# chihyaoma/cyclical-visual-captioning

Hardware: AMD Instinct MI355X
Metric: caption decode-steps/sec (BxT) at N=100,D=2048 (higher is better)
Workload: dtype f32; 1 GPU; cfg2: greedy caption decode; B_per_gpu=64, N=100, F=480, D=2048, A=1024, E=1024, V=5000, T=20, beam=1, hip_graph=True, parallelism=clips sharded over 1 rank(s), no collective, schedule=embedding-gate table (att-LSTM GEMM over K = 2R + one table row per word)

## Files before the change

### cyclical-visual-captioning_amd/csrc/blocks.hip

```cpp
#include <string.h>
#include "cvc_common.h"

namespace {
struct Entry { const char* name; void* fn; };
#define CVC_B(f) {#f, (void*)&f}
const Entry table[] = {
    CVC_B(cvc_attn_scores),
    CVC_B(cvc_attn_wsum),
    CVC_B(cvc_attn_scores_qparts),
    CVC_B(cvc_attn_wsum_quad),
    CVC_B(cvc_attn_wsum_frag),
    CVC_B(cvc_attn_wsum_quad_rm),
    CVC_B(cvc_attn_bwd_pair),
    CVC_B(cvc_ctxfeat_bwd_steps),
    CVC_B(cvc_tile_gemm_big),
    CVC_B(cvc_tile_gemm_plan),
    CVC_B(cvc_dproj_bwd_steps),
    CVC_B(cvc_linear_splitk_fwd),
    CVC_B(cvc_linear_top2_fwd),
    CVC_B(cvc_top2_final),
    CVC_B(cvc_packed_lstm_fwd),
    CVC_B(cvc_packed_linear_fwd),
    CVC_B(cvc_packed_lstm_embgate_fwd),
    CVC_B(cvc_packed_lstm_embgate_ex_fwd),
    CVC_B(cvc_packed_lstm_late_fwd),
    CVC_B(cvc_packed_lstm_train_fwd),
    CVC_B(cvc_packed_lstm_train_pre_fwd),
    CVC_B(cvc_packed_lstm_train_drop_fwd),
    CVC_B(cvc_lstm_pointwise_bwd),
    CVC_B(cvc_lstm_pointwise_bwd3),
    CVC_B(cvc_lstm_pointwise_bwd3_drop),
    CVC_B(cvc_pack_lstm_weights),
    CVC_B(cvc_linear_nn_planes_fwd),
    CVC_B(cvc_linear_nn_planes2_fwd),
    CVC_B(cvc_gru_seq_train_fwd),
    CVC_B(cvc_lstm_pointwise_bwd4_pair),
    CVC_B(cvc_beam_select_parts),
    CVC_B(cvc_sample_select_parts),
    CVC_B(cvc_sample_advance),
    CVC_B(cvc_tile_lstm_finish),
    CVC_B(cvc_tile_lstm_finish_embgate),
    CVC_B(cvc_tile_reorder_pack),
    CVC_B(cvc_decode_num_launches),
    CVC_B(cvc_gemm_force_generic),
    CVC_B(cvc_tile_gemm_loaders),
    CVC_B(cvc_gru_persistent_waves8),
    CVC_B(cvc_relu_dropout_fwd),
    CVC_B(cvc_relu_dropout_bwd),
    CVC_B(cvc_bn_workspace),
    CVC_B(cvc_bn_relu_train_fwd),
    CVC_B(cvc_bn_relu_train_bwd),
    CVC_B(cvc_class_softmax_bwd),
    CVC_B(cvc_layernorm_cat_bwd),
    CVC_B(cvc_attn_weighted_rows),
    CVC_B(cvc_stable_order),
    CVC_B(cvc_col_sum),
    CVC_B(cvc_col_sum_ws),
    CVC_B(cvc_lstm_persistent_sync_words),
    CVC_B(cvc_lstm_seq_persistent_fwd),
    CVC_B(cvc_lstm_seq_persistent_train_fwd),
    CVC_B(cvc_lstm_seq_fwd),
    CVC_B(cvc_lstm_seq_train_fwd),
    CVC_B(cvc_lstm_seq_bwd_work),
    CVC_B(cvc_lstm_seq_bwd),
    CVC_B(cvc_packed_lstm_bf16w_fwd),
    CVC_B(cvc_packed_linear_bf16w_fwd),
#ifdef CVC_EXPERIMENTAL
    CVC_B(cvc_gsk_plan),
    CVC_B(cvc_gsk_gemm),
    CVC_B(cvc_attn_scores_qslab),
    CVC_B(cvc_top2_slab),
    CVC_B(cvc_packed_lstm_ks_slices),
    CVC_B(cvc_packed_lstm_ks_fwd),
    CVC_B(cvc_packed_lstm_ksf_fwd),
    CVC_B(cvc_packed_lstm_ksx_local),
    CVC_B(cvc_packed_lstm_ksx_fwd),
    CVC_B(cvc_packed_lstm_wg_blocks),
    CVC_B(cvc_packed_linear_select_fwd),
    CVC_B(cvc_gru_persistent_halves),
#endif
};
}

extern "C" void* cvc_block(const char* name) {
    if (name == nullptr) return nullptr;
    for (const Entry& e : table)
        if (strcmp(e.name, name) == 0) return e.fn;
    return nullptr;
}
```

### cyclical-visual-captioning_amd/csrc/decode_driver.hip

```cpp
#include <hip/hip_runtime.h>
#include <new>
#include <stdint.h>
#include "../../include/cvc_hip.h"
#include "../../include/cvc_hip_blocks.h"
#include "../../include/cvc_hip_experimental.h"

struct gsk_launch {
    int U;
    int unit0[2], maxseg[2];
};
struct cvc_decode_plan {
    cvc_decode_desc d;
    int launches;
    gsk_launch ga, go, gl;
};

namespace {

#define CVC_TRY(expr)            \
    do {                         \
        int rc_ = (expr);        \
        ++n;                     \
        if (rc_ != 0) return rc_; \
    } while (0)

inline float* quad_off(float* buf, int k0) { return buf + (size_t)(k0 / 4) * 64 * 4; }
inline void* frag_off(void* xb, int k0) { return (char*)xb + (size_t)(k0 / 16) * 3 * 1024; }

int hip_rc(hipError_t e) { return e == hipSuccess ? 0 : (int)e; }

__global__ __launch_bounds__(256) void reset_kernel(uint4* dst, const uint4* src, size_t n16) {
    const size_t i = (size_t)blockIdx.x * 256 + threadIdx.x;
    if (i < n16) dst[i] = src != nullptr ? src[i] : uint4{0, 0, 0, 0};
}
int reset(void* dst, const void* src, size_t bytes, hipStream_t st) {
    if ((bytes & 15) || ((uintptr_t)dst & 15) || ((uintptr_t)src & 15)) {
        return hip_rc(src ? hipMemcpyAsync(dst, src, bytes, hipMemcpyDeviceToDevice, st) : hipMemsetAsync(dst, 0, bytes, st));
    }
    const size_t n16 = bytes / 16;
    hipLaunchKernelGGL(reset_kernel, dim3((unsigned)((n16 + 255) / 256)), dim3(256), 0, st, (uint4*)dst, (const uint4*)src, n16);
    return hip_rc(hipGetLastError());
}

void attn_sets(const cvc_decode_desc& d, int t, int rows, cvc_attn_set* sets) {
    sets[0] = cvc_attn_set{d.ppool, d.pool, d.mask, nullptr, d.scores_r, nullptr, d.att_steps + (size_t)t * rows * d.N, nullptr,
                           d.N, d.stream_r};
    sets[1] = cvc_attn_set{d.pconv, d.conv, nullptr, nullptr, d.scores_f, nullptr, d.attn_f, nullptr, d.F, d.stream_f};
}

int run_packed(cvc_decode_plan* p, hipStream_t st) {
    const cvc_decode_desc& d = p->d;
    const int rows = d.B, R = d.R, E = d.E, A = d.A, V = d.V, N = d.N;
    const size_t qbytes = (size_t)64 * 4 * sizeof(float);
    int n = 0;
    CVC_TRY(reset(d.xa[0], d.xa0_init, (size_t)((2 * R + E) / 4) * qbytes, st));
    CVC_TRY(reset(d.xl[0], nullptr, (size_t)(3 * R / 4) * qbytes, st));
    CVC_TRY(reset(d.ca[0], nullptr, (size_t)(R / 4) * qbytes, st));
    CVC_TRY(reset(d.cl[0], nullptr, (size_t)(R / 4) * qbytes, st));
    CVC_TRY(reset(d.words, nullptr, (size_t)rows * sizeof(int64_t), st));
    cvc_gemm_seg seg{d.fc, nullptr, d.w_fc, R, R, d.ld_w_fc, 0};
    CVC_TRY(cvc_linear_fwd(&seg, 1, d.b_ih_att, d.b_hh_att, rows, 4 * R, d.gate_fc, 4 * R, st));
    const int nblk_v = (V + 31) / 32;
    for (int t = 0; t < d.T; ++t) {
        const int rd = t & 1, wr = (t + 1) & 1;
        float *XA_r = d.xa[rd], *XA_w = d.xa[wr], *XL_r = d.xl[rd], *XL_w = d.xl[wr];
        CVC_TRY(cvc_packed_lstm_fwd((const float*)d.w_att, XA_r, 2 * R + E, nullptr, nullptr, d.gate_fc, d.ca[rd], rows, R,
                                    quad_off(XL_r, R), quad_off(XA_w, R + E), d.ca[wr], st));
        CVC_TRY(cvc_packed_linear_fwd((const float*)d.w_h, quad_off(XL_r, R), R, nullptr, rows, A, d.qsplit, d.q_parts, A, nullptr, st));
        cvc_attn_set sets[2];
        attn_sets(d, t, rows, sets);
        CVC_TRY(cvc_attn_scores_qparts(d.attn_kind, d.q_parts, d.qsplit, d.b_h, d.w_a, d.b_a, d.inv_temp, sets, 2, d.B, 1, A, st));
        CVC_TRY(cvc_attn_wsum_quad(sets, 2, d.B, 1, R, XL_r, st));
#ifdef CVC_EXPERIMENTAL
        if (d.lang_ksx)
            CVC_TRY(cvc_packed_lstm_ksx_fwd((const float*)d.w_lang, XL_r, 3 * R, d.b_ih_lang, d.b_hh_lang, nullptr, nullptr, nullptr, d.cl[rd],
                                            rows, R, XA_w, quad_off(XL_w, 2 * R), d.cl[wr], d.ksx_slab, d.ksx_flags, (unsigned)(t + 1), st));
        else
#endif
        CVC_TRY(cvc_packed_lstm_fwd((const float*)d.w_lang, XL_r, 3 * R, d.b_ih_lang, d.b_hh_lang, nullptr, d.cl[rd], rows, R, XA_w,
                                    quad_off(XL_w, 2 * R), d.cl[wr], st));
        CVC_TRY(cvc_packed_linear_fwd((const float*)d.w_o, XA_w, R, d.b_o, rows, V, 1, nullptr, V, d.top2_part, st));
        CVC_TRY(cvc_top2_final(d.top2_part, nblk_v, rows, d.unk_idx, d.words + (size_t)(t + 1) * rows, 1,
                               d.logprob ? d.logprob + (size_t)t * rows : nullptr, d.embed, E, quad_off(XA_w, R), 0, st));
    }
    p->launches = n;
    return 0;
}

int run_packed_eg(cvc_decode_plan* p, hipStream_t st) {
    const cvc_decode_desc& d = p->d;
    const int rows = d.B, R = d.R, A = d.A, V = d.V;
    const size_t qbytes = (size_t)64 * 4 * sizeof(float);
    int n = 0;
    CVC_TRY(reset(d.xa[0], nullptr, (size_t)(2 * R / 4) * qbytes, st));
    CVC_TRY(reset(d.xl[0], nullptr, (size_t)(3 * R / 4) * qbytes, st));
    CVC_TRY(reset(d.ca[0], nullptr, (size_t)(R / 4) * qbytes, st));
    CVC_TRY(reset(d.cl[0], nullptr, (size_t)(R / 4) * qbytes, st));
    CVC_TRY(reset(d.words, nullptr, (size_t)rows * sizeof(int64_t), st));
    cvc_gemm_seg seg{d.fc, nullptr, d.w_fc, R, R, d.ld_w_fc, 0};
    CVC_TRY(cvc_linear_fwd(&seg, 1, d.b_ih_att, d.b_hh_att, rows, 4 * R, d.gate_fc, 4 * R, st));
    const long long ws_att = (long long)(2 * R / 4) * 128, ws_lang = (long long)(3 * R / 4) * 128;
    const bool split2 = cvc_gemm_packed_split(-1) == 2;
    for (int t = 0; t < d.T; ++t) {
        const int rd = t & 1, wr = (t + 1) & 1;
        float *XA_r = d.xa[rd], *XA_w = d.xa[wr], *XL_r = d.xl[rd], *XL_w = d.xl[wr];
        const bool first = t == 0 && split2;
        CVC_TRY(cvc_packed_lstm_embgate_ex_fwd((const float*)d.w_att, ws_att, XA_r, first ? 32 : 2 * R, nullptr, nullptr, d.gate_fc,
                                               d.emb_gate, d.words + (size_t)t * rows, d.ca[rd], rows, R, quad_off(XL_r, R),
                                               quad_off(XA_w, R), d.ca[wr], d.att_w_cached, st));
        CVC_TRY(cvc_packed_linear_fwd((const float*)d.w_h, quad_off(XL_r, R), R, nullptr, rows, A, d.qsplit, d.q_parts, A, nullptr, st));
        cvc_attn_set sets[2];
        attn_sets(d, t, rows, sets);
        CVC_TRY(cvc_attn_scores_qparts(d.attn_kind, d.q_parts, d.qsplit, d.b_h, d.w_a, d.b_a, d.inv_temp, sets, 2, d.B, 1, A, st));
        CVC_TRY(cvc_attn_wsum_quad(sets, 2, d.B, 1, R, XL_r, st));
        if (first)
            CVC_TRY(cvc_packed_lstm_late_fwd((const float*)d.w_lang, ws_lang, XL_r, 2 * R, d.b_ih_lang, d.b_hh_lang, nullptr, d.cl[rd], rows,
                                             R, XA_w, quad_off(XL_w, 2 * R), d.cl[wr], nullptr, st));
#ifdef CVC_EXPERIMENTAL
        else if (d.lang_ksx)
            CVC_TRY(cvc_packed_lstm_ksx_fwd((const float*)d.w_lang, XL_r, 3 * R, d.b_ih_lang, d.b_hh_lang, nullptr, nullptr, nullptr, d.cl[rd],
                                            rows, R, XA_w, quad_off(XL_w, 2 * R), d.cl[wr], d.ksx_slab, d.ksx_flags, (unsigned)(t + 1), st));
#endif
        else
        CVC_TRY(cvc_packed_lstm_fwd((const float*)d.w_lang, XL_r, 3 * R, d.b_ih_lang, d.b_hh_lang, nullptr, d.cl[rd], rows, R, XA_w,
                                    quad_off(XL_w, 2 * R), d.cl[wr], st));
        CVC_TRY(cvc_packed_linear_fwd((const float*)d.w_o, XA_w, R, d.b_o, rows, V, 1, nullptr, V, d.top2_part, st));
        CVC_TRY(cvc_top2_final(d.top2_part, (V + 31) / 32, rows, d.unk_idx, d.words + (size_t)(t + 1) * rows, 1,
                               d.logprob ? d.logprob + (size_t)t * rows : nullptr, nullptr, 0, nullptr, 0, st));
    }
    p->launches = n;
    return 0;
}

#ifdef CVC_EXPERIMENTAL
int run_packed_gsk(cvc_decode_plan* p, hipStream_t st) {
    const cvc_decode_desc& d = p->d;
    const int rows = d.B, R = d.R, E = d.E, A = d.A, V = d.V;
    const size_t qbytes = (size_t)64 * 4 * sizeof(float);
    int n = 0;
    CVC_TRY(reset(d.xa[0], d.xa0_init, (size_t)((2 * R + E) / 4) * qbytes, st));
    CVC_TRY(reset(d.xl[0], nullptr, (size_t)(3 * R / 4) * qbytes, st));
    CVC_TRY(reset(d.ca[0], nullptr, (size_t)(R / 4) * qbytes, st));
    CVC_TRY(reset(d.cl[0], nullptr, (size_t)(R / 4) * qbytes, st));
    CVC_TRY(reset(d.words, nullptr, (size_t)rows * sizeof(int64_t), st));
    cvc_gemm_seg seg{d.fc, nullptr, d.w_fc, R, R, d.ld_w_fc, 0};
    CVC_TRY(cvc_linear_fwd(&seg, 1, d.b_ih_att, d.b_hh_att, rows, 4 * R, d.gate_fc, 4 * R, st));
    const long long ws_att = (long long)((2 * R + E) / 4) * 128, ws_lang = (long long)(3 * R / 4) * 128, ws_r = (long long)(R / 4) * 128;
    const float* w_att = (const float*)d.w_att;
    const float* w_lang = (const float*)d.w_lang;
    const int nblk_v = (V + 31) / 32;
    const cvc_gsk_segs seg_att{d.slab_att, p->ga.unit0[0], 2 * R / 32, p->ga.U, p->ga.maxseg[0]};
    const cvc_gsk_segs seg_o_a{d.slab_o, p->ga.unit0[1], R / 32, p->ga.U, p->ga.maxseg[1]};
    const cvc_gsk_segs seg_o_o{d.slab_o, 0, R / 32, p->go.U, p->go.maxseg[0]};
    const cvc_gsk_segs seg_lang{d.slab_lang, p->gl.unit0[0], 2 * R / 32, p->gl.U, p->gl.maxseg[0]};
    const cvc_gsk_segs seg_q{d.slab_q, p->gl.unit0[1], R / 32, p->gl.U, p->gl.maxseg[1]};
    for (int t = 0; t < d.T; ++t) {
        const int rd = t & 1, wr = (t + 1) & 1;
        float *XA_r = d.xa[rd], *XA_w = d.xa[wr], *XL_r = d.xl[rd], *XL_w = d.xl[wr];
        CVC_TRY(cvc_packed_lstm_late_fwd(w_att + (size_t)(R / 4) * 128, ws_att, quad_off(XA_r, R), E, nullptr, nullptr, d.gate_fc,
                                         d.ca[rd], rows, R, quad_off(XL_r, R), quad_off(XA_w, R + E), d.ca[wr],
                                         t == 0 ? nullptr : &seg_att, st));
        cvc_gsk_group gl[2] = {
            {w_lang, ws_lang, XL_r, R / 8, 2 * R / 32, 0, R / 32, d.slab_lang, p->gl.maxseg[0]},
            {(const float*)d.w_h, ws_r, quad_off(XL_r, R), A / 32, R / 32, 0, 0, d.slab_q, p->gl.maxseg[1]}};
        CVC_TRY(cvc_gsk_gemm(gl, 2, p->gl.U, st));
        cvc_attn_set sets[2];
        attn_sets(d, t, rows, sets);
        CVC_TRY(cvc_attn_scores_qslab(d.attn_kind, &seg_q, d.b_h, d.w_a, d.b_a, d.inv_temp, sets, 2, d.B, 1, A, st));
        CVC_TRY(cvc_attn_wsum_quad(sets, 2, d.B, 1, R, XL_r, st));
        CVC_TRY(cvc_packed_lstm_late_fwd(w_lang, ws_lang, XL_r, R, d.b_ih_lang, d.b_hh_lang, nullptr, d.cl[rd], rows, R, XA_w,
                                         quad_off(XL_w, 2 * R), d.cl[wr], &seg_lang, st));
        const bool last = t + 1 == d.T;
        cvc_gsk_group ga[2] = {
            {w_att, ws_att, XA_w, R / 8, 2 * R / 32, R / 32, E / 32, d.slab_att, p->ga.maxseg[0]},
            {(const float*)d.w_o, ws_r, XA_w, nblk_v, R / 32, 0, 0, d.slab_o, last ? p->go.maxseg[0] : p->ga.maxseg[1]}};
        if (last) CVC_TRY(cvc_gsk_gemm(ga + 1, 1, p->go.U, st));
        else CVC_TRY(cvc_gsk_gemm(ga, 2, p->ga.U, st));
        CVC_TRY(cvc_top2_slab(last ? &seg_o_o : &seg_o_a, d.b_o, V, rows, d.unk_idx, d.words + (size_t)(t + 1) * rows, 1,
                              d.logprob ? d.logprob + (size_t)t * rows : nullptr, d.embed, E, quad_off(XA_w, R), 0, st));
    }
    p->launches = n;
    return 0;
}

#endif

int run_tile(cvc_decode_plan* p, hipStream_t st) {
    const cvc_decode_desc& d = p->d;
    const int B = d.B, beam = d.beam, rows = B * beam, R = d.R, E = d.E, A = d.A, V = d.V;
    int n = 0;
    CVC_TRY(reset(d.words, nullptr, (size_t)rows * sizeof(int64_t), st));
    if (beam > 1) {
        CVC_TRY(reset(d.score, nullptr, (size_t)2 * rows * sizeof(float), st));
        CVC_TRY(reset(d.done, nullptr, (size_t)2 * rows, st));
    }
    CVC_TRY(cvc_tile_pack_rows(d.fc, R, nullptr, 0, B, R, d.xff, d.xff_stride, st));
    CVC_TRY(cvc_tile_gemm(d.w_fc_frag, d.xff, d.xff_stride, R, B, 4 * R, d.ks_fc, d.parts_fc, 4 * R, (long long)B * 4 * R, st));
    CVC_TRY(cvc_tile_linear_finish(d.parts_fc, d.ks_fc, (long long)B * 4 * R, 4 * R, d.b_ih_att, d.b_hh_att, B, 4 * R, d.gate_fc,
                                   4 * R, st));
    void* xl_hatt = frag_off(d.xlf, R);
    void* xl_hlang = frag_off(d.xlf, 2 * R);
    const bool eg = d.emb_gate != nullptr;
    const int E_pack = eg ? 0 : E, ka = 2 * R + E_pack;
    CVC_TRY(cvc_tile_reorder_pack(nullptr, d.words, beam, d.zero_state, d.zero_state, d.zero_state, d.zero_state, d.embed, E_pack, V,
                                  d.c_att_prev, d.c_lang_prev, d.xaf, d.xaf_stride, xl_hlang, d.xlf_stride, rows, R, st));
    const long long gs = (long long)rows * 4 * R;
    for (int t = 0; t < d.T; ++t) {
        CVC_TRY(cvc_tile_gemm(d.w_att, d.xaf, d.xaf_stride, ka, rows, 4 * R, d.ks_gate, d.parts_gate, 4 * R, gs, st));
        if (eg)
            CVC_TRY(cvc_tile_lstm_finish_embgate(d.parts_gate, d.ks_gate, gs, nullptr, nullptr, d.gate_fc, beam, d.emb_gate,
                                                 d.words + (size_t)t * rows, V, d.c_att_prev, rows, R, d.c_att, d.h_att, xl_hatt,
// ... 121 lines not shown
```

### cyclical-visual-captioning_amd/csrc/gemm_packed.hip

```cpp
#include "cvc_common.h"
#include "gemm_split.h"
#include "gsk.h"
#include "dropout_rng.h"

struct PackedArgs {
    const float* wp;
    const float* xq;
    int nquad;
    int M, Nout, R;
    const float* bias;
    const float* bias2;
    const float* gate_bias;
    const float* c_prev_q;
    float* c_out_q;
    float* h_dst1_q;
    float* h_dst2_q;
    float* y;
    int ldy;
    int ksplit;
    long long split_stride;
    float* top2_part;
    const float* c_prev_rm;
    float* h_rm;
    float* c_rm;
    float* gates_rm;
    float* h_rm2;
    float* h_rm3;
    long long gru_w_stride;
    long long gru_h_stride;
    const float* gru_gi[2];
    long long gru_gi_ld;
    float* gru_y[2];
    long long gru_y_ld;
    float* gru_gates[2];
    long long gru_g_ld;
    const float* emb_gate;
    const int64_t* word;
    unsigned* sel_counter;
    int64_t* sel_word; int sel_word_stride; float* sel_logprob; int sel_unk;
    int w_cached;
    DropSpec h3_drop;
    long long wstride;
    GskSegs early;
};

#ifdef CVC_TS
__device__ unsigned long long cvc_ts_buf[2 * 256 * 8 * 4];
extern "C" int cvc_debug_ts_read(unsigned long long* dst) {
    return hipMemcpyFromSymbol(dst, HIP_SYMBOL(cvc_ts_buf), sizeof(cvc_ts_buf)) == hipSuccess ? 0 : -1;
}
#define CVC_TS_MARK(k) do { if (LSTM && !GRU && lane == 0 && blockIdx.x < 256) ts_[k] = wall_clock64(); } while (0)
#else
#define CVC_TS_MARK(k) do {} while (0)
#endif

#ifndef CVC_LIN_W_NT
#define CVC_LIN_W_NT 0
#endif

template <int MT>
struct PFrag {
    f32x4 w[4];
    f32x4 x[MT][4];
#if defined(CVC_PABL) && CVC_PABL == 6
    f32x4 x2[MT][2];
#endif
};
template <int MT>
struct BFrag {
    u32x4 w[2];
    f32x4 x[MT][4];
};

template <int NW>
__device__ __forceinline__ float sum_partials(const float* red, int row, int ldm, int m) {
    float v = (red[(0 * 32 + row) * ldm + m] + red[(1 * 32 + row) * ldm + m]) +
              (red[(2 * 32 + row) * ldm + m] + red[(3 * 32 + row) * ldm + m]);
    if constexpr (NW == 8)
        v += (red[(4 * 32 + row) * ldm + m] + red[(5 * 32 + row) * ldm + m]) +
             (red[(6 * 32 + row) * ldm + m] + red[(7 * 32 + row) * ldm + m]);
    return v;
}

struct SelState { float t1, t2, gm, gs; int j1, j2; };
__device__ __forceinline__ SelState sel_init() { return SelState{-__builtin_inff(), -__builtin_inff(), -__builtin_inff(), 0.f, 0x7fffffff, 0x7fffffff}; }
__device__ __forceinline__ bool sel_better(float va, int ia, float vb, int ib) { return (va > vb) | ((va == vb) & (ia < ib)); }
__device__ __forceinline__ SelState sel_merge(SelState s, float u1, int k1, float u2, int k2, float um, float us) {
    if (sel_better(u1, k1, s.t1, s.j1)) {
        if (sel_better(s.t1, s.j1, u2, k2)) { s.t2 = s.t1; s.j2 = s.j1; } else { s.t2 = u2; s.j2 = k2; }
        s.t1 = u1; s.j1 = k1;
    } else if (sel_better(u1, k1, s.t2, s.j2)) { s.t2 = u1; s.j2 = k1; }
    const float nm = fmaxf(s.gm, um);
    s.gs = (nm == -__builtin_inff()) ? 0.f : s.gs * __expf(s.gm - nm) + us * __expf(um - nm);
    s.gm = nm;
    return s;
}

template <int MT, bool LSTM, int DEPTH, bool SPLIT, int NW, bool GRU = false, int NB = 1, bool SLAB = false, bool WC = false, bool WB16 = false>
__global__ __launch_bounds__(NW * 64) void skinny_gemm_packed_kernel(PackedArgs a) {
    static_assert(!WB16 || (SPLIT && NW == 8 && !GRU && NB == 1 && !SLAB), "bf16-stored weights: 8-wave split-product form only");
    using Frag = std::conditional_t<WB16, BFrag<MT>, PFrag<MT>>;
    using WT = std::conditional_t<WB16, uint16_t, float>;
    static_assert(!GRU || LSTM, "the GRU step shares the LSTM form's work split");
    static_assert(!SLAB || (LSTM && !GRU && NB == 1 && NW == 8), "slab sum: LSTM decode form, 8 waves, one block per workgroup");
    static_assert(NB == 1 || (LSTM && !GRU && NW == 8 && NB == 2), "two blocks per workgroup: LSTM form, 8 waves");
    constexpr int NWK = NW / NB;
    if constexpr (GRU) {
        a.wp += (size_t)blockIdx.y * a.gru_w_stride;
        a.xq += (size_t)blockIdx.y * a.gru_h_stride;
        a.h_dst1_q += (size_t)blockIdx.y * a.gru_h_stride;
        a.bias += (size_t)blockIdx.y * 3 * a.R;
        a.bias2 += (size_t)blockIdx.y * 3 * a.R;
    }
    static_assert(NW == 4 || NW == 8, "4 or 8 waves per workgroup");
    constexpr int LDM = MT * 32 + 1;
    __shared__ float red[(NW + (SLAB ? 1 : 0)) * 32 * LDM + NW * 64 * 6];
    const int tid = threadIdx.x, lane = tid & 63;
    const int wave = __builtin_amdgcn_readfirstlane(tid >> 6);
    const int i = lane & 31, kh = lane >> 5;
    const int M = a.M, R = a.R;
#ifdef CVC_TS
    unsigned long long ts_[4] = {0, 0, 0, 0};
#endif
    CVC_TS_MARK(0);

    int nchunk = a.nquad >> 3, c0 = 0;
    if (!LSTM && a.ksplit > 1) {
        const int lo = nchunk * (int)blockIdx.y / a.ksplit, hi = nchunk * ((int)blockIdx.y + 1) / a.ksplit;
        c0 = lo;
        nchunk = hi - lo;
    }
    const int wblk = NB == 1 ? 0 : wave / NWK, kw = NB == 1 ? wave : wave % NWK;
    const int n_my = nchunk > kw ? (nchunk - kw + NWK - 1) / NWK : 0;
    const WT* wl = reinterpret_cast<const WT*>(a.wp) + (size_t)((int)blockIdx.x * NB + wblk) * a.wstride + (size_t)i * (WB16 ? 8 : 4) +
                   (size_t)(c0 + kw) * 8 * 128 + kh * 4 * 128;
    const float* xl = a.xq + (size_t)i * 4 + (size_t)(c0 + kw) * 8 * 256 + kh * 4 * 256;
    constexpr size_t WSTEP = (size_t)NWK * 8 * 128, XSTEP = (size_t)NWK * 8 * 256;
#ifndef CVC_ROT_MUL
#define CVC_ROT_MUL 5
#endif
    const int rot = n_my > 0 ? (int)((blockIdx.x * CVC_ROT_MUL) % (unsigned)n_my) : 0;

    auto load = [&](Frag& f, int j) __attribute__((always_inline)) {
#if defined(CVC_PABL) && CVC_PABL == 1
        if (j > 0) { asm volatile("" : "+v"(f.w[0])); return; }
#endif
        int jr = j + rot;
        jr = jr >= n_my ? jr - n_my : jr;
        const WT* w = wl + (size_t)jr * WSTEP;
#if defined(CVC_PABL) && CVC_PABL == 4
        const float* x = a.xq + (size_t)i * 4 + kh * 4 * 256;
#else
        const float* x = xl + (size_t)jr * XSTEP;
#endif
        if constexpr (WB16) {
#pragma unroll
            for (int s2 = 0; s2 < 2; ++s2) {
                if constexpr (LSTM && !WC) f.w[s2] = __builtin_nontemporal_load(reinterpret_cast<const u32x4*>(w + s2 * 256));
                else f.w[s2] = *reinterpret_cast<const u32x4*>(w + s2 * 256);
#pragma unroll
                for (int q = 2 * s2; q < 2 * s2 + 2; ++q)
#pragma unroll
                    for (int mt = 0; mt < MT; ++mt) f.x[mt][q] = ld4(x + q * 256 + mt * 128);
            }
        } else {
#pragma unroll
            for (int q = 0; q < 4; ++q) {
                if constexpr (((LSTM && !GRU) || CVC_LIN_W_NT) && !WC) f.w[q] = __builtin_nontemporal_load(reinterpret_cast<const f32x4*>(w + q * 128));
                else f.w[q] = ld4(w + q * 128);
#if defined(CVC_PABL) && CVC_PABL == 3
                if (j > 0) continue;
#endif
#pragma unroll
                for (int mt = 0; mt < MT; ++mt) f.x[mt][q] = ld4(x + q * 256 + mt * 128);
            }
#if defined(CVC_PABL) && CVC_PABL == 6
            {
                int ja = jr + (n_my >> 1);
                ja = ja >= n_my ? ja - n_my : ja;
                const float* xa = xl + (size_t)ja * XSTEP;
#pragma unroll
                for (int s2 = 0; s2 < 2; ++s2)
#pragma unroll
                    for (int mt = 0; mt < MT; ++mt) f.x2[mt][s2] = ld4(xa + (s2 + 2) * 256 + mt * 128 + 64);
            }
#endif
        }
    };

    f32x4 eadd4[4] = {{0, 0, 0, 0}, {0, 0, 0, 0}, {0, 0, 0, 0}, {0, 0, 0, 0}};
    if constexpr (LSTM && !GRU) {
        if (a.emb_gate != nullptr && tid < NB * 2 * 64) {
            const int em0 = tid & 63;
            const long long eword = a.word[em0 < a.M ? em0 : a.M - 1];
            const float* trow = a.emb_gate + (size_t)eword * 4 * a.R + (size_t)((int)blockIdx.x * NB + (tid >> 7)) * 8 + ((tid >> 6) & 1) * 4;
#pragma unroll
            for (int g = 0; g < 4; ++g) eadd4[g] = ld4(trow + (size_t)g * a.R);
        }
    }

    f32x16 acc[MT];
#pragma unroll
    for (int mt = 0; mt < MT; ++mt)
#pragma unroll
        for (int r = 0; r < 16; ++r) acc[mt][r] = 0.f;

    auto mma = [&](const Frag& f) __attribute__((always_inline)) {
        if constexpr (WB16) {
#pragma unroll
            for (int s2 = 0; s2 < 2; ++s2) {
#pragma unroll
                for (int mt = 0; mt < MT; ++mt) {
                    const Split3 X = split8(f.x[mt][2 * s2], f.x[mt][2 * s2 + 1]);
                    acc[mt] = mfma_bf16(f.w[s2], X.lo, acc[mt]);
                    acc[mt] = mfma_bf16(f.w[s2], X.mid, acc[mt]);
                    acc[mt] = mfma_bf16(f.w[s2], X.hi, acc[mt]);
                }
            }
        } else {
#if defined(CVC_PABL) && CVC_PABL >= 2 && CVC_PABL <= 4
#pragma unroll
            for (int q = 0; q < 4; ++q) {
                asm volatile("" ::"v"(f.w[q]));
#pragma unroll
                for (int mt = 0; mt < MT; ++mt) asm volatile("" ::"v"(f.x[mt][q]));
            }
            return;
#endif
            if constexpr (SPLIT) {
#pragma unroll
                for (int s2 = 0; s2 < 2; ++s2) {
                    const Split3 W = split8(f.w[2 * s2], f.w[2 * s2 + 1]);
#pragma unroll
                    for (int mt = 0; mt < MT; ++mt) {
#if defined(CVC_PABL) && (CVC_PABL == 5 || CVC_PABL == 6)
                        Split3 X;
                        X.hi = __builtin_bit_cast(u32x4, f.x[mt][2 * s2]); X.mid = __builtin_bit_cast(u32x4, f.x[mt][2 * s2 + 1]);
#if CVC_PABL == 6
                        X.lo = __builtin_bit_cast(u32x4, f.x2[mt][s2]);
#else
                        X.lo = X.hi;
#endif
#else
                        const Split3 X = split8(f.x[mt][2 * s2], f.x[mt][2 * s2 + 1]);
#endif
                        acc[mt] = mfma_bf16(W.mid, X.mid, acc[mt]);
                        acc[mt] = mfma_bf16(W.lo, X.hi, acc[mt]);
                        acc[mt] = mfma_bf16(W.hi, X.lo, acc[mt]);
                        acc[mt] = mfma_bf16(W.mid, X.hi, acc[mt]);
                        acc[mt] = mfma_bf16(W.hi, X.mid, acc[mt]);
                        acc[mt] = mfma_bf16(W.hi, X.hi, acc[mt]);
                    }
// ... 39 lines not shown
                } else if constexpr (SPLIT) {
#pragma unroll
                    for (int g = 0; g < 4 + 4 * MT; ++g) {
                        __builtin_amdgcn_sched_group_barrier(0x002, 18, 0);
                        __builtin_amdgcn_sched_group_barrier(0x008, MT, 0);
                        __builtin_amdgcn_sched_group_barrier(0x020, 1, 0);
                    }
                } else {
#pragma unroll
                    for (int g = 0; g < 4 + 4 * MT; ++g) {
                        __builtin_amdgcn_sched_group_barrier(0x008, 2, 0);
                        __builtin_amdgcn_sched_group_barrier(0x020, 1, 0);
                        __builtin_amdgcn_sched_group_barrier(0x002, 2, 0);
                    }
                }
                __builtin_amdgcn_sched_barrier(0);
            }
        }
#pragma unroll
        for (int s = 0; s < DEPTH; ++s) {
            if (j + s + DEPTH - 1 < n_my) load(ring[(s + DEPTH - 1) % DEPTH], j + s + DEPTH - 1);
            if (j + s < n_my) mma(ring[s]);
        }
#pragma unroll
        for (int s = 0; s < DEPTH - 1; ++s)
            if (j + DEPTH + s < n_my) mma(ring[s]);
    } else {
        for (int j = 0; j < n_my; ++j) {
            load(ring[0], j);
            mma(ring[0]);
        }
    }

    CVC_TS_MARK(2);
    const int em = tid & 63, eqd = (tid >> 6) & 1, eb = tid >> 7;
    const bool ework = LSTM && tid < NB * 2 * 64 && em < M && em < MT * 32;
    const int ejq = ((int)blockIdx.x * NB + eb) * 8 + eqd * 4;
    const float* ered = red + (NB == 1 ? 0 : eb * NWK * 32 * LDM);
    const size_t eqoff = ((size_t)(ejq / 4) * 64 + em) * 4;
    f32x4 ecp = {0, 0, 0, 0}, eadd[4] = {{0, 0, 0, 0}, {0, 0, 0, 0}, {0, 0, 0, 0}, {0, 0, 0, 0}};
    f32x4 eadd2[4] = {{0, 0, 0, 0}, {0, 0, 0, 0}, {0, 0, 0, 0}, {0, 0, 0, 0}}, eadd3[4] = {{0, 0, 0, 0}, {0, 0, 0, 0}, {0, 0, 0, 0}, {0, 0, 0, 0}};

    if (GRU && ework) {
        const float* gi = (blockIdx.y == 0 ? a.gru_gi[0] : a.gru_gi[1]) + (size_t)em * a.gru_gi_ld + ejq;
        ecp = ld4(a.xq + eqoff);
#pragma unroll
        for (int g = 0; g < 3; ++g) {
            eadd[g] = ld4(gi + g * R) + ld4(a.bias + g * R + ejq);
            if (g < 2) eadd[g] += ld4(a.bias2 + g * R + ejq);
        }
        eadd[3] = ld4(a.bias2 + 2 * R + ejq);
    } else if (ework) {
        ecp = a.c_prev_rm != nullptr ? ld4(a.c_prev_rm + (size_t)em * R + ejq) : ld4(a.c_prev_q + eqoff);
        if (a.bias != nullptr) {
#pragma unroll
            for (int g = 0; g < 4; ++g) eadd[g] = ld4(a.bias + g * R + ejq);
        }
        if (a.bias2 != nullptr) {
#pragma unroll
            for (int g = 0; g < 4; ++g) eadd2[g] = ld4(a.bias2 + g * R + ejq);
        }
        if (a.gate_bias != nullptr) {
#pragma unroll
            for (int g = 0; g < 4; ++g) eadd3[g] = ld4(a.gate_bias + (size_t)em * 4 * R + g * R + ejq);
        }
    }

    constexpr int SLAB_MAXS = 10;
    f32x4 sv[SLAB ? SLAB_MAXS : 1];
    int s_nseg = 0;
    const float* s_p0 = nullptr;
    if constexpr (SLAB) {
        const int tile = (int)blockIdx.x >> 3, j = (int)blockIdx.x & 7;
        s_nseg = gsk_nseg(a.early, tile);
        s_p0 = gsk_part(a.early, tile, 0, j) + (size_t)tid * 4;
#pragma unroll
        for (int s = 0; s < SLAB_MAXS; ++s) sv[s] = ld4(s_p0 + (size_t)(s < s_nseg ? s : s_nseg - 1) * (8 * 2048));
    }

    constexpr int ECPW = 32 / NW;
    float ebias[ECPW];
#pragma unroll
    for (int c = 0; c < ECPW; ++c) {
        const int n = (int)blockIdx.x * 32 + wave * ECPW + c;
        ebias[c] = (!LSTM && a.top2_part != nullptr && a.bias != nullptr) ? a.bias[n < a.Nout ? n : a.Nout - 1] : 0.f;
    }

#pragma unroll
    for (int mt = 0; mt < MT; ++mt)
#pragma unroll
        for (int r = 0; r < 16; ++r) {
            const int row = (r & 3) + 8 * (r >> 2) + 4 * kh;
            red[(wave * 32 + row) * LDM + mt * 32 + i] = acc[mt][r];
        }
    if constexpr (SLAB) {
        f32x4 t = sv[0];
#pragma unroll
        for (int s = 1; s < SLAB_MAXS; ++s) t += s < s_nseg ? sv[s] : f32x4{0.f, 0.f, 0.f, 0.f};
        for (int s = SLAB_MAXS; s < s_nseg; ++s) t += ld4(s_p0 + (size_t)s * (8 * 2048));
        if ((tid >> 3) < MT * 32) {
#pragma unroll
            for (int e = 0; e < 4; ++e) red[(NW * 32 + (tid & 7) * 4 + e) * LDM + (tid >> 3)] = t[e];
        }
    }
    __syncthreads();

    if constexpr (GRU) {
        if (ework) {
            f32x4 hv, gr, gz, gn, gh;
#pragma unroll
            for (int e = 0; e < 4; ++e) {
                const int jj = eqd * 4 + e;
                float pre[3];
#pragma unroll
                for (int g = 0; g < 3; ++g) pre[g] = sum_partials<NWK>(ered, g * 8 + jj, LDM, em);
                const float rg = fast_sigmoid(pre[0] + eadd[0][e]), zg = fast_sigmoid(pre[1] + eadd[1][e]);
                const float hn = pre[2] + eadd[3][e];
                const float ng = fast_tanh(eadd[2][e] + rg * hn);
                hv[e] = ng + zg * (ecp[e] - ng);
                gr[e] = rg; gz[e] = zg; gn[e] = ng; gh[e] = hn;
            }
            st4(a.h_dst1_q + eqoff, hv);
            st4((blockIdx.y == 0 ? a.gru_y[0] : a.gru_y[1]) + (size_t)em * a.gru_y_ld + ejq, hv);
            float* gp = blockIdx.y == 0 ? a.gru_gates[0] : a.gru_gates[1];
            if (gp != nullptr) {
                gp += (size_t)em * a.gru_g_ld + ejq;
                st4(gp, gr); st4(gp + a.R, gz); st4(gp + 2 * a.R, gn); st4(gp + 3 * a.R, gh);
            }
        }
    } else if (LSTM) {
        if (ework) {
            f32x4 hv, cv, gv[4];
#pragma unroll
            for (int g = 0; g < 4; ++g) eadd[g] = ((eadd[g] + eadd2[g]) + eadd3[g]) + eadd4[g];
#pragma unroll
            for (int e = 0; e < 4; ++e) {
                const int jj = eqd * 4 + e;
                float pre[4];
#pragma unroll
                for (int g = 0; g < 4; ++g) {
                    float sp = sum_partials<NWK>(ered, g * 8 + jj, LDM, em);
                    if constexpr (SLAB) sp += red[(NW * 32 + g * 8 + jj) * LDM + em];
                    pre[g] = sp + eadd[g][e];
                }
                const float ig = fast_sigmoid(pre[0]), fg = fast_sigmoid(pre[1]);
                const float gg = fast_tanh(pre[2]), og = fast_sigmoid(pre[3]);
                const float c2 = fg * ecp[e] + ig * gg;
                cv[e] = c2;
                hv[e] = og * fast_tanh(c2);
                gv[0][e] = ig; gv[1][e] = fg; gv[2][e] = gg; gv[3][e] = og;
            }
            if (a.c_out_q != nullptr) st4(a.c_out_q + eqoff, cv);
            if (a.h_dst1_q != nullptr) st4(a.h_dst1_q + eqoff, hv);
            if (a.h_dst2_q != nullptr) st4(a.h_dst2_q + eqoff, hv);
            if (a.h_rm != nullptr) st4(a.h_rm + (size_t)em * R + ejq, hv);
            if (a.h_rm2 != nullptr) st4(a.h_rm2 + (size_t)em * R + ejq, hv);
            if (a.h_rm3 != nullptr) {
                f32x4 hd = hv;
                if (a.h3_drop.state != nullptr) {
                    const uint32_t s0 = a.h3_drop.state[0], s1 = a.h3_drop.state[1], s2 = a.h3_drop.state[2];
                    const uint32_t i0 = (uint32_t)em * (uint32_t)R + (uint32_t)ejq;
#pragma unroll
                    for (int e = 0; e < 4; ++e) hd[e] *= cvc_drop_mult(a.h3_drop, s0, s1, s2, i0 + e);
                }
                st4(a.h_rm3 + (size_t)em * R + ejq, hd);
            }
            if (a.c_rm != nullptr) st4(a.c_rm + (size_t)em * R + ejq, cv);
            if (a.gates_rm != nullptr) {
#pragma unroll
                for (int g = 0; g < 4; ++g) st4(a.gates_rm + (size_t)em * 4 * R + g * R + ejq, gv[g]);
            }
        }
#ifdef CVC_TS
        asm volatile("s_waitcnt vmcnt(0)" ::: "memory");
        CVC_TS_MARK(3);
        if (lane == 0 && blockIdx.x < 256) {
            unsigned long long* d = cvc_ts_buf + ((size_t)((a.nquad >= 1536 ? 0 : 1) * 256 + blockIdx.x) * 8 + wave) * 4;
            d[0] = ts_[0]; d[1] = ts_[1]; d[2] = ts_[2]; d[3] = ts_[3];
        }
#endif
    } else {
        const int n0 = blockIdx.x * 32;
        const bool lead = blockIdx.y == 0;
        float* y = a.y != nullptr ? a.y + (long long)blockIdx.y * a.split_stride : nullptr;
        if (y != nullptr) {
            for (int u = tid; u < 32 * MT * 32; u += NW * 64) {
                const int nl = u & 31, m = u >> 5;
                const int n = n0 + nl;
                if (m >= M || n >= a.Nout) continue;
                float v = sum_partials<NW>(red, nl, LDM, m);
                if (lead && a.bias != nullptr) v += a.bias[n];
                y[(size_t)m * a.ldy + n] = v;
            }
        }
        if (a.top2_part != nullptr) {
            float* scratch = red + NW * 32 * LDM;
            float v1 = -__builtin_inff(), v2 = -__builtin_inff(), mx = -__builtin_inff(), se = 0.f;
            int i1 = 0x7fffffff, i2 = 0x7fffffff;
            const int m = lane < MT * 32 ? lane : MT * 32 - 1;
            constexpr int CPW = 32 / NW;
#pragma unroll
            for (int c = 0; c < CPW; ++c) {
                const int nl = wave * CPW + c, n = n0 + nl;
                if (n >= a.Nout) break;
                const float v = sum_partials<NW>(red, nl, LDM, m) + ebias[c];
                if (v > v1) { v2 = v1; i2 = i1; v1 = v; i1 = n; }
                else if (v > v2) { v2 = v; i2 = n; }
                const float nm = fmaxf(mx, v);
                se = se * __expf(mx - nm) + __expf(v - nm);
                mx = nm;
            }
            float* r4 = scratch + ((size_t)wave * 64 + lane) * 6;
            r4[0] = v1; r4[1] = __int_as_float(i1); r4[2] = v2; r4[3] = __int_as_float(i2); r4[4] = mx; r4[5] = se;
            __syncthreads();
            if (wave == 0 && lane < M) {
                for (int w = 1; w < NW; ++w) {
                    const float* q4 = scratch + ((size_t)w * 64 + lane) * 6;
                    const float u1 = q4[0], u2 = q4[2];
                    const int k1 = __float_as_int(q4[1]), k2 = __float_as_int(q4[3]);
                    if (u1 > v1) { if (v1 >= u2) { v2 = v1; i2 = i1; } else { v2 = u2; i2 = k2; } v1 = u1; i1 = k1; }
                    else if (u1 > v2) { v2 = u1; i2 = k1; }
                    const float nm = fmaxf(mx, q4[4]);
                    se = (nm == -__builtin_inff()) ? 0.f : se * __expf(mx - nm) + q4[5] * __expf(q4[4] - nm);
                    mx = nm;
                }
                float* rec = a.top2_part + ((size_t)blockIdx.x * 64 + lane) * 6;
                if (a.sel_counter != nullptr) {
                    const float r6[6] = {v1, __int_as_float(i1), v2, __int_as_float(i2), mx, se};
#pragma unroll
                    for (int k = 0; k < 6; ++k) __hip_atomic_store(rec + k, r6[k], __ATOMIC_RELAXED, __HIP_MEMORY_SCOPE_AGENT);
                } else {
                    rec[0] = v1; rec[1] = __int_as_float(i1); rec[2] = v2; rec[3] = __int_as_float(i2); rec[4] = mx; rec[5] = se;
                }
            }
            if (a.sel_counter != nullptr) {
                asm volatile("s_waitcnt vmcnt(0)" ::: "memory");
                __syncthreads();
                int* flag = reinterpret_cast<int*>(scratch);
                if (tid == 0) {
                    const unsigned old = __hip_atomic_fetch_add(a.sel_counter, 1u, __ATOMIC_RELAXED, __HIP_MEMORY_SCOPE_AGENT);
                    const bool last = old == gridDim.x - 1;
                    if (last) {
                        __hip_atomic_store(a.sel_counter, 0u, __ATOMIC_RELAXED, __HIP_MEMORY_SCOPE_AGENT);
                        __builtin_amdgcn_fence(__ATOMIC_ACQUIRE, "agent");
                    }
                    flag[0] = last ? 1 : 0;
                }
                __syncthreads();
                if (flag[0] == 0) return;
                __syncthreads();
                const int nb = (int)gridDim.x;
                SelState ss = sel_init();
                const int mrow = lane < M ? lane : M - 1;
                constexpr int RB = 8;
                for (int b0 = wave; b0 < nb; b0 += NW * RB) {
                    f32x2 r0[RB], r1[RB], r2[RB];
#pragma unroll
                    for (int k = 0; k < RB; ++k) {
                        const int b = b0 + k * NW;
                        const f32x2* q2 = reinterpret_cast<const f32x2*>(a.top2_part + ((size_t)(b < nb ? b : nb - 1) * 64 + mrow) * 6);
                        r0[k] = q2[0]; r1[k] = q2[1]; r2[k] = q2[2];
                    }
#pragma unroll
                    for (int k = 0; k < RB; ++k)
                        if (b0 + k * NW < nb) ss = sel_merge(ss, r0[k].x, __float_as_int(r0[k].y), r1[k].x, __float_as_int(r1[k].y), r2[k].x, r2[k].y);
                }
                float* r8 = scratch + ((size_t)wave * 64 + lane) * 6;
                r8[0] = ss.t1; r8[1] = __int_as_float(ss.j1); r8[2] = ss.t2; r8[3] = __int_as_float(ss.j2); r8[4] = ss.gm; r8[5] = ss.gs;
                __syncthreads();
                if (wave == 0 && lane < M) {
                    for (int w = 1; w < NW; ++w) {
                        const float* q4 = scratch + ((size_t)w * 64 + lane) * 6;
                        ss = sel_merge(ss, q4[0], __float_as_int(q4[1]), q4[2], __float_as_int(q4[3]), q4[4], q4[5]);
                    }
                    const bool use2 = (ss.j1 == a.sel_unk) && ss.j2 != 0x7fffffff;
                    int wsel = use2 ? ss.j2 : ss.j1;
                    if (wsel == 0x7fffffff || wsel < 0) wsel = 0;
                    a.sel_word[(size_t)lane * a.sel_word_stride] = wsel;
                    if (a.sel_logprob != nullptr) a.sel_logprob[lane] = (use2 ? ss.t2 : ss.t1) - (ss.gm + __logf(ss.gs));
                }
            }
        }
    }
}

#ifndef CVC_PACKED_DEPTH
#define CVC_PACKED_DEPTH 4
#endif
#ifndef CVC_PACKED_DEPTH8
#define CVC_PACKED_DEPTH8 3
#endif
#ifndef CVC_BF16W_DEPTH
#define CVC_BF16W_DEPTH 4
#endif

static int cvc_packed_lstm_blocks = 1;
extern "C" int cvc_packed_lstm_wg_blocks(int n) {
    const int prev = cvc_packed_lstm_blocks;
    if (n >= 1) cvc_packed_lstm_blocks = n >= 2 ? 2 : 1;
    return prev;
}

template <bool LSTM>
static int launch_packed(const PackedArgs& a_in, int blocks, hipStream_t st) {
    PackedArgs a = a_in;
    if (a.M < 1 || a.M > 64 || (a.nquad & 7) || a.nquad < 8) return CVC_E_BADARG;
    if (a.wstride == 0) a.wstride = (long long)a.nquad * 128;
    const dim3 grid(blocks, LSTM || a.ksplit < 1 ? 1 : a.ksplit);
    if constexpr (LSTM) {
        if (cvc_gemm_split_mode == 2 && cvc_packed_lstm_blocks == 2 && (blocks & 1) == 0 && a.M > 32 && a.h_rm == nullptr && a.c_prev_rm == nullptr) {
            hipLaunchKernelGGL((skinny_gemm_packed_kernel<2, true, CVC_PACKED_DEPTH8, true, 8, false, 2>), dim3(blocks / 2), dim3(512), 0, st, a);
            return cvc_launch_status();
        }
    }
    if constexpr (LSTM) {
        if (cvc_gemm_split_mode == 2 && a.w_cached) {
            if (a.M > 32) hipLaunchKernelGGL((skinny_gemm_packed_kernel<2, true, CVC_PACKED_DEPTH8, true, 8, false, 1, false, true>), grid, dim3(512), 0, st, a);
            else hipLaunchKernelGGL((skinny_gemm_packed_kernel<1, true, CVC_PACKED_DEPTH8, true, 8, false, 1, false, true>), grid, dim3(512), 0, st, a);
            return cvc_launch_status();
        }
    }
    if (cvc_gemm_split_mode == 2) {
        if (a.M <= 32) hipLaunchKernelGGL((skinny_gemm_packed_kernel<1, LSTM, CVC_PACKED_DEPTH8, true, 8>), grid, dim3(512), 0, st, a);
        else hipLaunchKernelGGL((skinny_gemm_packed_kernel<2, LSTM, CVC_PACKED_DEPTH8, true, 8>), grid, dim3(512), 0, st, a);
    } else if (cvc_gemm_split_mode) {
        if (a.M <= 32) hipLaunchKernelGGL((skinny_gemm_packed_kernel<1, LSTM, CVC_PACKED_DEPTH, true, 4>), grid, dim3(256), 0, st, a);
        else hipLaunchKernelGGL((skinny_gemm_packed_kernel<2, LSTM, CVC_PACKED_DEPTH, true, 4>), grid, dim3(256), 0, st, a);
    } else {
        if (a.M <= 32) hipLaunchKernelGGL((skinny_gemm_packed_kernel<1, LSTM, CVC_PACKED_DEPTH, false, 4>), grid, dim3(256), 0, st, a);
        else hipLaunchKernelGGL((skinny_gemm_packed_kernel<2, LSTM, CVC_PACKED_DEPTH, false, 4>), grid, dim3(256), 0, st, a);
    }
    return cvc_launch_status();
}

template <bool LSTM>
static int launch_packed_bf16w(PackedArgs a, int blocks, hipStream_t st) {
    if (a.wstride == 0) a.wstride = (long long)a.nquad * 128;
    const dim3 grid(blocks, LSTM || a.ksplit < 1 ? 1 : a.ksplit);
    if constexpr (LSTM) {
        if (a.w_cached) {
            if (a.M <= 32) hipLaunchKernelGGL((skinny_gemm_packed_kernel<1, true, CVC_BF16W_DEPTH, true, 8, false, 1, false, true, true>), grid, dim3(512), 0, st, a);
            else hipLaunchKernelGGL((skinny_gemm_packed_kernel<2, true, CVC_BF16W_DEPTH, true, 8, false, 1, false, true, true>), grid, dim3(512), 0, st, a);
            return cvc_launch_status();
        }
    }
    if (a.M <= 32) hipLaunchKernelGGL((skinny_gemm_packed_kernel<1, LSTM, CVC_BF16W_DEPTH, true, 8, false, 1, false, false, true>), grid, dim3(512), 0, st, a);
    else hipLaunchKernelGGL((skinny_gemm_packed_kernel<2, LSTM, CVC_BF16W_DEPTH, true, 8, false, 1, false, false, true>), grid, dim3(512), 0, st, a);
    return cvc_launch_status();
}

extern "C" int cvc_packed_lstm_fwd(const float* wp, const float* xq, int K, const float* b_ih, const float* b_hh,
                                   const float* gate_bias, const float* c_prev_q, int M, int R, float* h_dst1_q,
                                   float* h_dst2_q, float* c_out_q, cvc_stream_t stream) {
    if (!wp || !xq || !c_prev_q || !c_out_q || (K & 31) || R < 8 || (R & 7)) return CVC_E_BADARG;
    PackedArgs a{};
    a.wp = wp; a.xq = xq; a.nquad = K / 4; a.M = M; a.Nout = 4 * R; a.R = R;
    a.bias = b_ih; a.bias2 = b_hh; a.gate_bias = gate_bias; a.c_prev_q = c_prev_q; a.c_out_q = c_out_q;
    a.h_dst1_q = h_dst1_q; a.h_dst2_q = h_dst2_q; a.ksplit = 1;
    return launch_packed<true>(a, R / 8, (hipStream_t)stream);
}

extern "C" int cvc_packed_lstm_embgate_fwd(const float* wp, const float* xq, int K, const float* b_ih, const float* b_hh,
                                           const float* gate_bias, const float* emb_gate, const int64_t* word,
                                           const float* c_prev_q, int M, int R, float* h_dst1_q, float* h_dst2_q,
                                           float* c_out_q, cvc_stream_t stream) {
    if (!wp || !xq || !c_prev_q || !c_out_q || !emb_gate || !word || (K & 31) || R < 8 || (R & 7)) return CVC_E_BADARG;
    PackedArgs a{};
    a.wp = wp; a.xq = xq; a.nquad = K / 4; a.M = M; a.Nout = 4 * R; a.R = R;
    a.bias = b_ih; a.bias2 = b_hh; a.gate_bias = gate_bias; a.c_prev_q = c_prev_q; a.c_out_q = c_out_q;
    a.h_dst1_q = h_dst1_q; a.h_dst2_q = h_dst2_q; a.ksplit = 1; a.emb_gate = emb_gate; a.word = word;
    return launch_packed<true>(a, R / 8, (hipStream_t)stream);
}

extern "C" int cvc_packed_lstm_embgate_ex_fwd(const float* wp, long long w_blk_stride, const float* xq, int K, const float* b_ih,
                                              const float* b_hh, const float* gate_bias, const float* emb_gate, const int64_t* word,
                                              const float* c_prev_q, int M, int R, float* h_dst1_q, float* h_dst2_q,
                                              float* c_out_q, int w_cached, cvc_stream_t stream) {
    if (!wp || !xq || !c_prev_q || !c_out_q || !emb_gate || !word || (K & 31) || K < 32 || R < 8 || (R & 7)) return CVC_E_BADARG;
    if (w_blk_stride != 0 && (w_blk_stride < (long long)(K / 4) * 128 || (w_blk_stride & 3))) return CVC_E_BADARG;
    PackedArgs a{};
    a.wp = wp; a.xq = xq; a.nquad = K / 4; a.M = M; a.Nout = 4 * R; a.R = R; a.wstride = w_blk_stride;
    a.bias = b_ih; a.bias2 = b_hh; a.gate_bias = gate_bias; a.c_prev_q = c_prev_q; a.c_out_q = c_out_q;
    a.h_dst1_q = h_dst1_q; a.h_dst2_q = h_dst2_q; a.ksplit = 1; a.emb_gate = emb_gate; a.word = word; a.w_cached = w_cached ? 1 : 0;
    return launch_packed<true>(a, R / 8, (hipStream_t)stream);
}

extern "C" int cvc_packed_lstm_bf16w_fwd(const uint16_t* wp, long long w_blk_stride, const float* xq, int K, const float* b_ih,
                                         const float* b_hh, const float* gate_bias, const float* emb_gate, const int64_t* word,
                                         const float* c_prev_q, int M, int R, float* h_dst1_q, float* h_dst2_q, float* c_out_q,
                                         int w_cached, cvc_stream_t stream) {
    if (!wp || !xq || !c_prev_q || !c_out_q || (K & 31) || K < 32 || R < 8 || (R & 7) || M < 1 || M > 64) return CVC_E_BADARG;
    if ((emb_gate != nullptr) != (word != nullptr)) return CVC_E_BADARG;
    if (w_blk_stride != 0 && (w_blk_stride < (long long)K * 32 || (w_blk_stride & 7))) return CVC_E_BADARG;
    if (((uintptr_t)wp & 15) || ((uintptr_t)xq & 15)) return CVC_E_BADARG;
    PackedArgs a{};
    a.wp = reinterpret_cast<const float*>(wp); a.xq = xq; a.nquad = K / 4; a.M = M; a.Nout = 4 * R; a.R = R; a.wstride = w_blk_stride;
    a.bias = b_ih; a.bias2 = b_hh; a.gate_bias = gate_bias; a.c_prev_q = c_prev_q; a.c_out_q = c_out_q;
    a.h_dst1_q = h_dst1_q; a.h_dst2_q = h_dst2_q; a.ksplit = 1; a.emb_gate = emb_gate; a.word = word; a.w_cached = w_cached ? 1 : 0;
    return launch_packed_bf16w<true>(a, R / 8, (hipStream_t)stream);
}

extern "C" int cvc_packed_lstm_late_fwd(const float* wp, long long w_blk_stride, const float* xq, int K, const float* b_ih,
                                        const float* b_hh, const float* gate_bias, const float* c_prev_q, int M, int R,
                                        float* h_dst1_q, float* h_dst2_q, float* c_out_q, const cvc_gsk_segs* early,
                                        cvc_stream_t stream) {
    if (!wp || !xq || !c_prev_q || !c_out_q || (K & 31) || K < 32 || R < 8 || (R & 7) || M < 1 || M > 64 ||
        w_blk_stride < (long long)(K / 4) * 128 || (w_blk_stride & 3))
        return CVC_E_BADARG;
    if (cvc_gemm_split_mode != 2) return CVC_E_BADARG;
    PackedArgs a{};
    a.wp = wp; a.xq = xq; a.nquad = K / 4; a.M = M; a.Nout = 4 * R; a.R = R; a.wstride = w_blk_stride;
    a.bias = b_ih; a.bias2 = b_hh; a.gate_bias = gate_bias; a.c_prev_q = c_prev_q; a.c_out_q = c_out_q;
    a.h_dst1_q = h_dst1_q; a.h_dst2_q = h_dst2_q; a.ksplit = 1;
    const dim3 grid(R / 8);
    hipStream_t st = (hipStream_t)stream;
    if (early != nullptr) {
        if (!early->slab || early->nchunk < 1 || early->U < 1 || early->maxseg < 1 || early->unit0 < 0 || (R & 63)) return CVC_E_BADARG;
        a.early = *early;
        if (M <= 32) hipLaunchKernelGGL((skinny_gemm_packed_kernel<1, true, CVC_PACKED_DEPTH8, true, 8, false, 1, true>), grid, dim3(512), 0, st, a);
        else hipLaunchKernelGGL((skinny_gemm_packed_kernel<2, true, CVC_PACKED_DEPTH8, true, 8, false, 1, true>), grid, dim3(512), 0, st, a);
    } else {
        if (M <= 32) hipLaunchKernelGGL((skinny_gemm_packed_kernel<1, true, CVC_PACKED_DEPTH8, true, 8>), grid, dim3(512), 0, st, a);
        else hipLaunchKernelGGL((skinny_gemm_packed_kernel<2, true, CVC_PACKED_DEPTH8, true, 8>), grid, dim3(512), 0, st, a);
    }
    return cvc_launch_status();
}

static int packed_lstm_train_impl(const float* wp, const float* xq, int K, const float* b_ih, const float* b_hh, const float* gate_pre,
                                  const float* c_prev, int M, int R, float* h_out, float* c_out, float* gates_out, float* h_out2,
                                  float* h_out3, cvc_stream_t stream, DropSpec h3_drop = DropSpec{nullptr, 0, 0, 0.f});
// ... 166 lines not shown
#pragma unroll
    for (int i = 0; i < 5; ++i) s += (i < a.nseg - 1 && q >= a.q_end[i]) ? 1 : 0;
    const int qs = q - (s ? a.q_end[s - 1] : 0);
    f32x4 v = {0, 0, 0, 0};
    if (m < a.M) v = ld4(a.x[s] + (size_t)m * a.ldx[s] + qs * 4);
    st4(a.xq + ((size_t)q * 64 + m) * 4, v);
}

}

extern "C" int cvc_pack_lstm_segs(const float* const* ws, const long long* lds, const int* widths, int nseg, int R, float* wp,
                                  cvc_stream_t stream) {
    if (!ws || !lds || !widths || !wp || nseg < 1 || nseg > 4 || R < 8 || (R & 7)) return CVC_E_BADARG;
    PackWArgs a{};
    int q = 0;
    for (int s = 0; s < nseg; ++s) {
        if (!ws[s] || widths[s] < 4 || (widths[s] & 3) || lds[s] < widths[s] || (lds[s] & 3) || ((uintptr_t)ws[s] & 15)) return CVC_E_BADARG;
        q += widths[s] / 4;
        a.w[s] = ws[s]; a.ld[s] = lds[s]; a.q_end[s] = q;
    }
    if (q & 7) return CVC_E_BADARG;
    a.nseg = nseg; a.R = R; a.wp = wp;
    hipLaunchKernelGGL(pack_lstm_w_kernel, dim3(R / 8, (q + 63) / 64), dim3(256), 0, (hipStream_t)stream, a);
    return cvc_launch_status();
}

extern "C" int cvc_pack_lstm_weights(const float* w_ih, int K_ih, const float* w_hh, int K_hh, int R, float* wp,
                                     cvc_stream_t stream) {
    if (!w_ih || !w_hh || !wp || K_ih < 4 || K_hh < 4 || (K_ih & 3) || (K_hh & 3) || ((K_ih + K_hh) & 31) || R < 8 || (R & 7))
        return CVC_E_BADARG;
    const float* ws[2] = {w_ih, w_hh};
    const long long lds[2] = {K_ih, K_hh};
    const int widths[2] = {K_ih, K_hh};
    return cvc_pack_lstm_segs(ws, lds, widths, 2, R, wp, stream);
}

extern "C" int cvc_pack_quad_segs(const float* const* xs, const long long* ldx, const int* widths, int nseg, int M, float* xq,
                                  cvc_stream_t stream) {
    if (!xs || !ldx || !widths || !xq || nseg < 1 || nseg > 6 || M < 1 || M > 64) return CVC_E_BADARG;
    PackXArgs a{};
    int q = 0;
    for (int s = 0; s < nseg; ++s) {
        if (!xs[s] || widths[s] < 4 || (widths[s] & 3) || (ldx[s] & 3) || ((uintptr_t)xs[s] & 15)) return CVC_E_BADARG;
        q += widths[s] / 4;
        a.x[s] = xs[s]; a.ldx[s] = ldx[s]; a.q_end[s] = q;
    }
    a.nseg = nseg; a.M = M; a.xq = xq;
    hipLaunchKernelGGL(pack_quad_segs_kernel, dim3((q * 64 + 255) / 256), dim3(256), 0, (hipStream_t)stream, a);
    return cvc_launch_status();
}

extern "C" int cvc_packed_linear_select_fwd(const float* wp, const float* xq, int K, const float* bias, int M, int Nout,
                                            float* top2_part, unsigned* counter, int unk_idx, int64_t* word, int word_stride,
                                            float* logprob, cvc_stream_t stream) {
    if (!wp || !xq || (K & 31) || Nout < 2 || !top2_part || !counter || !word || word_stride < 1 || M < 1 || M > 64) return CVC_E_BADARG;
    PackedArgs a{};
    a.wp = wp; a.xq = xq; a.nquad = K / 4; a.M = M; a.Nout = Nout; a.R = 0;
    a.bias = bias; a.ksplit = 1; a.top2_part = top2_part;
    a.sel_counter = counter; a.sel_unk = unk_idx; a.sel_word = word; a.sel_word_stride = word_stride; a.sel_logprob = logprob;
    return launch_packed<false>(a, (Nout + 31) / 32, (hipStream_t)stream);
}

extern "C" int cvc_packed_linear_fwd(const float* wp, const float* xq, int K, const float* bias, int M, int Nout,
                                     int ksplit, float* y, int ldy, float* top2_part, cvc_stream_t stream) {
    if (!wp || !xq || (K & 31) || Nout < 1 || ksplit < 1 || (!y && !top2_part)) return CVC_E_BADARG;
    if (ksplit > 1 && top2_part != nullptr) return CVC_E_BADARG;
    PackedArgs a{};
    a.wp = wp; a.xq = xq; a.nquad = K / 4; a.M = M; a.Nout = Nout; a.R = 0;
    a.bias = bias; a.y = y; a.ldy = ldy; a.ksplit = ksplit; a.split_stride = (long long)M * ldy; a.top2_part = top2_part;
    return launch_packed<false>(a, (Nout + 31) / 32, (hipStream_t)stream);
}

extern "C" int cvc_packed_linear_bf16w_fwd(const uint16_t* wp, const float* xq, int K, const float* bias, int M, int Nout,
                                           int ksplit, float* y, int ldy, float* top2_part, cvc_stream_t stream) {
    if (!wp || !xq || (K & 31) || K < 32 || Nout < 1 || ksplit < 1 || (!y && !top2_part) || M < 1 || M > 64) return CVC_E_BADARG;
    if (ksplit > 1 && top2_part != nullptr) return CVC_E_BADARG;
    if (y != nullptr && ldy < Nout) return CVC_E_BADARG;
    if (((uintptr_t)wp & 15) || ((uintptr_t)xq & 15)) return CVC_E_BADARG;
    PackedArgs a{};
    a.wp = reinterpret_cast<const float*>(wp); a.xq = xq; a.nquad = K / 4; a.M = M; a.Nout = Nout; a.R = 0;
    a.bias = bias; a.y = y; a.ldy = ldy; a.ksplit = ksplit; a.split_stride = (long long)M * ldy; a.top2_part = top2_part;
    return launch_packed_bf16w<false>(a, (Nout + 31) / 32, (hipStream_t)stream);
}
```

### cyclical-visual-captioning_amd/csrc/vocab.hip

```cpp
#include "cvc_common.h"
#include "gsk.h"
#include "dropout_rng.h"
#include <math.h>

namespace {

constexpr int WG = 256;

__device__ __forceinline__ float block_sum(float v, float* red) {
    const int lane = threadIdx.x & 63, wave = threadIdx.x >> 6;
    v = wave_sum(v);
    __syncthreads();
    if (lane == 0) red[wave] = v;
    __syncthreads();
    return (red[0] + red[1]) + (red[2] + red[3]);
}
__device__ __forceinline__ float block_max(float v, float* red) {
    const int lane = threadIdx.x & 63, wave = threadIdx.x >> 6;
    v = wave_max(v);
    __syncthreads();
    if (lane == 0) red[wave] = v;
    __syncthreads();
    return fmaxf(fmaxf(red[0], red[1]), fmaxf(red[2], red[3]));
}

__global__ __launch_bounds__(WG) void embed_relu_fwd_kernel(const float* table, const int64_t* idx, const float* drop, DropSpec rng,
                                                            int M, int E, float* out) {
    const int m = blockIdx.y;
    const int e = (blockIdx.x * WG + threadIdx.x) * 4;
    if (e >= E) return;
    f32x4 v = ld4(table + (size_t)idx[m] * E + e);
    v.x = fmaxf(v.x, 0.f); v.y = fmaxf(v.y, 0.f); v.z = fmaxf(v.z, 0.f); v.w = fmaxf(v.w, 0.f);
    if (drop != nullptr) v *= ld4(drop + (size_t)m * E + e);
    if (rng.state != nullptr) {
        const uint32_t s0 = rng.state[0], s1 = rng.state[1], s2 = rng.state[2], i0 = (uint32_t)m * (uint32_t)E + (uint32_t)e;
#pragma unroll
        for (int k = 0; k < 4; ++k) v[k] *= cvc_drop_mult(rng, s0, s1, s2, i0 + k);
    }
    st4(out + (size_t)m * E + e, v);
}

__global__ __launch_bounds__(WG) void dropout_rng_kernel(const float* x, DropSpec rng, size_t n, float* y) {
    const size_t i = ((size_t)blockIdx.x * WG + threadIdx.x) * 4;
    if (i >= n) return;
    const uint32_t s0 = rng.state[0], s1 = rng.state[1], s2 = rng.state[2];
    if (i + 4 <= n) {
        f32x4 v = ld4(x + i);
#pragma unroll
        for (int k = 0; k < 4; ++k) v[k] *= cvc_drop_mult(rng, s0, s1, s2, (uint32_t)(i + k));
        st4(y + i, v);
    } else {
        for (size_t k = i; k < n; ++k) y[k] = x[k] * cvc_drop_mult(rng, s0, s1, s2, (uint32_t)k);
    }
}

constexpr int EMB_CHUNK = 16;

__global__ __launch_bounds__(WG) void embed_bwd_pieces_kernel(const int64_t* idx, const int64_t* order, const float* drop, DropSpec rng,
                                                              const float* d_out, int M, int E, float* part) {
    const int r0 = blockIdx.y * EMB_CHUNK;
    const int e = (blockIdx.x * WG + threadIdx.x) * 4;
    if (e >= E) return;
    const int r1 = min(M, r0 + EMB_CHUNK);
    int start = r0;
    int64_t w = idx[order[r0]];
    f32x4 acc = {0, 0, 0, 0};
    for (int r = r0; r < r1; ++r) {
        const int64_t m = order[r];
        const int64_t wr = idx[m];
        if (wr != w) {
            st4(part + (size_t)start * E + e, acc);
            acc = f32x4{0, 0, 0, 0};
            start = r;
            w = wr;
        }
        f32x4 g = ld4(d_out + (size_t)m * E + e);
        if (drop != nullptr) g *= ld4(drop + (size_t)m * E + e);
        if (rng.state != nullptr) {
            const uint32_t s0 = rng.state[0], s1 = rng.state[1], s2 = rng.state[2], i0 = (uint32_t)m * (uint32_t)E + (uint32_t)e;
#pragma unroll
            for (int k = 0; k < 4; ++k) g[k] *= cvc_drop_mult(rng, s0, s1, s2, i0 + k);
        }
        acc += g;
    }
    st4(part + (size_t)start * E + e, acc);
// ... 16 lines not shown
}

__global__ __launch_bounds__(WG) void log_softmax_kernel(const float* logits, int V, float* logp) {
    __shared__ float red[4];
    const float* x = logits + (size_t)blockIdx.x * V;
    float* y = logp + (size_t)blockIdx.x * V;
    float m = -INFINITY;
    for (int v = threadIdx.x; v < V; v += WG) m = fmaxf(m, x[v]);
    m = block_max(m, red);
    float s = 0.f;
    for (int v = threadIdx.x; v < V; v += WG) s += expf(x[v] - m);
    s = block_sum(s, red);
    const float lse = m + logf(s);
    for (int v = threadIdx.x; v < V; v += WG) y[v] = x[v] - lse;
}

__global__ __launch_bounds__(WG) void log_softmax_bwd_kernel(const float* logp, const float* d_logp, int V, float* d_logits) {
    __shared__ float red[4];
    const size_t o = (size_t)blockIdx.x * V;
    float s = 0.f;
    for (int v = threadIdx.x; v < V; v += WG) s += d_logp[o + v];
    s = block_sum(s, red);
    for (int v = threadIdx.x; v < V; v += WG) d_logits[o + v] = d_logp[o + v] - expf(logp[o + v]) * s;
}

__global__ __launch_bounds__(WG) void nll_bwd_kernel(const int64_t* target, const float* w, const float* g, int V,
                                                     float* d_logp) {
    const int m = blockIdx.y;
    const int v = blockIdx.x * WG + threadIdx.x;
    if (v >= V) return;
    d_logp[(size_t)m * V + v] = v == (int)target[m] ? -w[m] * g[0] : 0.f;
}

struct Top2 { float v1; int i1; float v2; int i2; };
__device__ __forceinline__ bool better(float va, int ia, float vb, int ib) { return (va > vb) | ((va == vb) & (ia < ib)); }
__device__ __forceinline__ Top2 merge(Top2 a, Top2 b) {
    Top2 r;
    if (better(a.v1, a.i1, b.v1, b.i1)) {
        r.v1 = a.v1; r.i1 = a.i1;
        if (better(a.v2, a.i2, b.v1, b.i1)) { r.v2 = a.v2; r.i2 = a.i2; } else { r.v2 = b.v1; r.i2 = b.i1; }
    } else {
        r.v1 = b.v1; r.i1 = b.i1;
        if (better(b.v2, b.i2, a.v1, a.i1)) { r.v2 = b.v2; r.i2 = b.i2; } else { r.v2 = a.v1; r.i2 = a.i1; }
    }
    return r;
}

__global__ __launch_bounds__(WG) void top2_unk_kernel(const float* logits, int V, int unk, int64_t* word, int wstride,
                                                      float* logprob) {
    __shared__ float red[4];
    __shared__ Top2 tred[4];
    const int row = blockIdx.x;
    const float* x = logits + (size_t)row * V;
    Top2 t{-INFINITY, 0x7fffffff, -INFINITY, 0x7fffffff};
    for (int v = threadIdx.x; v < V; v += WG) {
        const float xv = x[v];
        if (better(xv, v, t.v1, t.i1)) { t.v2 = t.v1; t.i2 = t.i1; t.v1 = xv; t.i1 = v; }
        else if (better(xv, v, t.v2, t.i2)) { t.v2 = xv; t.i2 = v; }
    }
#pragma unroll
    for (int o = 32; o > 0; o >>= 1) {
        Top2 u;
        u.v1 = __shfl_xor(t.v1, o, 64); u.i1 = __shfl_xor(t.i1, o, 64);
        u.v2 = __shfl_xor(t.v2, o, 64); u.i2 = __shfl_xor(t.i2, o, 64);
        t = merge(t, u);
    }
    const int lane = threadIdx.x & 63, wave = threadIdx.x >> 6;
    if (lane == 0) tred[wave] = t;
    __syncthreads();
    t = merge(merge(tred[0], tred[1]), merge(tred[2], tred[3]));
    const float m = t.v1;
    float s = 0.f;
    for (int v = threadIdx.x; v < V; v += WG) s += expf(x[v] - m);
    s = block_sum(s, red);
    if (threadIdx.x == 0) {
        const bool use2 = (t.i1 == unk) && V > 1;
        int w = use2 ? t.i2 : t.i1;
        if ((unsigned)w >= (unsigned)V) w = 0;
        word[(size_t)row * wstride] = w;
        if (logprob != nullptr) logprob[row] = (use2 ? t.v2 : t.v1) - (m + logf(s));
    }
}

__global__ __launch_bounds__(WG) void top2_final_kernel(const float* part, int nblocks, int unk, int64_t* word, int wstride,
                                                        float* logprob, const float* table, int E, float* emb_out, int emb_ld) {
    __shared__ float red[4];
    __shared__ Top2 tred[4];
    __shared__ int chosen;
    const int row = blockIdx.x;
    Top2 t{-INFINITY, 0x7fffffff, -INFINITY, 0x7fffffff};
    float mx = -INFINITY;
    for (int b = threadIdx.x; b < nblocks; b += WG) {
        const float* rec = part + ((size_t)b * 64 + row) * 6;
        Top2 u{rec[0], __float_as_int(rec[1]), rec[2], __float_as_int(rec[3])};
        t = merge(t, u);
        mx = fmaxf(mx, rec[4]);
    }
#pragma unroll
    for (int o = 32; o > 0; o >>= 1) {
        Top2 u;
        u.v1 = __shfl_xor(t.v1, o, 64); u.i1 = __shfl_xor(t.i1, o, 64);
        u.v2 = __shfl_xor(t.v2, o, 64); u.i2 = __shfl_xor(t.i2, o, 64);
        t = merge(t, u);
    }
    const int lane = threadIdx.x & 63, wave = threadIdx.x >> 6;
    if (lane == 0) tred[wave] = t;
    mx = block_max(mx, red);
    t = merge(merge(tred[0], tred[1]), merge(tred[2], tred[3]));
    float se = 0.f;
    for (int b = threadIdx.x; b < nblocks; b += WG) {
        const float* rec = part + ((size_t)b * 64 + row) * 6;
        se += rec[5] * expf(rec[4] - mx);
    }
    se = block_sum(se, red);
    if (threadIdx.x == 0) {
        const bool use2 = (t.i1 == unk) && t.i2 != 0x7fffffff;
        int w = use2 ? t.i2 : t.i1;
        if (w == 0x7fffffff || w < 0) w = 0;
        word[(size_t)row * wstride] = w;
        if (logprob != nullptr) logprob[row] = (use2 ? t.v2 : t.v1) - (mx + logf(se));
        chosen = w;
    }
    if (emb_out != nullptr) {
        __syncthreads();
        const float* src = table + (size_t)chosen * E;
        for (int e = threadIdx.x * 4; e < E; e += WG * 4) {
            f32x4 v = ld4(src + e);
            v.x = fmaxf(v.x, 0.f); v.y = fmaxf(v.y, 0.f); v.z = fmaxf(v.z, 0.f); v.w = fmaxf(v.w, 0.f);
            if (emb_ld > 0) st4(emb_out + (size_t)row * emb_ld + e, v);
            else st4(emb_out + ((size_t)(e >> 2) * 64 + row) * 4, v);
        }
    }
}

template <int ITEMS>
__global__ __launch_bounds__(WG) void top2_slab_kernel(GskSegs g, const float* bias, int V, int unk, int64_t* word, int wstride,
                                                       float* logprob, const float* table, int E, float* emb_out, int emb_ld) {
    __shared__ float red[4];
    __shared__ Top2 tred[4];
    __shared__ int chosen;
    constexpr int MAXS = 6;
    const int row = blockIdx.x;
    const int nitem = ((V + 31) >> 5) * 8;
    f32x4 sv[ITEMS][MAXS], bv[ITEMS];
    int nseg[ITEMS], col0[ITEMS];
    const float* p0[ITEMS];
#pragma unroll
    for (int k = 0; k < ITEMS; ++k) {
        const int it = min((int)threadIdx.x + k * WG, nitem - 1);
        const int blk = it >> 3, rq = it & 7;
        nseg[k] = gsk_nseg(g, blk >> 3);
        col0[k] = (int)threadIdx.x + k * WG < nitem ? blk * 32 + rq * 4 : V;
        p0[k] = gsk_part(g, blk >> 3, 0, blk & 7) + (size_t)row * 32 + rq * 4;
#pragma unroll
        for (int s = 0; s < MAXS; ++s) sv[k][s] = ld4(p0[k] + (size_t)(s < nseg[k] ? s : nseg[k] - 1) * (8 * 2048));
#pragma unroll
        for (int e = 0; e < 4; ++e) bv[k][e] = (bias != nullptr && col0[k] + e < V) ? bias[col0[k] + e] : 0.f;
    }
    Top2 t{-INFINITY, 0x7fffffff, -INFINITY, 0x7fffffff};
    float mx = -INFINITY;
    f32x4 val[ITEMS];
#pragma unroll
    for (int k = 0; k < ITEMS; ++k) {
        f32x4 x = sv[k][0];
#pragma unroll
        for (int s = 1; s < MAXS; ++s) x += s < nseg[k] ? sv[k][s] : f32x4{0.f, 0.f, 0.f, 0.f};
        for (int s = MAXS; s < nseg[k]; ++s) x += ld4(p0[k] + (size_t)s * (8 * 2048));
        x += bv[k];
#pragma unroll
        for (int e = 0; e < 4; ++e) {
            const int v = col0[k] + e;
            const float xv = v < V ? x[e] : -INFINITY;
            val[k][e] = xv;
            if (v < V) {
                if (better(xv, v, t.v1, t.i1)) { t.v2 = t.v1; t.i2 = t.i1; t.v1 = xv; t.i1 = v; }
                else if (better(xv, v, t.v2, t.i2)) { t.v2 = xv; t.i2 = v; }
                mx = fmaxf(mx, xv);
            }
        }
    }
#pragma unroll
    for (int o = 32; o > 0; o >>= 1) {
        Top2 u;
        u.v1 = __shfl_xor(t.v1, o, 64); u.i1 = __shfl_xor(t.i1, o, 64);
        u.v2 = __shfl_xor(t.v2, o, 64); u.i2 = __shfl_xor(t.i2, o, 64);
        t = merge(t, u);
    }
    const int lane = threadIdx.x & 63, wave = threadIdx.x >> 6;
    if (lane == 0) tred[wave] = t;
    mx = block_max(mx, red);
    t = merge(merge(tred[0], tred[1]), merge(tred[2], tred[3]));
    float se = 0.f;
#pragma unroll
    for (int k = 0; k < ITEMS; ++k)
#pragma unroll
        for (int e = 0; e < 4; ++e) se += val[k][e] == -INFINITY ? 0.f : expf(val[k][e] - mx);
    se = block_sum(se, red);
    if (threadIdx.x == 0) {
        const bool use2 = (t.i1 == unk) && t.i2 != 0x7fffffff;
        int w = use2 ? t.i2 : t.i1;
        if (w == 0x7fffffff || w < 0) w = 0;
        word[(size_t)row * wstride] = w;
        if (logprob != nullptr) logprob[row] = (use2 ? t.v2 : t.v1) - (mx + logf(se));
// ... 501 lines not shown
#else
extern "C" const char* cvc_version(void) { return "cvc_hip 0.2 gfx950"; }
#endif

static int embed_fwd_impl(const float* table, const int64_t* idx, const float* drop, DropSpec rng, int M, int E, float* out,
                          cvc_stream_t stream) {
    if (!table || !idx || !out || M < 1 || E < 4 || (E & 3) || (long long)M * E > 0xffffffffll) return CVC_E_BADARG;
    hipLaunchKernelGGL(embed_relu_fwd_kernel, dim3((E / 4 + WG - 1) / WG, M), dim3(WG), 0, (hipStream_t)stream, table, idx,
                       drop, rng, M, E, out);
    return cvc_launch_status();
}

static int embed_bwd_impl(const float* table, const int64_t* idx, const int64_t* order, const float* drop, DropSpec rng,
                          const float* d_out, int M, int E, float* d_table, float* workspace, cvc_stream_t stream) {
    if (!table || !idx || !order || !d_out || !d_table || !workspace || M < 1 || E < 4 || (E & 3)) return CVC_E_BADARG;
    const int gx = (E / 4 + WG - 1) / WG;
    hipLaunchKernelGGL(embed_bwd_pieces_kernel, dim3(gx, (M + EMB_CHUNK - 1) / EMB_CHUNK), dim3(WG), 0, (hipStream_t)stream, idx,
                       order, drop, rng, d_out, M, E, workspace);
    hipLaunchKernelGGL(embed_bwd_runs_kernel, dim3(gx, M), dim3(WG), 0, (hipStream_t)stream, table, idx, order, workspace, M, E,
                       d_table);
    return cvc_launch_status();
}

extern "C" int cvc_embed_relu_fwd(const float* table, const int64_t* idx, const float* drop, int M, int E, float* out,
                                  cvc_stream_t stream) {
    return embed_fwd_impl(table, idx, drop, cvc_drop_spec(nullptr, 0, 0.f), M, E, out, stream);
}

extern "C" int cvc_embed_relu_bwd(const float* table, const int64_t* idx, const int64_t* order, const float* drop,
                                  const float* d_out, int M, int E, float* d_table, float* workspace, cvc_stream_t stream) {
    return embed_bwd_impl(table, idx, order, drop, cvc_drop_spec(nullptr, 0, 0.f), d_out, M, E, d_table, workspace, stream);
}

extern "C" int cvc_embed_relu_rng_fwd(const float* table, const int64_t* idx, const uint32_t* rng_state, unsigned site, float p, int M,
                                      int E, float* out, cvc_stream_t stream) {
    if (!rng_state || p < 0.f || p >= 1.f) return CVC_E_BADARG;
    return embed_fwd_impl(table, idx, nullptr, cvc_drop_spec(rng_state, site, p), M, E, out, stream);
}

extern "C" int cvc_embed_relu_rng_bwd(const float* table, const int64_t* idx, const int64_t* order, const uint32_t* rng_state,
                                      unsigned site, float p, const float* d_out, int M, int E, float* d_table, float* workspace,
                                      cvc_stream_t stream) {
    if (!rng_state || p < 0.f || p >= 1.f) return CVC_E_BADARG;
    return embed_bwd_impl(table, idx, order, nullptr, cvc_drop_spec(rng_state, site, p), d_out, M, E, d_table, workspace, stream);
}

extern "C" int cvc_dropout_rng(const float* x, long long n, const uint32_t* rng_state, unsigned site, float p, float* y,
                               cvc_stream_t stream) {
    if (!x || !y || !rng_state || n < 1 || n > 0xffffffffll || p < 0.f || p >= 1.f || ((uintptr_t)x & 15) || ((uintptr_t)y & 15))
        return CVC_E_BADARG;
    hipLaunchKernelGGL(dropout_rng_kernel, dim3((unsigned)((n / 4 + WG) / WG)), dim3(WG), 0, (hipStream_t)stream, x,
                       cvc_drop_spec(rng_state, site, p), (size_t)n, y);
    return cvc_launch_status();
}

extern "C" int cvc_log_softmax_fwd(const float* logits, int M, int V, float* logp, cvc_stream_t stream) {
    if (!logits || !logp || M < 1 || V < 1) return CVC_E_BADARG;
    hipLaunchKernelGGL(log_softmax_kernel, dim3(M), dim3(WG), 0, (hipStream_t)stream, logits, V, logp);
    return cvc_launch_status();
}

extern "C" int cvc_log_softmax_bwd(const float* logp, const float* d_logp, int M, int V, float* d_logits,
                                   cvc_stream_t stream) {
    if (!logp || !d_logp || !d_logits || M < 1 || V < 1) return CVC_E_BADARG;
    hipLaunchKernelGGL(log_softmax_bwd_kernel, dim3(M), dim3(WG), 0, (hipStream_t)stream, logp, d_logp, V, d_logits);
    return cvc_launch_status();
}

extern "C" int cvc_nll_bwd(const int64_t* target, const float* w, const float* g, int M, int V, float* d_logp,
                           cvc_stream_t stream) {
    if (!target || !w || !g || !d_logp || M < 1 || V < 1) return CVC_E_BADARG;
    hipLaunchKernelGGL(nll_bwd_kernel, dim3((V + WG - 1) / WG, M), dim3(WG), 0, (hipStream_t)stream, target, w, g, V, d_logp);
    return cvc_launch_status();
}

extern "C" int cvc_top2_unk(const float* logits, int M, int V, int unk_idx, int64_t* word, int word_stride,
                            float* logprob, cvc_stream_t stream) {
    if (!logits || !word || M < 1 || V < 1 || word_stride < 1) return CVC_E_BADARG;
    hipLaunchKernelGGL(top2_unk_kernel, dim3(M), dim3(WG), 0, (hipStream_t)stream, logits, V, unk_idx, word, word_stride,
                       logprob);
    return cvc_launch_status();
}

extern "C" int cvc_top2_final(const float* part, int nblocks, int M, int unk_idx, int64_t* word, int word_stride,
                              float* logprob, const float* table, int E, float* emb_out, int emb_ld,
                              cvc_stream_t stream) {
    if (!part || !word || nblocks < 1 || M < 1 || M > 64 || word_stride < 1) return CVC_E_BADARG;
    if (emb_out != nullptr && (!table || E < 4 || (E & 3) || (emb_ld & 3) || (emb_ld != 0 && emb_ld < E))) return CVC_E_BADARG;
    hipLaunchKernelGGL(top2_final_kernel, dim3(M), dim3(WG), 0, (hipStream_t)stream, part, nblocks, unk_idx, word, word_stride,
                       logprob, table, E, emb_out, emb_ld);
    return cvc_launch_status();
}

extern "C" int cvc_top2_slab(const cvc_gsk_segs* logits, const float* bias, int V, int M, int unk_idx, int64_t* word,
                             int word_stride, float* logprob, const float* table, int E, float* emb_out, int emb_ld,
                             cvc_stream_t stream) {
    if (!logits || !logits->slab || logits->nchunk < 1 || logits->U < 1 || logits->maxseg < 1 || logits->unit0 < 0 || !word || V < 2 ||
        M < 1 || M > 64 || word_stride < 1)
        return CVC_E_BADARG;
    if (emb_out != nullptr && (!table || E < 4 || (E & 3) || (emb_ld & 3) || (emb_ld != 0 && emb_ld < E))) return CVC_E_BADARG;
    const int nitem = ((V + 31) / 32) * 8;
    hipStream_t st = (hipStream_t)stream;
    if (nitem <= 5 * WG)
        hipLaunchKernelGGL(top2_slab_kernel<5>, dim3(M), dim3(WG), 0, st, *logits, bias, V, unk_idx, word, word_stride, logprob, table, E,
                           emb_out, emb_ld);
    else if (nitem <= 8 * WG)
        hipLaunchKernelGGL(top2_slab_kernel<8>, dim3(M), dim3(WG), 0, st, *logits, bias, V, unk_idx, word, word_stride, logprob, table, E,
                           emb_out, emb_ld);
    else
        return CVC_E_TOOBIG;
    return cvc_launch_status();
}

extern "C" int cvc_nll_fwd(const float* logp, const int64_t* target, const float* w, int M, int V, float* loss_sum,
                           cvc_stream_t stream) {
    if (!logp || !target || !w || !loss_sum || M < 1 || V < 1) return CVC_E_BADARG;
    hipLaunchKernelGGL(nll_fwd_kernel, dim3(1), dim3(WG), 0, (hipStream_t)stream, logp, target, w, M, V, loss_sum);
    return cvc_launch_status();
}

extern "C" int cvc_vocab_nll_fwd(const float* logits, const int64_t* target, const float* w, int M, int V, float* lse,
                                 int64_t* argmax, float* row_loss, float* loss_sum, cvc_stream_t stream) {
    if (!logits || !target || !w || !lse || !row_loss || !loss_sum || M < 1 || V < 1) return CVC_E_BADARG;
    hipLaunchKernelGGL(vocab_nll_fwd_kernel, dim3(M), dim3(WG), 0, (hipStream_t)stream, logits, target, w, V, lse, argmax,
                       row_loss);
    hipLaunchKernelGGL(row_sum_kernel, dim3(1), dim3(WG), 0, (hipStream_t)stream, row_loss, M, loss_sum);
    return cvc_launch_status();
}

extern "C" int cvc_vocab_head_nll_fwd(const float* parts, int nparts, long long part_stride, int ld, const float* bias,
                                      const int64_t* target, const float* w, int M, int V, float* pre, int ld_pre, int64_t* argmax,
                                      float* row_loss, float* loss_sum, cvc_stream_t stream) {
    if (!parts || nparts < 1 || !target || !w || !pre || !row_loss || !loss_sum || M < 1 || V < 1 || V > WG * NLL_CACHE || ld < V ||
        ld_pre < V)
        return CVC_E_BADARG;
    hipLaunchKernelGGL(vocab_head_nll_kernel, dim3(M), dim3(WG), 0, (hipStream_t)stream, parts, nparts, part_stride, ld, bias, target, w, V,
                       pre, ld_pre, argmax, row_loss);
    hipLaunchKernelGGL(row_sum_kernel, dim3(1), dim3(WG), 0, (hipStream_t)stream, row_loss, M, loss_sum);
    return cvc_launch_status();
}

__global__ __launch_bounds__(WG) void stable_order_kernel(const int64_t* key, int n, int64_t* order) {
    extern __shared__ int64_t keys[];
    __shared__ int cnt[8][32];
    for (int j = threadIdx.x; j < n; j += WG) keys[j] = key[j];
    __syncthreads();
    const int il = threadIdx.x & 31, sg = threadIdx.x >> 5;
    const int i = blockIdx.x * 32 + il;
    const int per = (n + 7) / 8;
    const int j0 = sg * per, j1 = min(n, j0 + per);
    int r = 0;
    if (i < n) {
        const int64_t k = keys[i];
        const int m = min(max(i, j0), j1);
#pragma unroll 8
        for (int j = j0; j < m; ++j) r += keys[j] <= k ? 1 : 0;
#pragma unroll 8
        for (int j = max(m, i + 1); j < j1; ++j) r += keys[j] < k ? 1 : 0;
    }
    cnt[sg][il] = r;
    __syncthreads();
    if (sg == 0 && i < n) {
        int t = 0;
#pragma unroll
        for (int g = 0; g < 8; ++g) t += cnt[g][il];
        order[t] = i;
    }
}

__global__ __launch_bounds__(WG) void col_sum_kernel(const float* x, long long ld, int S, int rows_per_chunk, int n, float* out, long long ld_out,
                                                     float* out2) {
    __shared__ float part[4][64];
    const int lane = threadIdx.x & 63, wave = threadIdx.x >> 6;
    const int c = blockIdx.x * 64 + lane;
// ... 238 lines not shown
```

### cyclical-visual-captioning_amd/cvc/decode/engine.py

```python
from __future__ import annotations

import ctypes as C
import os
from typing import Dict, List, Optional, Tuple


import numpy as np
import torch

from .. import hip
from .weights import *
from .weights import _segs
from .path_packed import PackedPath
from .path_tile import TilePath
from .path_ring import RingPath
from .path_experimental import ExperimentalPaths

def _capture_mode() -> str:
    import torch.distributed as dist
    if dist.is_available() and dist.is_initialized() and dist.get_backend() == "nccl":
        return "thread_local"
    return "global"


class DecodeEngine(PackedPath, TilePath, RingPath, ExperimentalPaths):
    _warm = set()

    def __init__(self, weights: DecodeWeights, feats: Dict[str, torch.Tensor], T: int, unk_idx: int, beam: int = 1,
                 inv_temp: float = 1.0, own_features: bool = False, path: str = "auto", gate_ksplit: Optional[bool] = None,
                 driver: bool = True, gsk: Optional[bool] = None, embgate: Optional[bool] = None, lang_ksx: Optional[bool] = None,
                 sample_n: int = 1, temperature: Optional[float] = None, seed: Optional[int] = None, weights_dtype: str = "fp32"):
        W = self.W = weights
        self.T, self.unk, self.beam = int(T), int(unk_idx), int(beam)
        if weights_dtype not in WEIGHTS_DTYPES:
            raise RuntimeError(f"DecodeEngine: weights_dtype must be one of {WEIGHTS_DTYPES}, got {weights_dtype!r}")
        self.weights_dtype = weights_dtype
        self.bf16w = weights_dtype == "bf16"
        if self.bf16w:
            why = None
            if self.beam != 1:
                why = f"beam search (beam = {self.beam}) runs on the tile path"
            elif int(sample_n) != 1:
                why = f"sample_n = {sample_n} > 1 runs on the tile path"
            elif path in ("tile", "ring"):
                why = f'path="{path}" was asked for'
            elif gsk or gate_ksplit or lang_ksx:
                why = "gsk / gate_ksplit / lang_ksx are experimental schedules of the fp32 kernels"
            elif embgate is not None and not embgate:
                why = "embgate=False: the packed path without the embedding-gate schedule"
            if why is not None:
                raise RuntimeError(f'DecodeEngine: weights_dtype="bf16" covers the packed path with the embedding-gate schedule only '
                                   f"(beam = 1, one caption per clip, <= 64 rows); refused: {why}")
            gsk, gate_ksplit, lang_ksx = False, False, False
        self.sampling = temperature is not None
        if self.sampling:
            tau = float(temperature)
            if not (0.0 < tau < float("inf")):
                raise RuntimeError(f"DecodeEngine: the sampling temperature must be a positive finite number, got {temperature!r}")
            if self.beam != 1:
                raise RuntimeError("DecodeEngine: sampling (temperature) and beam search (beam > 1) exclude each other")
            if gsk or gate_ksplit or lang_ksx:
                raise RuntimeError("DecodeEngine: sampling runs on the default schedules only (no gsk / gate_ksplit / lang_ksx)")
            if int(sample_n) < 1:
                raise RuntimeError(f"DecodeEngine: sample_n must be >= 1, got {sample_n}")
            self.inv_tau = 1.0 / tau
            gate_ksplit, lang_ksx = False, False
        elif int(sample_n) != 1:
            raise RuntimeError("DecodeEngine: sample_n > 1 needs a sampling temperature")
        self.nq = int(sample_n) if self.sampling else self.beam
        fc, conv, pconv = feats["fc_feats"], feats["conv_feats"], feats["p_conv_feats"]
        pool, ppool = feats["pool_feats"], feats["p_pool_feats"]
        mask = feats["pnt_mask"][:, 1:] if feats["pnt_mask"].shape[1] == pool.shape[1] + 1 else feats["pnt_mask"]
        self.B, self.N, self.F = pool.shape[0], pool.shape[1], conv.shape[1]
        B, N, Fr, R, A, V = self.B, self.N, self.F, W.R, W.A, W.V
        dev = pool.device
        if self.bf16w and (B * self.nq > 64 or R % 32 or W.E % 32 or A % 32):
            raise RuntimeError(f'DecodeEngine: weights_dtype="bf16" covers the packed path only: at most 64 rows and R, E, A '
                               f"multiples of 32 (got {B * self.nq} rows, R = {R}, E = {W.E}, A = {A})")
        for name, t, shape in (("fc_feats", fc, (B, R)), ("conv_feats", conv, (B, Fr, R)), ("p_conv_feats", pconv, (B, Fr, A)),
                               ("pool_feats", pool, (B, N, R)), ("p_pool_feats", ppool, (B, N, A))):
            if tuple(t.shape) != shape:
                raise RuntimeError(f"DecodeEngine: {name} has shape {tuple(t.shape)}, expected {shape}")
            hip._dev(t, name=name)
        self.mask = hip._mask(mask)
        if own_features:
            fc, conv, pconv, pool, ppool = (t.clone() for t in (fc, conv, pconv, pool, ppool))
            self.mask = self.mask.clone()
        self.own_features = own_features
        self.feats = (fc, conv, pconv, pool, ppool)
        nb = lambda t: t.numel() * t.element_size()
        rows = self.rows = B * self.nq
        f32 = dict(device=dev, dtype=torch.float32)
        z = lambda *s: torch.zeros(*s, **f32)
        self.h_att, self.c_att = [z(rows, R), z(rows, R)], [z(rows, R), z(rows, R)]
        self.h_lang, self.c_lang = [z(rows, R), z(rows, R)], [z(rows, R), z(rows, R)]
        self.q = z(rows, A)
        self.scores_r, self.scores_f = z(rows, N), z(rows, Fr)
        self.attn_f = z(rows, Fr)
        self.ctx_sum = z(rows, R)
        self.logits = z(rows, V)
        self.gate_fc = z(rows, 4 * R)
        self.QSPLIT = 8
        self.q_parts = z(self.QSPLIT, rows, A)
        self.emb = z(rows, W.E)
        self.top2_part = z((V + 31) // 32, 64, 6)
        self.att_steps = z(self.T, rows, N)
        self.words = torch.zeros(self.T + 1, rows, dtype=torch.int64, device=dev)
        self.logprob = z(self.T, rows)
        self.fc = fc
        self.clip_of_row = torch.arange(rows, device=dev, dtype=torch.int64) // self.nq
        if self.sampling:
            self.rng = torch.zeros(4, device=dev, dtype=torch.int32)
            self.seed(0 if seed is None else seed)
        if self.beam > 1:
            self.score = z(2, rows)
            self.done = torch.zeros(2, rows, dtype=torch.uint8, device=dev)
            self.parent = torch.zeros(self.T, rows, dtype=torch.int64, device=dev)
            self.bt_seq = torch.zeros(self.B, self.T, dtype=torch.int64, device=dev)
            self.bt_att = z(self.B, self.T, N)
            self.gather_tmp = [z(rows, R) for _ in range(4)]
            self.beam_ws = z(17 * rows)
        self.inv_temp = float(inv_temp)
        self.graph: Optional[torch.cuda.CUDAGraph] = None
        self._keep: List = []
        self.packed = self.nq == 1 and rows <= 64 and path != "tile" and R % 32 == 0 and W.E % 32 == 0 and A % 32 == 0
        self.gate_ksplit = GATE_KSPLIT_DEFAULT if gate_ksplit is None else gate_ksplit
        self.gate_fused = self.gate_ksplit == "fused"
        self.gate_ksplit = bool(self.gate_ksplit)
        gsk_ok = self.packed and R % 64 == 0 and not self.gate_ksplit and hip.gemm_packed_split(-1) == 2
        if gsk and not gsk_ok:
            raise RuntimeError("DecodeEngine: the stream-K schedule needs the packed path, R % 64 == 0 and cvc_gemm_packed_split(2)")
        self.gsk = False if gsk is None else bool(gsk)
        self.tile = (not self.packed) and (self.nq > 1 or rows > 64 or path == "tile") and R % 16 == 0 and W.E % 16 == 0 and path != "ring"
        eg_ok = (self.packed and not self.gsk and not self.gate_ksplit) or self.tile
        if embgate and not eg_ok:
            raise RuntimeError("DecodeEngine: the embedding-gate schedule needs the packed path (without gsk / gate_ksplit) or the tile path")
        self.embgate = (eg_ok and 4 * V * 4 * R <= EMBGATE_MAX_BYTES) if embgate is None else bool(embgate)
        if self.sampling and self.packed and not self.embgate:
            raise RuntimeError("DecodeEngine: sampling on the packed path needs the embedding-gate schedule (the attention cell reads "
                               "the sampled word from words[t])")
        if self.bf16w and not (self.packed and self.embgate):
            raise RuntimeError('DecodeEngine: weights_dtype="bf16" needs the embedding-gate schedule, and its table '
                               f"({4 * V * 4 * R} bytes) is over EMBGATE_MAX_BYTES")
        bpw = 2 if self.bf16w else 4
        keep = cache_plan(bpw * (V * R + A * R), {"ppool": nb(ppool), "pconv": nb(pconv), "pool": nb(pool), "conv": nb(conv)},
                          gate_weight_bytes=bpw * 4 * R * 2 * R if (self.packed and self.embgate and (rows > 32 or self.bf16w)) else None,
                          lang_weight_bytes=bpw * 4 * R * 3 * R if self.bf16w else None)
        self.cache_keep = keep
        self.att_w_cached = bool(keep.get("att_w", False))
        self.lang_w_cached = bool(keep.get("lang_w", False))
        self.stream_r = (0 if keep["ppool"] else 1) | (0 if keep["pool"] else 2)
        self.stream_f = (0 if keep["pconv"] else 1) | (0 if keep["conv"] else 2)
        self._plan = None
        self._driver = driver
        exp = hip.experimental_built()
        if not exp and (self.gsk or self.gate_ksplit or lang_ksx):
            raise RuntimeError("DecodeEngine: gsk / gate_ksplit / lang_ksx are experimental schedules (include/cvc_hip_experimental.h): "
                               "this libcvc_hip.so was built without CVC_EXPERIMENTAL=1")
        ksx_ok = (exp and self.packed and not self.gsk and not self.gate_ksplit and R == 2048 and self.T > 1 and
                  hip.gemm_packed_split(-1) == 2 and int(hip.lib().cvc_packed_lstm_ks_slices(3 * R, R)) == 8)
        if lang_ksx and not ksx_ok:
            raise RuntimeError("DecodeEngine: lang_ksx needs the packed path at R = 2048, T > 1, split-product arithmetic")
        self.lang_ksx = ksx_ok and not self.bf16w and (LANG_KSX_DEFAULT if lang_ksx is None else bool(lang_ksx))
        self._ksx_checked = False
        if self.lang_ksx:
            self.ksx_slab = torch.empty(8 * (R // 8) * 2048, device=dev, dtype=torch.float32)
            self.ksx_flags = torch.zeros(R // 8 + 1, device=dev, dtype=torch.int32)
        if self.packed:
            self._alloc_packed()
        elif self.tile:
            self._alloc_tile()
        self._launches = self._build_launches()
        if driver and not self.sampling and not self.bf16w and (self.tile or (self.packed and not (self.ks_att or self.ks_lang))):
            self._bind_driver()


    def _bind_driver(self):
        W, L = self.W, hip.lib()
        ptr = lambda t: None if t is None else t.data_ptr()
        d = hip.DecodeDesc()
        d.B, d.beam, d.T, d.N, d.F, d.R, d.A, d.E, d.V = self.B, self.beam, self.T, self.N, self.F, W.R, W.A, W.E, W.V
        d.unk_idx, d.attn_kind, d.inv_temp = self.unk, W.kind, self.inv_temp
        d.stream_r, d.stream_f = self.stream_r, self.stream_f
        for k in ("b_ih_att", "b_hh_att", "b_ih_lang", "b_hh_lang", "b_h", "w_a", "b_a", "b_o", "embed"):
            setattr(d, k, ptr(getattr(W, k)))
        fc, conv, pconv, pool, ppool = self.feats
        d.fc, d.conv, d.pconv, d.pool, d.ppool, d.mask = ptr(fc), ptr(conv), ptr(pconv), ptr(pool), ptr(ppool), ptr(self.mask)
        d.words, d.att_steps, d.logprob = ptr(self.words), ptr(self.att_steps), ptr(self.logprob)
        d.scores_r, d.scores_f, d.attn_f = ptr(self.scores_r), ptr(self.scores_f), ptr(self.attn_f)
        if self.packed:
            R = W.R
            d.path, d.qsplit = 0, self.QSPLIT
            d.w_att, d.w_lang, d.w_h, d.w_o = ptr(W.p_att2 if self.embgate else W.p_att), ptr(W.p_lang), ptr(W.p_h), ptr(W.p_o)
            w_fc = W.w_ih_att[:, R:2 * R]
            d.w_fc, d.ld_w_fc = w_fc.data_ptr(), w_fc.stride(0)
            d.gate_fc, d.q_parts, d.top2_part = ptr(self.gate_fc), ptr(self.q_parts), ptr(self.top2_part)
            for name, bufs in (("xa", self.XA), ("xl", self.XL), ("ca", self.cA), ("cl", self.cL)):
                arr = getattr(d, name)
                arr[0], arr[1] = ptr(bufs[0]), ptr(bufs[1])
            d.xa0_init = ptr(self.XA0_init)
            if self.embgate:
                d.w_att = ptr(W.p_att2)
                d.emb_gate, d.sel_counter = ptr(W.t_embgate), ptr(self.sel_counter)
                d.att_w_cached = int(self.att_w_cached)
            if self.lang_ksx:
                d.lang_ksx, d.ksx_slab, d.ksx_flags = 1, ptr(self.ksx_slab), ptr(self.ksx_flags)
            if self.gsk:
                d.gsk_nwg = self.gsk_nwg
                d.slab_att, d.slab_lang, d.slab_q, d.slab_o = (ptr(self.slab_att), ptr(self.slab_lang), ptr(self.slab_q),
                                                              ptr(self.slab_o))
        else:
            d.path = 1
            d.ks_gate, d.ks_q, d.ks_o, d.ks_fc = self.ks_gate, self.ks_q, self.ks_o, self.ks_fc
            d.w_att, d.w_lang, d.w_h, d.w_o, d.w_fc_frag = ptr(W.t_att2 if self.embgate else W.t_att), ptr(W.t_lang), ptr(W.t_h), ptr(W.t_o), ptr(W.t_fc)
            if self.embgate:
                d.emb_gate = ptr(W.t_embgate)
            d.gate_fc, d.q, d.q_parts, d.logits = ptr(self.gate_fc_clip), ptr(self.q), ptr(self.parts_q), ptr(self.logits)
            for name, t in (("xaf", self.XAf), ("xlf", self.XLf), ("xhf", self.XHf), ("xff", self.XFf)):
                p_, s_ = hip._frag_ptr(t)
                setattr(d, name, p_)
                setattr(d, name + "_stride", s_)
            d.parts_gate, d.parts_o, d.parts_fc = ptr(self.parts_gate), ptr(self.parts_o), ptr(self.parts_fc)
            d.h_att, d.c_att, d.h_lang, d.c_lang = ptr(self.t_h_att), ptr(self.t_c_att), ptr(self.t_h_lang), ptr(self.t_c_lang)
            d.c_att_prev, d.c_lang_prev, d.zero_state = ptr(self.t_c_att_prev), ptr(self.t_c_lang_prev), ptr(self.t_zero)
            if self.beam > 1:
                d.score, d.done, d.parent, d.beam_ws = ptr(self.score), ptr(self.done), ptr(self.parent), ptr(self.beam_ws)
        plan = C.c_void_p()
        hip._check(L.cvc_decode_plan_create(C.byref(d), C.byref(plan)), "cvc_decode_plan_create")
        self._desc, self._plan = d, plan
        self._plan_call = L.cvc_decode_beam if self.beam > 1 else L.cvc_decode_greedy

    def __del__(self):
        plan = getattr(self, "_plan", None)
        if plan is not None and plan.value:
            try:
                hip.lib().cvc_decode_plan_destroy(plan)
            except Exception:
                pass
            self._plan = None

    def _run_driver(self):
        hip._check(self._plan_call(self._plan, torch.cuda.current_stream().cuda_stream), "cvc_decode_greedy/beam")


    def _reset(self):
        if self.tile:
            self.words[0].zero_()
            if self.beam > 1:
                self.score.zero_()
                self.done.zero_()
            return
        if self.packed:
            self.XA[0].copy_(self.XA0_init)
            self.XL[0].zero_()
            self.cA[0].zero_()
            self.cL[0].zero_()
            self.words[0].zero_()
            return
        for bufs in (self.h_att, self.c_att, self.h_lang, self.c_lang):
            bufs[0].zero_()
        self.words[0].zero_()
        if self.beam > 1:
            self.score.zero_()
            self.done.zero_()

    def _run_launches(self, timers=None):
        stream = torch.cuda.current_stream().cuda_stream
        for name, fn, args in self._python_launches():
            if timers is not None:
                e0, e1 = torch.cuda.Event(enable_timing=True), torch.cuda.Event(enable_timing=True)
                e0.record()
            if fn == "copy":
                args[0].copy_(args[1])
            else:
                rc = fn(*args, stream)
                if rc != 0:
# ... 132 lines not shown
```

### cyclical-visual-captioning_amd/cvc/decode/path_packed.py

```python
from __future__ import annotations

import ctypes as C
import os
from typing import Dict, List, Optional, Tuple

import torch

from .. import hip
from .weights import *
from .weights import _segs


class PackedPath:
    def _alloc_packed(self):
        W, R, E = self.W, self.W.R, self.W.E
        dev = self.fc.device
        if self.bf16w:
            bind_bf16(W)
        if not self.embgate and not hasattr(W, "p_att"):
            W.p_att = pack_weights(torch.cat([W.w_ih_att[:, 0:R], W.w_ih_att[:, 2 * R:2 * R + E], W.w_hh_att], 1), R)
        if not self.bf16w and not hasattr(W, "p_lang"):
            W.p_lang = pack_weights(torch.cat([W.w_ih_lang, W.w_hh_lang], 1), R)
            W.p_h = pack_weights(W.w_h)
            W.p_o = pack_weights(W.w_o)
        if self.embgate and not self.bf16w and not hasattr(W, "p_att2"):
            W.p_att2 = pack_weights(torch.cat([W.w_ih_att[:, 0:R], W.w_hh_att], 1), R)
            W.t_embgate = embgate_table(W)
        zq = lambda k: torch.zeros(k // 4, 64, 4, device=dev, dtype=torch.float32)
        ka = 2 * R if self.embgate else 2 * R + E
        self.XA, self.XL = [zq(ka), zq(ka)], [zq(3 * R), zq(3 * R)]
        self.sel_counter = torch.zeros(4, device=dev, dtype=torch.int32)
        self.cA, self.cL = [zq(R), zq(R)], [zq(R), zq(R)]
        bos = torch.relu(W.embed[0]).view(1, E).expand(self.rows, E).contiguous()
        self.XA0_init = zq(ka)
        if not self.embgate:
            self.XA0_init[R // 4:(R + E) // 4] = to_quad(bos)
        L = hip.lib()
        self.ks_att = int(L.cvc_packed_lstm_ks_slices(2 * R + E, R)) if self.gate_ksplit else 0
        self.ks_lang = int(L.cvc_packed_lstm_ks_slices(3 * R, R)) if self.gate_ksplit else 0
        self.ks_pad = KS_PAD_QUADS if (self.ks_att or self.ks_lang) else 0
        if self.ks_pad and not hasattr(W, "p_att_ks"):
            W.p_att_ks = pack_weights(torch.cat([W.w_ih_att[:, 0:R], W.w_ih_att[:, 2 * R:2 * R + E], W.w_hh_att], 1), R, self.ks_pad)
            W.p_lang_ks = pack_weights(torch.cat([W.w_ih_lang, W.w_hh_lang], 1), R, self.ks_pad)
        if self.ks_att or self.ks_lang:
            self.gate_slab = torch.empty(max(self.ks_att, self.ks_lang) * (R // 8) * 2048, device=dev, dtype=torch.float32)
            self.gate_counters = torch.zeros(R // 64, device=dev, dtype=torch.int32)
        if self.gsk:
            A, V = W.A, W.V
            self.gsk_nwg = int(torch.cuda.get_device_properties(dev).multi_processor_count)
            nt_r, nt_v, nt_a = R // 64, ((V + 31) // 32 + 7) // 8, (A // 32 + 7) // 8
            self.plan_a = hip.gsk_plan([nt_r, nt_v], [2 * R // 32, R // 32], self.gsk_nwg)
            self.plan_o = hip.gsk_plan([nt_v], [R // 32], self.gsk_nwg)
            self.plan_l = hip.gsk_plan([nt_r, nt_a], [2 * R // 32, R // 32], self.gsk_nwg)
            slab = lambda ntile, maxseg: torch.zeros(ntile * maxseg * 16384, device=dev, dtype=torch.float32)
            self.slab_att = slab(nt_r, self.plan_a["maxseg"][0])
            self.slab_o = slab(nt_v, max(self.plan_a["maxseg"][1], self.plan_o["maxseg"][0]))
            self.slab_lang = slab(nt_r, self.plan_l["maxseg"][0])
            self.slab_q = slab(nt_a, self.plan_l["maxseg"][1])

    def _build_packed(self):
        L, W = hip.lib(), self.W
        B, N, Fr, R, A, E, V, rows = self.B, self.N, self.F, W.R, W.A, W.E, W.V, self.rows
        fc, conv, pconv, pool, ppool = self.feats
        ptr = lambda t: None if t is None else t.data_ptr()
        qoff = lambda buf, k0: buf.data_ptr() + (k0 // 4) * 64 * 4 * 4
        out = []
        seg_fc = _segs([(fc, None, W.r_w_fc if self.bf16w else W.w_ih_att[:, R:2 * R], False)])
        out.append(("gate_fc", L.cvc_linear_fwd, (seg_fc, 1, ptr(W.b_ih_att), ptr(W.b_hh_att), rows, 4 * R, ptr(self.gate_fc),
                                                  4 * R)))
        self._keep.append(seg_fc)
        nblk_v = (V + 31) // 32
        if self.gsk:
            return out + self._build_gsk_steps()
        if self.embgate:
            return out + self._build_embgate_steps()
        for t in range(self.T):
            rd, wr = t & 1, (t + 1) & 1
            XA_r, XA_w, XL_r, XL_w = self.XA[rd], self.XA[wr], self.XL[rd], self.XL[wr]
            if self.ks_att and self.gate_fused:
                out.append(("att_lstm", L.cvc_packed_lstm_ksf_fwd, (ptr(W.p_att), ptr(XA_r), 2 * R + E, None, None, ptr(self.gate_fc),
                                                                    ptr(self.cA[rd]), rows, R, qoff(XL_r, R), qoff(XA_w, R + E),
                                                                    ptr(self.cA[wr]), ptr(self.gate_slab), ptr(self.gate_counters))))
            elif self.ks_att:
                wp_att = W.p_att_ks if self.ks_pad else W.p_att
                out.append(("att_lstm", L.cvc_packed_lstm_ks_fwd, (ptr(wp_att), ptr(XA_r), 2 * R + E, None, None, ptr(self.gate_fc),
                                                                   ptr(self.cA[rd]), rows, R, qoff(XL_r, R), qoff(XA_w, R + E),
                                                                   ptr(self.cA[wr]), ptr(self.gate_slab), wp_att.stride(0))))
            else:
                out.append(("att_lstm", L.cvc_packed_lstm_fwd, (ptr(W.p_att), ptr(XA_r), 2 * R + E, None, None, ptr(self.gate_fc),
                                                                ptr(self.cA[rd]), rows, R, qoff(XL_r, R), qoff(XA_w, R + E),
                                                                ptr(self.cA[wr]))))
            out.append(("h2attn", L.cvc_packed_linear_fwd, (ptr(W.p_h), qoff(XL_r, R), R, None, rows, A, self.QSPLIT,
                                                            ptr(self.q_parts), A, None)))
            sets = (hip.AttnSet * 2)()
            sets[0] = hip.AttnSet(ptr(ppool), ptr(pool), ptr(self.mask), None, ptr(self.scores_r), None,
                                  ptr(self.att_steps[t]), None, N, self.stream_r)
            sets[1] = hip.AttnSet(ptr(pconv), ptr(conv), None, None, ptr(self.scores_f), None, ptr(self.attn_f), None, Fr,
                                  self.stream_f)
            out.append(("attn_scores", L.cvc_attn_scores_qparts, (W.kind, ptr(self.q_parts), self.QSPLIT, ptr(W.b_h), ptr(W.w_a),
                                                                  ptr(W.b_a), self.inv_temp, sets, 2, B, 1, A)))
            out.append(("attn_wsum", L.cvc_attn_wsum_quad, (sets, 2, B, 1, R, ptr(XL_r))))
            if self.ks_lang and self.gate_fused:
                out.append(("lang_lstm", L.cvc_packed_lstm_ksf_fwd, (ptr(W.p_lang), ptr(XL_r), 3 * R, ptr(W.b_ih_lang),
                                                                     ptr(W.b_hh_lang), None, ptr(self.cL[rd]), rows, R, ptr(XA_w),
                                                                     qoff(XL_w, 2 * R), ptr(self.cL[wr]), ptr(self.gate_slab),
                                                                     ptr(self.gate_counters))))
            elif self.ks_lang:
                wp_lang = W.p_lang_ks if self.ks_pad else W.p_lang
                out.append(("lang_lstm", L.cvc_packed_lstm_ks_fwd, (ptr(wp_lang), ptr(XL_r), 3 * R, ptr(W.b_ih_lang),
                                                                    ptr(W.b_hh_lang), None, ptr(self.cL[rd]), rows, R, ptr(XA_w),
                                                                    qoff(XL_w, 2 * R), ptr(self.cL[wr]), ptr(self.gate_slab),
                                                                    wp_lang.stride(0))))
            elif self.lang_ksx:
                out.append(self._lang_ksx_launch(t, XL_r, XA_w, XL_w, rd, wr))
            else:
                out.append(("lang_lstm", L.cvc_packed_lstm_fwd, (ptr(W.p_lang), ptr(XL_r), 3 * R, ptr(W.b_ih_lang), ptr(W.b_hh_lang),
                                                                 None, ptr(self.cL[rd]), rows, R, ptr(XA_w), qoff(XL_w, 2 * R),
                                                                 ptr(self.cL[wr]))))
            out.append(("logits", L.cvc_packed_linear_fwd, (ptr(W.p_o), ptr(XA_w), R, ptr(W.b_o), rows, V, 1, None, V,
                                                            ptr(self.top2_part))))
            out.append(("word_select", L.cvc_top2_final, (ptr(self.top2_part), nblk_v, rows, self.unk, ptr(self.words[t + 1]), 1,
                                                          ptr(self.logprob[t]), ptr(W.embed), E, qoff(XA_w, R), 0)))
            self._keep.append(sets)
        return out

    def _build_embgate_steps(self):
        L, W = hip.lib(), self.W
        B, N, Fr, R, A, V, rows = self.B, self.N, self.F, W.R, W.A, W.V, self.rows
        fc, conv, pconv, pool, ppool = self.feats
        ptr = lambda t: None if t is None else t.data_ptr()
        qoff = lambda buf, k0: buf.data_ptr() + (k0 // 4) * 64 * 4 * 4
        out = []
        nblk_v = (V + 31) // 32
        if self.bf16w:
            att_fn, linear_fn = L.cvc_packed_lstm_bf16w_fwd, L.cvc_packed_linear_bf16w_fwd
            w_att, att_stride, embgate, w_h, w_o = W.pb_att2, 2 * R * 32, W.r_embgate, W.pb_h, W.pb_o
        else:
            att_fn, linear_fn = L.cvc_packed_lstm_embgate_ex_fwd, L.cvc_packed_linear_fwd
            w_att, att_stride, embgate, w_h, w_o = W.p_att2, (2 * R // 4) * 128, W.t_embgate, W.p_h, W.p_o
        for t in range(self.T):
            rd, wr = t & 1, (t + 1) & 1
            XA_r, XA_w, XL_r, XL_w = self.XA[rd], self.XA[wr], self.XL[rd], self.XL[wr]
            first = t == 0 and (self.bf16w or hip.gemm_packed_split(-1) == 2)
            out.append(("att_lstm", att_fn, (ptr(w_att), att_stride, ptr(XA_r), 32 if first else 2 * R, None, None,
                                             ptr(self.gate_fc), ptr(embgate), ptr(self.words[t]), ptr(self.cA[rd]),
                                             rows, R, qoff(XL_r, R), qoff(XA_w, R), ptr(self.cA[wr]),
                                             1 if self.att_w_cached else 0)))
            out.append(("h2attn", linear_fn, (ptr(w_h), qoff(XL_r, R), R, None, rows, A, self.QSPLIT, ptr(self.q_parts), A, None)))
            sets = (hip.AttnSet * 2)()
            sets[0] = hip.AttnSet(ptr(ppool), ptr(pool), ptr(self.mask), None, ptr(self.scores_r), None,
                                  ptr(self.att_steps[t]), None, N, self.stream_r)
            sets[1] = hip.AttnSet(ptr(pconv), ptr(conv), None, None, ptr(self.scores_f), None, ptr(self.attn_f), None, Fr,
                                  self.stream_f)
            out.append(("attn_scores", L.cvc_attn_scores_qparts, (W.kind, ptr(self.q_parts), self.QSPLIT, ptr(W.b_h), ptr(W.w_a),
                                                                  ptr(W.b_a), self.inv_temp, sets, 2, B, 1, A)))
            out.append(("attn_wsum", L.cvc_attn_wsum_quad, (sets, 2, B, 1, R, ptr(XL_r))))
            if self.bf16w:
                out.append(("lang_lstm", L.cvc_packed_lstm_bf16w_fwd, (ptr(W.pb_lang), 3 * R * 32, ptr(XL_r), 2 * R if first else 3 * R,
                                                                       ptr(W.b_ih_lang), ptr(W.b_hh_lang), None, None, None, ptr(self.cL[rd]),
                                                                       rows, R, ptr(XA_w), qoff(XL_w, 2 * R), ptr(self.cL[wr]),
                                                                       1 if self.lang_w_cached else 0)))
            elif first:
                out.append(("lang_lstm", L.cvc_packed_lstm_late_fwd, (ptr(W.p_lang), (3 * R // 4) * 128, ptr(XL_r), 2 * R, ptr(W.b_ih_lang),
                                                                      ptr(W.b_hh_lang), None, ptr(self.cL[rd]), rows, R, ptr(XA_w),
                                                                      qoff(XL_w, 2 * R), ptr(self.cL[wr]), None)))
            elif self.lang_ksx:
                out.append(self._lang_ksx_launch(t, XL_r, XA_w, XL_w, rd, wr))
            else:
                out.append(("lang_lstm", L.cvc_packed_lstm_fwd, (ptr(W.p_lang), ptr(XL_r), 3 * R, ptr(W.b_ih_lang), ptr(W.b_hh_lang),
                                                                 None, ptr(self.cL[rd]), rows, R, ptr(XA_w), qoff(XL_w, 2 * R),
                                                                 ptr(self.cL[wr]))))
            if self.sampling:
                out.append(("logits", linear_fn, (ptr(w_o), ptr(XA_w), R, ptr(W.b_o), rows, V, 1, ptr(self.logits), V, None)))
                out.append(("word_select", L.cvc_sample_select_parts, (ptr(self.logits), 1, 0, None, rows, V, self.unk, self.inv_tau,
                                                                       ptr(self.rng), t, ptr(self.words[t + 1]), 1,
                                                                       ptr(self.logprob[t]))))
            else:
                out.append(("logits", linear_fn, (ptr(w_o), ptr(XA_w), R, ptr(W.b_o), rows, V, 1, None, V, ptr(self.top2_part))))
                out.append(("word_select", L.cvc_top2_final, (ptr(self.top2_part), nblk_v, rows, self.unk, ptr(self.words[t + 1]), 1,
                                                              ptr(self.logprob[t]), None, 0, None, 0)))
            self._keep.append(sets)
        return out
```

### cyclical-visual-captioning_amd/cvc/decode/weights.py

```python
from __future__ import annotations

import ctypes as C
import os
from typing import Dict, List, Optional

import torch

from .. import hip


class DecodeWeights:

    def __init__(self, sd: Dict[str, torch.Tensor], softattn_type: str = "additive"):
        g = lambda k: sd[k].detach().contiguous()
        self.w_ih_att, self.w_hh_att = g("decoder_core.att_lstm.weight_ih"), g("decoder_core.att_lstm.weight_hh")
        self.b_ih_att, self.b_hh_att = g("decoder_core.att_lstm.bias_ih"), g("decoder_core.att_lstm.bias_hh")
        self.w_ih_lang, self.w_hh_lang = g("decoder_core.lang_lstm.weight_ih"), g("decoder_core.lang_lstm.weight_hh")
        self.b_ih_lang, self.b_hh_lang = g("decoder_core.lang_lstm.bias_ih"), g("decoder_core.lang_lstm.bias_hh")
        self.w_h, self.b_h = g("decoder_core.soft_attn.h2attn.weight"), g("decoder_core.soft_attn.h2attn.bias")
        self.kind = hip.ATTN_ADDITIVE if softattn_type == "additive" else hip.ATTN_DOT
        if self.kind == hip.ATTN_ADDITIVE:
            self.w_a = g("decoder_core.soft_attn.alpha_net.weight").reshape(-1)
            self.b_a = g("decoder_core.soft_attn.alpha_net.bias")
        else:
            self.w_a = self.b_a = None
        self.embed = g("embed.0.weight")
        self.w_o, self.b_o = g("logit.weight"), g("logit.bias")
        self.R = self.w_hh_att.shape[1]
        self.A = self.w_h.shape[0]
        self.E = self.embed.shape[1]
        self.V = self.w_o.shape[0]
        for t in vars(self).values():
            if isinstance(t, torch.Tensor) and (not t.is_cuda or t.dtype != torch.float32):
                raise RuntimeError("DecodeWeights: parameters must be fp32 tensors on the GPU (no CPU fallback)")


def _segs(items):
    arr = (hip.GemmSeg * len(items))()
    for i, (x, idx, w, relu) in enumerate(items):
        arr[i] = hip.GemmSeg(x.data_ptr(), None if idx is None else idx.data_ptr(), w.data_ptr(), w.shape[1], x.stride(0),
                             w.stride(0), 1 if relu else 0)
    return arr


def pack_weights(w: torch.Tensor, lstm_R: Optional[int] = None, pad_quads: int = 0) -> torch.Tensor:
    n, k = w.shape
    assert k % 32 == 0, k
    if lstm_R is not None:
        R = lstm_R
        assert n == 4 * R and R % 8 == 0
        i = torch.arange(32, device=w.device)
        rows = ((i >> 3) * R + (i & 7)).view(1, 32) + (torch.arange(R // 8, device=w.device) * 8).view(-1, 1)
        w = w[rows.reshape(-1)]
        nb = R // 8
    else:
        nb = (n + 31) // 32
        if nb * 32 != n:
            w = torch.cat([w, w.new_zeros(nb * 32 - n, k)], 0)
    out = w.view(nb, 32, k // 4, 4).permute(0, 2, 1, 3)
    if pad_quads:
        padded = w.new_zeros(nb, k // 4 + pad_quads, 32, 4)
        padded[:, :k // 4] = out
        return padded
    return out.contiguous()


def lstm_packed_rows(R: int, device) -> torch.Tensor:
    i = torch.arange(32, device=device)
    return (((i >> 3) * R + (i & 7)).view(1, 32) + (torch.arange(R // 8, device=device) * 8).view(-1, 1)).reshape(-1)


WEIGHTS_DTYPES = ("fp32", "bf16")
BF16_ROUNDED_KEYS = ("decoder_core.att_lstm.weight_ih", "decoder_core.att_lstm.weight_hh", "decoder_core.lang_lstm.weight_ih",
                     "decoder_core.lang_lstm.weight_hh", "decoder_core.soft_attn.h2attn.weight", "logit.weight")


def bf16_round(t: torch.Tensor) -> torch.Tensor:
    if t.dtype != torch.float32:
        raise RuntimeError(f"bf16_round: fp32 in, fp32 out (got {t.dtype})")
    u = t.contiguous().view(torch.int32)
    r = ((u + (((u >> 16) & 1) + 0x7FFF)) & -65536).view(torch.float32)
    return torch.where(torch.isnan(t), t, r)


def pack_weights_bf16(w: torch.Tensor, lstm_R: Optional[int] = None) -> torch.Tensor:
    n, k = w.shape
    assert k % 32 == 0, k
    if lstm_R is not None:
        assert n == 4 * lstm_R and lstm_R % 8 == 0
        w = w[lstm_packed_rows(lstm_R, w.device)]
        nb = lstm_R // 8
    else:
        nb = (n + 31) // 32
        if nb * 32 != n:
            w = torch.cat([w, w.new_zeros(nb * 32 - n, k)], 0)
    return bf16_round(w).to(torch.bfloat16).view(nb, 32, k // 8, 8).permute(0, 2, 1, 3).contiguous()


def unpack_weights_bf16(p: torch.Tensor, n: Optional[int] = None, lstm_R: Optional[int] = None) -> torch.Tensor:
    nb, k8 = p.shape[0], p.shape[1]
    w = p.permute(0, 2, 1, 3).reshape(nb * 32, k8 * 8).float()
    if lstm_R is not None:
        out = torch.empty_like(w)
        out[lstm_packed_rows(lstm_R, w.device)] = w
        w = out
    return w if n is None else w[:n]


def bind_bf16(W: "DecodeWeights") -> "DecodeWeights":
    if hasattr(W, "pb_lang"):
        return W
    R, E = W.R, W.E
    W.pb_att2 = pack_weights_bf16(torch.cat([W.w_ih_att[:, 0:R], W.w_hh_att], 1), R)
    W.pb_h = pack_weights_bf16(W.w_h)
    W.pb_o = pack_weights_bf16(W.w_o)
    W.r_w_fc = bf16_round(W.w_ih_att[:, R:2 * R])
    W.r_embgate = hip.tile_mm(torch.relu(W.embed), bf16_round(W.w_ih_att[:, 2 * R:2 * R + E]))
    W.pb_lang = pack_weights_bf16(torch.cat([W.w_ih_lang, W.w_hh_lang], 1), R)
    return W


EMBGATE_MAX_BYTES = 1 << 30


def embgate_table(W: "DecodeWeights") -> torch.Tensor:
    R, E = W.R, W.E
    return hip.tile_mm(torch.relu(W.embed), W.w_ih_att[:, 2 * R:2 * R + E])


def to_quad(x: torch.Tensor) -> torch.Tensor:
    m, k = x.shape
    out = x.new_zeros(k // 4, 64, 4)
    out[:, :m] = x.view(m, k // 4, 4).permute(1, 0, 2)
    return out


def from_quad(xq: torch.Tensor, m: int) -> torch.Tensor:
    return xq[:, :m].permute(1, 0, 2).reshape(m, -1)


def split3_bf16(x: torch.Tensor):
    def top(v):
        return (v.view(torch.int32) & -65536).view(torch.float32)
    hi = top(x)
    r1 = x - hi
    mid = top(r1)
    lo = top(r1 - mid)
    bits = lambda v: (v.view(torch.int32) >> 16).to(torch.int16)
    return bits(hi), bits(mid), bits(lo)


def to_frag(x: torch.Tensor, rows_alloc: Optional[int] = None) -> torch.Tensor:
    m, k = x.shape
    assert k % 16 == 0, k
    ra = rows_alloc if rows_alloc is not None else (m + 31) // 32 * 32
    xp = x.new_zeros(ra, k)
    xp[:m] = x
    planes = torch.stack(split3_bf16(xp.contiguous()), 0)
    return planes.view(3, ra // 32, 32, k // 16, 2, 8).permute(1, 3, 0, 4, 2, 5).contiguous()


def from_frag(xb: torch.Tensor, m: int) -> torch.Tensor:
    nb, ks = xb.shape[0], xb.shape[1]
    f = (xb.to(torch.int32) << 16).view(torch.float32)
    x = f.sum(2).permute(0, 3, 1, 2, 4).reshape(nb * 32, ks * 16)
    return x[:m]


def pack_weights_tile(w: torch.Tensor, lstm_R: Optional[int] = None) -> torch.Tensor:
    n, k = w.shape
    assert k % 16 == 0, k
    if lstm_R is not None:
        R = lstm_R
        assert n == 4 * R and R % 8 == 0
        i = torch.arange(32, device=w.device)
        rows = ((i >> 3) * R + (i & 7)).view(1, 32) + (torch.arange(R // 8, device=w.device) * 8).view(-1, 1)
        w = w[rows.reshape(-1)]
    return to_frag(w, (n + 127) // 128 * 128)


GATE_KSPLIT_DEFAULT = False
KS_PAD_QUADS = 0

CACHE_BUDGET = int(os.environ.get("CVC_CACHE_BUDGET_MB", "208")) << 20
LANG_KSX_DEFAULT = os.environ.get("CVC_LANG_KSX", "0") == "1"
CACHE_LANG_GATE_WEIGHTS = os.environ.get("CVC_LANG_W_CACHED", "1") != "0"
CACHE_GATE_WEIGHTS = os.environ.get("CVC_ATT_W_CACHED", "1") != "0"


def cache_plan(linear_weight_bytes: int, feature_bytes: Dict[str, int], budget: int = CACHE_BUDGET,
               gate_weight_bytes: Optional[int] = None, lang_weight_bytes: Optional[int] = None) -> Dict[str, bool]:
    names = list(feature_bytes)
    room = budget - linear_weight_bytes
    plan = {}
    if gate_weight_bytes is not None:
        plan["att_w"] = bool(CACHE_GATE_WEIGHTS and 0 < gate_weight_bytes <= room)
        if plan["att_w"]:
            room -= gate_weight_bytes
# ... 13 lines not shown
```

### cyclical-visual-captioning_amd/cvc/hip.py

```python
from __future__ import annotations

import ctypes as C
import functools
import os
from typing import List, Optional, Sequence

import torch

_HERE = os.path.dirname(os.path.abspath(__file__))
LIB_PATH = os.environ.get("CVC_LIB") or os.path.join(_HERE, "lib", "libcvc_hip.so")

ATTN_ADDITIVE, ATTN_DOT = 0, 1


class AttnSet(C.Structure):
    _fields_ = [("proj", C.c_void_p), ("ctx", C.c_void_p), ("mask", C.c_void_p), ("frame_mask", C.c_void_p),
                ("scores", C.c_void_p), ("frame_masked", C.c_void_p), ("attn", C.c_void_p), ("ctx_out", C.c_void_p),
                ("n", C.c_int), ("stream", C.c_int)]


class GemmSeg(C.Structure):
    _fields_ = [("x", C.c_void_p), ("idx", C.c_void_p), ("w", C.c_void_p),
                ("k", C.c_int), ("ldx", C.c_int), ("ldw", C.c_int), ("relu", C.c_int)]

# ... 112 lines not shown
    "cvc_train_loop_profile_read": [C.POINTER(_I), C.POINTER(_I), C.POINTER(_F), _I],
    "cvc_attn_fwd": [_I, _P, _P, _P, _F, C.POINTER(AttnSet), _I, _I, _I, _I, _I, _P, _P],
    "cvc_attn_scores": [_I, _P, _P, _P, _F, C.POINTER(AttnSet), _I, _I, _I, _I, _P],
    "cvc_attn_scores_qparts": [_I, _P, _I, _P, _P, _P, _F, C.POINTER(AttnSet), _I, _I, _I, _I, _P],
    "cvc_linear_splitk_fwd": [C.POINTER(GemmSeg), _I, _P, _I, _I, _I, _P, _P],
    "cvc_linear_top2_fwd": [C.POINTER(GemmSeg), _I, _P, _I, _I, _P, _P, _P],
    "cvc_top2_final": [_P, _I, _I, _I, _P, _I, _P, _P, _I, _P, _I, _P],
    "cvc_attn_wsum_quad": [C.POINTER(AttnSet), _I, _I, _I, _I, _P, _P],
    "cvc_packed_lstm_fwd": [_P, _P, _I, _P, _P, _P, _P, _I, _I, _P, _P, _P, _P],
    "cvc_packed_linear_fwd": [_P, _P, _I, _P, _I, _I, _I, _P, _I, _P, _P],
    "cvc_packed_lstm_wg_blocks": [_I],
    "cvc_packed_lstm_embgate_fwd": [_P, _P, _I, _P, _P, _P, _P, _P, _P, _I, _I, _P, _P, _P, _P],
    "cvc_packed_lstm_embgate_ex_fwd": [_P, _LL, _P, _I, _P, _P, _P, _P, _P, _P, _I, _I, _P, _P, _P, _I, _P],
    "cvc_packed_linear_select_fwd": [_P, _P, _I, _P, _I, _I, _P, _P, _I, _P, _I, _P, _P],
    "cvc_gsk_plan": [C.POINTER(_I), C.POINTER(_I), _I, _I, C.POINTER(_I), C.POINTER(_I), C.POINTER(_I)],
    "cvc_gsk_gemm": [C.POINTER(GskGroup), _I, _I, _P],
    "cvc_packed_lstm_late_fwd": [_P, _LL, _P, _I, _P, _P, _P, _P, _I, _I, _P, _P, _P, C.POINTER(GskSegs), _P],
    "cvc_attn_scores_qslab": [_I, C.POINTER(GskSegs), _P, _P, _P, _F, C.POINTER(AttnSet), _I, _I, _I, _I, _P],
    "cvc_top2_slab": [C.POINTER(GskSegs), _P, _I, _I, _I, _P, _I, _P, _P, _I, _P, _I, _P],
    "cvc_packed_lstm_train_fwd": [_P, _P, _I, _P, _P, _P, _I, _I, _P, _P, _P, _P, _P, _P],
    "cvc_pack_lstm_weights": [_P, _I, _P, _I, _I, _P, _P],
    "cvc_pack_lstm_segs": [C.POINTER(_P), C.POINTER(_LL), C.POINTER(_I), _I, _I, _P, _P],
    "cvc_packed_lstm_train_pre_fwd": [_P, _P, _I, _P, _P, _P, _P, _I, _I, _P, _P, _P, _P, _P, _P],
    "cvc_pack_quad_segs": [C.POINTER(_P), C.POINTER(_LL), C.POINTER(_I), _I, _I, _P, _P],
    "cvc_beam_backtrack": [_P, _P, _P, _I, _I, _I, _I, _P, _P, _P],
    "cvc_gru_seq_fwd": [_P, _P, _LL, _LL, _P, _P, _I, _I, _I, _I, _P, _P, _LL, _LL, _P],
    "cvc_gru_seq_train_fwd": [_P, _P, _LL, _LL, _P, _P, _I, _I, _I, _I, _P, _P, _LL, _LL, _P, _LL, _LL, _P],
    "cvc_lstm_pointwise_bwd4_pair": [C.POINTER(PwBwdArgs), C.POINTER(PwBwdArgs), _I, _P],
    "cvc_gru_persistent_halves": [_I],
    "cvc_gru_persistent_waves8": [_I],
    "cvc_gru_persistent_sync_words": [],
    "cvc_gru_seq_persistent_train_fwd": [_P, _P, _LL, _LL, _P, _P, _I, _I, _I, _I, _P, _P, _LL, _LL, _P, _LL, _LL, _P, _P],
    "cvc_gru_seq_bwd_ksplit": [_I],
    "cvc_gru_bwd_persistent_sync_words": [],
    "cvc_gru_seq_bwd_persistent": [_P, _LL, _LL, _P, _LL, _LL, _P, _LL, _LL, _P, _I, _I, _I, _I, _P, _P, _P, _P, _P],
    "cvc_linear_nn_planes_fwd": [_P, _I, _I, C.POINTER(NNSeg), _I, _I, _P, _P],
    "cvc_linear_nn_planes2_fwd": [_P, _P, _I, _I, _I, C.POINTER(NNSeg), _I, _I, _P, _I, _P],
    "cvc_gru_seq_bwd": [_P, _LL, _LL, _P, _LL, _LL, _P, _LL, _LL, _P, _I, _I, _I, _I, _P, _P, _P, _P],
    "cvc_gru_seq_persistent_fwd": [_P, _P, _LL, _LL, _P, _P, _I, _I, _I, _I, _P, _P, _LL, _LL, _P, _P],
    "cvc_lstm_persistent_sync_words": [],
    "cvc_lstm_seq_persistent_fwd": [_P, _P, _LL, _LL, _P, _P, _I, _I, _I, _I, _P, _P, _LL, _LL, _P, _P],
    "cvc_lstm_seq_persistent_train_fwd": [_P, _P, _LL, _LL, _P, _P, _I, _I, _I, _I, _P, _P, _LL, _LL, _P, _LL, _LL, _P, _LL, _LL, _P, _P],
    "cvc_lstm_seq_fwd": [_P, _P, _LL, _LL, _P, _P, _I, _I, _I, _I, _P, _P, _LL, _LL, _P],
    "cvc_lstm_seq_train_fwd": [_P, _P, _LL, _LL, _P, _P, _I, _I, _I, _I, _P, _P, _LL, _LL, _P, _LL, _LL, _P, _LL, _LL, _P],
    "cvc_lstm_seq_bwd_work": [_I, _I, _I],
    "cvc_lstm_seq_bwd": [_P, _LL, _LL, _P, _LL, _LL, _P, _LL, _LL, _P, _I, _I, _I, _I, _P, _P, _P],
    "cvc_packed_lstm_ks_slices": [_I, _I],
    "cvc_packed_lstm_ks_fwd": [_P, _P, _I, _P, _P, _P, _P, _I, _I, _P, _P, _P, _P, _LL, _P],
    "cvc_packed_lstm_ksf_fwd": [_P, _P, _I, _P, _P, _P, _P, _I, _I, _P, _P, _P, _P, _P, _P],
    "cvc_packed_lstm_ksx_local": [_I],
    "cvc_packed_lstm_ksx_fwd": [_P, _P, _I, _P, _P, _P, _P, _P, _P, _I, _I, _P, _P, _P, _P, _P, C.c_uint, _P],
    "cvc_attn_wsum": [C.POINTER(AttnSet), _I, _I, _I, _I, _P, _P],
    "cvc_attn_bwd": [_I, _P, _P, _F, _P, _P, _P, _P, _P, _I, _I, _I, _I, _I, _P, _P, _P, _P, _P, _P],
    "cvc_linear_fwd": [C.POINTER(GemmSeg), _I, _P, _P, _I, _I, _P, _I, _P],
    "cvc_gemm_force_generic": [_I],
    "cvc_gemm_packed_split": [_I],
    "cvc_lstm_cell_fwd": [C.POINTER(GemmSeg), _I, _P, _P, _P, _P, _I, _I, _P, _P, _P, _P],
    "cvc_lstm_pointwise_bwd": [_P, _P, _P, _P, _P, _I, _I, _P, _P, _P, _P],
    "cvc_lstm_pointwise_bwd3": [_P, _P, _P, _P, _P, _P, _P, _I, _I, _P, _P, _P, _P],
    "cvc_linear_nn_fwd": [_P, _I, _I, C.POINTER(NNSeg), _I, _I, _P, _P],
    "cvc_pack_quad": [_P, _LL, _I, _I, _P, _P],
    "cvc_embed_relu_fwd": [_P, _P, _P, _I, _I, _P, _P],
    "cvc_embed_relu_bwd": [_P, _P, _P, _P, _P, _I, _I, _P, _P, _P],
    "cvc_embed_relu_rng_fwd": [_P, _P, _P, C.c_uint, _F, _I, _I, _P, _P],
    "cvc_embed_relu_rng_bwd": [_P, _P, _P, _P, C.c_uint, _F, _P, _I, _I, _P, _P, _P],
    "cvc_dropout_rng": [_P, _LL, _P, C.c_uint, _F, _P, _P],
    "cvc_packed_lstm_train_drop_fwd": [_P, _P, _I, _P, _P, _P, _P, _I, _I, _P, _P, _P, _P, _P, _P, C.c_uint, _F, _P],
    "cvc_lstm_pointwise_bwd3_drop": [_P, _P, _P, _P, C.c_uint, _F, _P, _P, _P, _P, _I, _I, _P, _P, _P, _P],
    "cvc_log_softmax_fwd": [_P, _I, _I, _P, _P],
    "cvc_log_softmax_bwd": [_P, _P, _I, _I, _P, _P],
    "cvc_nll_bwd": [_P, _P, _P, _I, _I, _P, _P],
    "cvc_top2_unk": [_P, _I, _I, _I, _P, _I, _P, _P],
    "cvc_nll_fwd": [_P, _P, _P, _I, _I, _P, _P],
    "cvc_vocab_nll_fwd": [_P, _P, _P, _I, _I, _P, _P, _P, _P, _P],
    "cvc_vocab_nll_bwd": [_P, _P, _P, _P, _P, _I, _I, _P, _P],
    "cvc_grounder_fwd": [_P, _P, _P, _P, _I, _I, _I, _I, _P, _P],
    "cvc_grounder_bwd": [_P, _P, _P, _I, _I, _I, _I, _P, _P, _P],
    "cvc_beam_select": [_P, _P, _P, _I, _I, _I, _I, _I, _P, _P, _P, _P, _P, _P],
    "cvc_beam_select_parts": [_P, _I, _LL, _P, _P, _P, _I, _I, _I, _I, _I, _P, _P, _P, _P, _P, _P],
    "cvc_sample_select_parts": [_P, _I, _LL, _P, _I, _I, _I, _F, _P, _I, _P, _I, _P, _P],
    "cvc_sample_advance": [_P, _P],
    "cvc_packed_lstm_bf16w_fwd": [_P, _LL, _P, _I, _P, _P, _P, _P, _P, _P, _I, _I, _P, _P, _P, _I, _P],
    "cvc_packed_linear_bf16w_fwd": [_P, _P, _I, _P, _I, _I, _I, _P, _I, _P, _P],
    "cvc_gather_rows": [_P, _P, _I, _I, _I, _P, _P],
    "cvc_tile_rows_alloc": [_I],
    "cvc_tile_gemm_loaders": [_I],
    "cvc_tile_gemm": [_P, _P, _LL, _I, _I, _I, _I, _P, _I, _LL, _P],
    "cvc_tile_lstm_finish": [_P, _I, _LL, _P, _P, _P, _I, _P, _I, _I, _P, _P, _P, _LL, _P, _LL, _P],
    "cvc_tile_lstm_finish_embgate": [_P, _I, _LL, _P, _P, _P, _I, _P, _P, _I, _P, _I, _I, _P, _P, _P, _LL, _P, _LL, _P],
    "cvc_tile_linear_finish": [_P, _I, _LL, _I, _P, _P, _I, _I, _P, _I, _P],
    "cvc_tile_pack_rows": [_P, _I, _P, _I, _I, _I, _P, _LL, _P],
    "cvc_tile_pack_rows_any": [_P, _LL, _I, _I, _P, _LL, _P],
    "cvc_tile_pack_cols": [_P, _LL, _I, _I, _P, _LL, _P],
    "cvc_tile_reorder_pack": [_P, _P, _I, _P, _P, _P, _P, _P, _I, _I, _P, _P, _P, _LL, _P, _LL, _I, _I, _P],
    "cvc_attn_wsum_frag": [C.POINTER(AttnSet), _I, _I, _I, _I, _P, _LL, _P],
    "cvc_class_softmax_fwd": [_P, _LL, _P, _P, _I, _I, _I, _P, _P, _P],
    "cvc_layernorm_cat_fwd": [C.POINTER(_P), C.POINTER(_LL), C.POINTER(_I), _I, _LL, _F, _P, _LL, _P],
    "cvc_frame_embed_fwd": [_P, _P, _I, _P, _P, _I, _P, _P, _LL, _P, _P],
    "cvc_decode_plan_create": [C.POINTER(DecodeDesc), C.POINTER(C.c_void_p)],
    "cvc_decode_plan_destroy": [_P],
    "cvc_decode_plan_set_features": [_P, _P, _P, _P, _P, _P, _P],
    "cvc_decode_num_launches": [_P],
    "cvc_decode_greedy": [_P, _P],
    "cvc_decode_beam": [_P, _P],
    "cvc_optim_chunk_elems": [],
    "cvc_adam_clip_step": [_P, _I, _P, _I, _F, _F, _F, _F, _F, _I, _P, _P, _P, _P],
    "cvc_comm_unique_id": [_P],
    "cvc_comm_init": [_I, _I, _P, C.POINTER(C.c_void_p)],
    "cvc_allreduce_grads": [_P, _P, _LL, _P],
    "cvc_comm_destroy": [_P],
}
_VOID_RETURN = {"cvc_decode_plan_destroy"}
BLOCKS = {
    "cvc_attn_scores", "cvc_attn_wsum", "cvc_attn_scores_qparts", "cvc_attn_wsum_quad", "cvc_attn_wsum_frag", "cvc_attn_wsum_quad_rm",
    "cvc_attn_bwd_pair", "cvc_ctxfeat_bwd_steps", "cvc_dproj_bwd_steps", "cvc_tile_gemm_big", "cvc_tile_gemm_plan", "cvc_linear_splitk_fwd", "cvc_linear_top2_fwd", "cvc_top2_final", "cvc_packed_lstm_fwd", "cvc_packed_linear_fwd",
    "cvc_packed_lstm_embgate_fwd", "cvc_packed_lstm_embgate_ex_fwd", "cvc_packed_lstm_late_fwd", "cvc_packed_lstm_train_fwd",
    "cvc_packed_lstm_train_pre_fwd", "cvc_packed_lstm_train_drop_fwd", "cvc_lstm_pointwise_bwd", "cvc_lstm_pointwise_bwd3",
    "cvc_lstm_pointwise_bwd3_drop", "cvc_pack_lstm_weights", "cvc_linear_nn_planes_fwd", "cvc_linear_nn_planes2_fwd", "cvc_gru_seq_train_fwd", "cvc_lstm_pointwise_bwd4_pair", "cvc_beam_select_parts", "cvc_sample_select_parts", "cvc_sample_advance", "cvc_tile_lstm_finish",
    "cvc_tile_lstm_finish_embgate", "cvc_tile_reorder_pack", "cvc_decode_num_launches", "cvc_gemm_force_generic",
    "cvc_tile_gemm_loaders", "cvc_gru_persistent_waves8", "cvc_relu_dropout_fwd", "cvc_relu_dropout_bwd", "cvc_bn_workspace",
    "cvc_bn_relu_train_fwd", "cvc_bn_relu_train_bwd", "cvc_class_softmax_bwd", "cvc_layernorm_cat_bwd", "cvc_stable_order", "cvc_col_sum", "cvc_col_sum_ws", "cvc_attn_weighted_rows",
    "cvc_lstm_persistent_sync_words", "cvc_lstm_seq_persistent_fwd", "cvc_lstm_seq_persistent_train_fwd", "cvc_lstm_seq_fwd", "cvc_lstm_seq_train_fwd", "cvc_lstm_seq_bwd_work", "cvc_lstm_seq_bwd",
    "cvc_packed_lstm_bf16w_fwd", "cvc_packed_linear_bf16w_fwd"}
EXPERIMENTAL = {
    "cvc_gsk_plan", "cvc_gsk_gemm", "cvc_attn_scores_qslab", "cvc_top2_slab", "cvc_packed_lstm_ks_slices", "cvc_packed_lstm_ks_fwd",
    "cvc_packed_lstm_ksf_fwd", "cvc_packed_lstm_ksx_local", "cvc_packed_lstm_ksx_fwd", "cvc_packed_lstm_wg_blocks",
    "cvc_packed_linear_select_fwd", "cvc_gru_persistent_halves"}

_lib = None


def _missing(name):
    def fn(*_a, **_k):
        raise RuntimeError(f"{name} is an experimental form (include/cvc_hip_experimental.h): this libcvc_hip.so was built without "
                           "CVC_EXPERIMENTAL=1 (`CVC_EXPERIMENTAL=1 python cyclical-visual-captioning_amd/build_hip.py --force`)")
    return fn


def lib() -> C.CDLL:
    global _lib
    if _lib is None:
        if not os.path.exists(LIB_PATH):
            raise RuntimeError(
                f"{LIB_PATH} is missing: build it with `python cyclical-visual-captioning_amd/build_hip.py` "
                "(hipcc --offload-arch=gfx950).  There is no CPU fallback for the caption-decode hot path.")
        l = C.CDLL(LIB_PATH)
        l.cvc_block.restype = C.c_void_p
        l.cvc_block.argtypes = [C.c_char_p]
        for name, argtypes in SIGNATURES.items():
            restype = None if name in _VOID_RETURN else (C.c_longlong if name in ("cvc_train_loop_bwd_ws", "cvc_bn_workspace", "cvc_col_sum_ws") else C.c_int)
            if name in BLOCKS or name in EXPERIMENTAL:
                addr = l.cvc_block(name.encode())
                if not addr:
                    if name in BLOCKS:
                        raise RuntimeError(f"{LIB_PATH}: building block {name} is not in the library's table (stale build?)")
                    setattr(l, name, _missing(name))
                    continue
                setattr(l, name, C.CFUNCTYPE(restype, *argtypes)(addr))
                continue
            fn = getattr(l, name)
            fn.argtypes = argtypes
            fn.restype = restype
        l.cvc_version.restype = C.c_char_p
        l.cvc_version.argtypes = []
        _lib = l
    return _lib


def experimental_built() -> bool:
    return b"+experimental" in lib().cvc_version()


def version() -> str:
    return lib().cvc_version().decode()


_weights_generation = 0


def weights_generation() -> int:
    return _weights_generation


_warned = set()


def warn_once(key: str, msg: str):
    if key not in _warned:
        _warned.add(key)
        import warnings
        warnings.warn("cvc: " + msg, RuntimeWarning, stacklevel=3)


def bump_weights_generation() -> int:
    global _weights_generation
    _weights_generation += 1
    return _weights_generation


_step_status: dict = {}
_deferred_status = None


def step_status(device) -> torch.Tensor:
    dev = torch.device(device)
    key = dev.index if dev.index is not None else torch.cuda.current_device()
# ... 749 lines not shown
```

### include/cvc_hip_blocks.h

```cpp
#ifndef CVC_HIP_BLOCKS_H
#define CVC_HIP_BLOCKS_H
#include "cvc_hip.h"
#ifdef __cplusplus
extern "C" {
#endif

int cvc_attn_scores(int kind, const float* q, const float* w_a, const float* b_a, float inv_temp,
                    const cvc_attn_set* sets, int nsets, int nclip, int nq, int A, cvc_stream_t stream);
int cvc_attn_wsum(const cvc_attn_set* sets, int nsets, int nclip, int nq, int R, float* ctx_sum,
                  cvc_stream_t stream);
int cvc_attn_scores_qparts(int kind, const float* q_parts, int q_nparts, const float* q_bias, const float* w_a,
                           const float* b_a, float inv_temp, const cvc_attn_set* sets, int nsets, int nclip,
                           int nq, int A, cvc_stream_t stream);
int cvc_attn_wsum_quad(const cvc_attn_set* sets, int nsets, int nclip, int nq, int R, float* ctx_sum_q,
                       cvc_stream_t stream);
int cvc_attn_wsum_frag(const cvc_attn_set* sets, int nsets, int nclip, int nq, int R, void* ctx_frag,
                       long long frag_mblk_stride, cvc_stream_t stream);
int cvc_attn_wsum_quad_rm(const cvc_attn_set* sets, int nsets, int nclip, int R, float* ctx_sum_q, float* ctx_sum_rm,
                          cvc_stream_t stream);
int cvc_attn_bwd_pair(int kind, const cvc_grad_src* q, const float* q_bias, const float* w_a, float inv_temp,
                      const cvc_attn_set* sets, int nsets, const cvc_grad_src* d_ctx, int nclip, int nq, int A, int R,
                      float* d_q, float* d_q_q, float* d_w_part, float* const* d_proj, float* const* d_ctxfeat,
                      cvc_stream_t stream);
int cvc_ctxfeat_bwd_steps(const float* attn, const float* d_ctx_all, int T, int B, int n, int R, float* d_feat, cvc_stream_t stream);
// ... 58 lines not shown
    unsigned site;
    float p;
    const float *d_c, *gates, *c_prev, *c_new;
    int M;
    float *d_gates, *d_c_prev, *d_gates_q, *dg_sum;
    int q_row0;
} cvc_pw_bwd_args;
int cvc_lstm_pointwise_bwd4_pair(const cvc_pw_bwd_args* a, const cvc_pw_bwd_args* b, int R, cvc_stream_t stream);
int cvc_linear_nn_planes2_fwd(const float* dy_q, const float* dy_q2, int K, int M, int M2, const cvc_nn_seg* segs, int nsegs,
                              int ksplit, float* workspace, int reduce, cvc_stream_t stream);
int cvc_beam_select_parts(const float* parts, int nparts, long long part_stride, const float* bias,
                          const float* score_in, const uint8_t* done_in, int B, int beam, int V, int unk_idx,
                          int first_step, int64_t* parent, int64_t* word, float* score_out, uint8_t* done_out,
                          float* workspace, cvc_stream_t stream);
#define CVC_SAMPLE_SITE 0x53000000u
int cvc_sample_select_parts(const float* parts, int nparts, long long part_stride, const float* bias, int M, int V, int unk_idx,
                            float inv_tau, const uint32_t* rng_state, int t, int64_t* word, int word_stride, float* logprob,
                            cvc_stream_t stream);
int cvc_sample_advance(uint32_t* rng_state, cvc_stream_t stream);
int cvc_tile_lstm_finish(const float* parts, int nparts, long long part_stride, const float* b_ih, const float* b_hh,
                         const float* gate_bias, int gb_div, const float* c_prev, int M, int R, float* c_out,
                         float* h_out, void* frag1, long long frag1_stride, void* frag2, long long frag2_stride,
                         cvc_stream_t stream);
int cvc_tile_lstm_finish_embgate(const float* parts, int nparts, long long part_stride, const float* b_ih, const float* b_hh,
                                 const float* gate_bias, int gb_div, const float* emb_gate, const int64_t* word, int V,
                                 const float* c_prev, int M, int R, float* c_out, float* h_out, void* frag1,
                                 long long frag1_stride, void* frag2, long long frag2_stride, cvc_stream_t stream);
int cvc_tile_reorder_pack(const int64_t* parent, const int64_t* word, int beam, const float* h_att, const float* c_att,
                          const float* h_lang, const float* c_lang, const float* table, int E, int V,
                          float* c_att_prev, float* c_lang_prev, void* xa, long long xa_stride, void* xl_hlang,
                          long long xl_stride, int rows, int R, cvc_stream_t stream);
int cvc_decode_num_launches(const cvc_decode_plan* plan);
int cvc_gemm_force_generic(int on);
int cvc_tile_gemm_loaders(int on);
int cvc_gru_persistent_waves8(int on);
int cvc_relu_dropout_fwd(const float* x, const float* bias, long long rows, int N, const uint32_t* rng_state, unsigned site,
                         float p, float* y, cvc_stream_t stream);
int cvc_relu_dropout_bwd(const float* dy, const float* y, long long n, const uint32_t* rng_state, unsigned site, float p, float* dx,
                         cvc_stream_t stream);
long long cvc_bn_workspace(long long rows, int C);
int cvc_bn_relu_train_fwd(const float* x, const float* gamma, const float* beta, float eps, float momentum, float* running_mean,
                          float* running_var, long long rows, int C, float* y, float* save_mean, float* save_invstd,
                          float* workspace, cvc_stream_t stream);
int cvc_bn_relu_train_bwd(const float* x, const float* dy, const float* y, const float* gamma, const float* save_mean,
                          const float* save_invstd, long long rows, int C, float* dx, float* dgamma, float* dbeta,
                          float* workspace, cvc_stream_t stream);
int cvc_class_softmax_bwd(const float* p_rows, const float* d_rows, const float* d_sim, const uint8_t* pad, int B, int N, int C,
                          float* d_logits, cvc_stream_t stream);
int cvc_layernorm_cat_bwd(const float* const* xs, const long long* ldx, const int* widths, int nseg, long long rows, float eps,
                          const float* d_out, long long ld_out, float* const* dxs, const long long* lddx, cvc_stream_t stream);

int cvc_attn_weighted_rows(const float* w, const float* X, int nclip, int nq, int n, int R, float scale, float* out, cvc_stream_t stream);

int cvc_stable_order(const int64_t* key, int n, int64_t* order, cvc_stream_t stream);
long long cvc_col_sum_ws(int S, int n);
int cvc_col_sum(const float* x, long long ld, int S, int n, float* out, float* out2, float* ws, cvc_stream_t stream);

int cvc_lstm_persistent_sync_words(void);
int cvc_lstm_seq_persistent_fwd(const float* wp, const float* gi, long long gi_ld_m, long long gi_ld_t, const float* b_ih,
                                const float* b_hh, int M, int F, int H, int ndir, float* hq, float* y, long long y_ld_m,
                                long long y_ld_t, unsigned* sync, cvc_stream_t stream);
int cvc_lstm_seq_persistent_train_fwd(const float* wp, const float* gi, long long gi_ld_m, long long gi_ld_t, const float* b_ih,
                                      const float* b_hh, int M, int F, int H, int ndir, float* hq, float* y, long long y_ld_m,
                                      long long y_ld_t, float* gates, long long g_ld_m, long long g_ld_t, float* c, long long c_ld_m,
                                      long long c_ld_t, unsigned* sync, cvc_stream_t stream);
int cvc_lstm_seq_fwd(const float* wp, const float* gi, long long gi_ld_m, long long gi_ld_t, const float* b_ih, const float* b_hh,
                     int M, int F, int H, int ndir, float* hq, float* y, long long y_ld_m, long long y_ld_t, cvc_stream_t stream);
int cvc_lstm_seq_train_fwd(const float* wp, const float* gi, long long gi_ld_m, long long gi_ld_t, const float* b_ih,
                           const float* b_hh, int M, int F, int H, int ndir, float* hq, float* y, long long y_ld_m, long long y_ld_t,
                           float* gates, long long g_ld_m, long long g_ld_t, float* c, long long c_ld_m, long long c_ld_t,
                           cvc_stream_t stream);
int cvc_lstm_seq_bwd_work(int M, int H, int ndir);
int cvc_lstm_seq_bwd(const float* dy, long long dy_ld_m, long long dy_ld_t, const float* gates, long long g_ld_m, long long g_ld_t,
                     const float* c, long long c_ld_m, long long c_ld_t, const float* w_hh, int M, int F, int H, int ndir, float* dg,
                     float* work, cvc_stream_t stream);

int cvc_packed_lstm_bf16w_fwd(const uint16_t* wp, long long w_blk_stride, const float* xq, int K, const float* b_ih,
                              const float* b_hh, const float* gate_bias, const float* emb_gate, const int64_t* word,
                              const float* c_prev_q, int M, int R, float* h_dst1_q, float* h_dst2_q, float* c_out_q,
                              int w_cached, cvc_stream_t stream);
int cvc_packed_linear_bf16w_fwd(const uint16_t* wp, const float* xq, int K, const float* bias, int M, int Nout, int ksplit,
                                float* y, int ldy, float* top2_part, cvc_stream_t stream);

#ifdef __cplusplus
}
#endif
#endif
```

Baseline: 332,300 decode-steps/s.

## Use variable rows-per-block vocab head with row-major top2 partials and batched resets

The vocabulary output projection now packs weights with a chosen number of rows per block (up to 32) instead of a fixed 32. This lets the V=5000 head launch more, smaller blocks across the GPU, and the top-2 partial records are laid out per lane for a new final reduction kernel. The five per-decode reset launches are also merged into one multi-segment kernel. The cost is more top2 partial records to reduce and possibly lower per-block weight reuse, plus new packing paths in the weight setup.

```diff
diff --git a/cyclical-visual-captioning_amd/csrc/blocks.hip b/cyclical-visual-captioning_amd/csrc/blocks.hip
--- a/cyclical-visual-captioning_amd/csrc/blocks.hip
+++ b/cyclical-visual-captioning_amd/csrc/blocks.hip
@@ -65,6 +65,10 @@
     CVC_B(cvc_lstm_seq_bwd),
     CVC_B(cvc_packed_lstm_bf16w_fwd),
     CVC_B(cvc_packed_linear_bf16w_fwd),
+    CVC_B(cvc_packed_linear_block_rows),
+    CVC_B(cvc_packed_linear_rows_fwd),
+    CVC_B(cvc_packed_linear_rows_bf16w_fwd),
+    CVC_B(cvc_top2_final_rows),
 #ifdef CVC_EXPERIMENTAL
     CVC_B(cvc_gsk_plan),
     CVC_B(cvc_gsk_gemm),
diff --git a/cyclical-visual-captioning_amd/csrc/decode_driver.hip b/cyclical-visual-captioning_amd/csrc/decode_driver.hip
--- a/cyclical-visual-captioning_amd/csrc/decode_driver.hip
+++ b/cyclical-visual-captioning_amd/csrc/decode_driver.hip
@@ -42,6 +42,37 @@
     return hip_rc(hipGetLastError());
 }
 
+constexpr int RESET_MAX = 6;
+struct ResetSeg { uint4* dst; const uint4* src; unsigned n16, blk0; };
+struct ResetTable { ResetSeg s[RESET_MAX]; int n; };
+__global__ __launch_bounds__(256) void reset_segs_kernel(ResetTable t) {
+    const unsigned b = blockIdx.x;
+    ResetSeg g = t.s[0];
+#pragma unroll
+    for (int k = 1; k < RESET_MAX; ++k)
+        if (k < t.n && b >= t.s[k].blk0) g = t.s[k];
+    const size_t i = (size_t)(b - g.blk0) * 256 + threadIdx.x;
+    if (i < g.n16) g.dst[i] = g.src != nullptr ? g.src[i] : uint4{0, 0, 0, 0};
+}
+struct ResetBatch {
+    ResetTable t{};
+    unsigned blocks = 0;
+    int add(void* dst, const void* src, size_t bytes, hipStream_t st) {
+        if ((bytes & 15) || ((uintptr_t)dst & 15) || ((uintptr_t)src & 15) || t.n == RESET_MAX || bytes / 16 > 0x7fffffffu)
+            return reset(dst, src, bytes, st);
+        if (bytes == 0) return 0;
+        const unsigned n16 = (unsigned)(bytes / 16);
+        t.s[t.n++] = ResetSeg{(uint4*)dst, (const uint4*)src, n16, blocks};
+        blocks += (n16 + 255) / 256;
+        return 0;
+    }
+    int flush(hipStream_t st) {
+        if (t.n == 0) return 0;
+        hipLaunchKernelGGL(reset_segs_kernel, dim3(blocks), dim3(256), 0, st, t);
+        return hip_rc(hipGetLastError());
+    }
+};
+
 void attn_sets(const cvc_decode_desc& d, int t, int rows, cvc_attn_set* sets) {
     sets[0] = cvc_attn_set{d.ppool, d.pool, d.mask, nullptr, d.scores_r, nullptr, d.att_steps + (size_t)t * rows * d.N, nullptr,
                            d.N, d.stream_r};
@@ -53,14 +84,19 @@
     const int rows = d.B, R = d.R, E = d.E, A = d.A, V = d.V, N = d.N;
     const size_t qbytes = (size_t)64 * 4 * sizeof(float);
     int n = 0;
-    CVC_TRY(reset(d.xa[0], d.xa0_init, (size_t)((2 * R + E) / 4) * qbytes, st));
-    CVC_TRY(reset(d.xl[0], nullptr, (size_t)(3 * R / 4) * qbytes, st));
-    CVC_TRY(reset(d.ca[0], nullptr, (size_t)(R / 4) * qbytes, st));
-    CVC_TRY(reset(d.cl[0], nullptr, (size_t)(R / 4) * qbytes, st));
-    CVC_TRY(reset(d.words, nullptr, (size_t)rows * sizeof(int64_t), st));
+    ResetBatch rs;
+    int rrc = rs.add(d.xa[0], d.xa0_init, (size_t)((2 * R + E) / 4) * qbytes, st);
+    if (rrc == 0) rrc = rs.add(d.xl[0], nullptr, (size_t)(3 * R / 4) * qbytes, st);
+    if (rrc == 0) rrc = rs.add(d.ca[0], nullptr, (size_t)(R / 4) * qbytes, st);
+    if (rrc == 0) rrc = rs.add(d.cl[0], nullptr, (size_t)(R / 4) * qbytes, st);
+    if (rrc == 0) rrc = rs.add(d.words, nullptr, (size_t)rows * sizeof(int64_t), st);
+    if (rrc != 0) return rrc;
+    CVC_TRY(rs.flush(st));
     cvc_gemm_seg seg{d.fc, nullptr, d.w_fc, R, R, d.ld_w_fc, 0};
     CVC_TRY(cvc_linear_fwd(&seg, 1, d.b_ih_att, d.b_hh_att, rows, 4 * R, d.gate_fc, 4 * R, st));
-    const int nblk_v = (V + 31) / 32;
+    const int rb_v = cvc_packed_linear_block_rows(V);
+    if (rb_v < 1) return CVC_E_BADARG;
+    const int nblk_v = (V + rb_v - 1) / rb_v;
     for (int t = 0; t < d.T; ++t) {
         const int rd = t & 1, wr = (t + 1) & 1;
         float *XA_r = d.xa[rd], *XA_w = d.xa[wr], *XL_r = d.xl[rd], *XL_w = d.xl[wr];
@@ -79,9 +115,9 @@
 #endif
         CVC_TRY(cvc_packed_lstm_fwd((const float*)d.w_lang, XL_r, 3 * R, d.b_ih_lang, d.b_hh_lang, nullptr, d.cl[rd], rows, R, XA_w,
                                     quad_off(XL_w, 2 * R), d.cl[wr], st));
-        CVC_TRY(cvc_packed_linear_fwd((const float*)d.w_o, XA_w, R, d.b_o, rows, V, 1, nullptr, V, d.top2_part, st));
-        CVC_TRY(cvc_top2_final(d.top2_part, nblk_v, rows, d.unk_idx, d.words + (size_t)(t + 1) * rows, 1,
-                               d.logprob ? d.logprob + (size_t)t * rows : nullptr, d.embed, E, quad_off(XA_w, R), 0, st));
+        CVC_TRY(cvc_packed_linear_rows_fwd((const float*)d.w_o, XA_w, R, d.b_o, rows, V, rb_v, nullptr, V, d.top2_part, st));
+        CVC_TRY(cvc_top2_final_rows(d.top2_part, nblk_v, rows, d.unk_idx, d.words + (size_t)(t + 1) * rows, 1,
+                                    d.logprob ? d.logprob + (size_t)t * rows : nullptr, d.embed, E, quad_off(XA_w, R), 0, st));
     }
     p->launches = n;
     return 0;
@@ -92,13 +128,19 @@
     const int rows = d.B, R = d.R, A = d.A, V = d.V;
     const size_t qbytes = (size_t)64 * 4 * sizeof(float);
     int n = 0;
-    CVC_TRY(reset(d.xa[0], nullptr, (size_t)(2 * R / 4) * qbytes, st));
-    CVC_TRY(reset(d.xl[0], nullptr, (size_t)(3 * R / 4) * qbytes, st));
-    CVC_TRY(reset(d.ca[0], nullptr, (size_t)(R / 4) * qbytes, st));
-    CVC_TRY(reset(d.cl[0], nullptr, (size_t)(R / 4) * qbytes, st));
-    CVC_TRY(reset(d.words, nullptr, (size_t)rows * sizeof(int64_t), st));
+    ResetBatch rs;
+    int rrc = rs.add(d.xa[0], nullptr, (size_t)(2 * R / 4) * qbytes, st);
+    if (rrc == 0) rrc = rs.add(d.xl[0], nullptr, (size_t)(3 * R / 4) * qbytes, st);
+    if (rrc == 0) rrc = rs.add(d.ca[0], nullptr, (size_t)(R / 4) * qbytes, st);
+    if (rrc == 0) rrc = rs.add(d.cl[0], nullptr, (size_t)(R / 4) * qbytes, st);
+    if (rrc == 0) rrc = rs.add(d.words, nullptr, (size_t)rows * sizeof(int64_t), st);
+    if (rrc != 0) return rrc;
+    CVC_TRY(rs.flush(st));
     cvc_gemm_seg seg{d.fc, nullptr, d.w_fc, R, R, d.ld_w_fc, 0};
     CVC_TRY(cvc_linear_fwd(&seg, 1, d.b_ih_att, d.b_hh_att, rows, 4 * R, d.gate_fc, 4 * R, st));
+    const int rb_v = cvc_packed_linear_block_rows(V);
+    if (rb_v < 1) return CVC_E_BADARG;
+    const int nblk_v = (V + rb_v - 1) / rb_v;
     const long long ws_att = (long long)(2 * R / 4) * 128, ws_lang = (long long)(3 * R / 4) * 128;
     const bool split2 = cvc_gemm_packed_split(-1) == 2;
     for (int t = 0; t < d.T; ++t) {
@@ -124,9 +166,9 @@
         else
         CVC_TRY(cvc_packed_lstm_fwd((const float*)d.w_lang, XL_r, 3 * R, d.b_ih_lang, d.b_hh_lang, nullptr, d.cl[rd], rows, R, XA_w,
                                     quad_off(XL_w, 2 * R), d.cl[wr], st));
-        CVC_TRY(cvc_packed_linear_fwd((const float*)d.w_o, XA_w, R, d.b_o, rows, V, 1, nullptr, V, d.top2_part, st));
-        CVC_TRY(cvc_top2_final(d.top2_part, (V + 31) / 32, rows, d.unk_idx, d.words + (size_t)(t + 1) * rows, 1,
-                               d.logprob ? d.logprob + (size_t)t * rows : nullptr, nullptr, 0, nullptr, 0, st));
+        CVC_TRY(cvc_packed_linear_rows_fwd((const float*)d.w_o, XA_w, R, d.b_o, rows, V, rb_v, nullptr, V, d.top2_part, st));
+        CVC_TRY(cvc_top2_final_rows(d.top2_part, nblk_v, rows, d.unk_idx, d.words + (size_t)(t + 1) * rows, 1,
+                                    d.logprob ? d.logprob + (size_t)t * rows : nullptr, nullptr, 0, nullptr, 0, st));
     }
     p->launches = n;
     return 0;
diff --git a/cyclical-visual-captioning_amd/csrc/gemm_packed.hip b/cyclical-visual-captioning_amd/csrc/gemm_packed.hip
--- a/cyclical-visual-captioning_amd/csrc/gemm_packed.hip
+++ b/cyclical-visual-captioning_amd/csrc/gemm_packed.hip
@@ -2,6 +2,7 @@
 #include "gemm_split.h"
 #include "gsk.h"
 #include "dropout_rng.h"
+#include "word_select.h"
 
 struct PackedArgs {
     const float* wp;
@@ -41,6 +42,7 @@
     int w_cached;
     DropSpec h3_drop;
     long long wstride;
+    int rb;
     GskSegs early;
 };
 
@@ -82,22 +84,10 @@
     return v;
 }
 
-struct SelState { float t1, t2, gm, gs; int j1, j2; };
-__device__ __forceinline__ SelState sel_init() { return SelState{-__builtin_inff(), -__builtin_inff(), -__builtin_inff(), 0.f, 0x7fffffff, 0x7fffffff}; }
-__device__ __forceinline__ bool sel_better(float va, int ia, float vb, int ib) { return (va > vb) | ((va == vb) & (ia < ib)); }
-__device__ __forceinline__ SelState sel_merge(SelState s, float u1, int k1, float u2, int k2, float um, float us) {
-    if (sel_better(u1, k1, s.t1, s.j1)) {
-        if (sel_better(s.t1, s.j1, u2, k2)) { s.t2 = s.t1; s.j2 = s.j1; } else { s.t2 = u2; s.j2 = k2; }
-        s.t1 = u1; s.j1 = k1;
-    } else if (sel_better(u1, k1, s.t2, s.j2)) { s.t2 = u1; s.j2 = k1; }
-    const float nm = fmaxf(s.gm, um);
-    s.gs = (nm == -__builtin_inff()) ? 0.f : s.gs * __expf(s.gm - nm) + us * __expf(um - nm);
-    s.gm = nm;
-    return s;
-}
-
-template <int MT, bool LSTM, int DEPTH, bool SPLIT, int NW, bool GRU = false, int NB = 1, bool SLAB = false, bool WC = false, bool WB16 = false>
+template <int MT, bool LSTM, int DEPTH, bool SPLIT, int NW, bool GRU = false, int NB = 1, bool SLAB = false, bool WC = false, bool WB16 = false,
+          bool VRB = false>
 __global__ __launch_bounds__(NW * 64) void skinny_gemm_packed_kernel(PackedArgs a) {
+    static_assert(!VRB || (!LSTM && NB == 1 && !SLAB), "variable block rows: linear form only");
     static_assert(!WB16 || (SPLIT && NW == 8 && !GRU && NB == 1 && !SLAB), "bf16-stored weights: 8-wave split-product form only");
     using Frag = std::conditional_t<WB16, BFrag<MT>, PFrag<MT>>;
     using WT = std::conditional_t<WB16, uint16_t, float>;
@@ -119,6 +109,9 @@
     const int wave = __builtin_amdgcn_readfirstlane(tid >> 6);
     const int i = lane & 31, kh = lane >> 5;
     const int M = a.M, R = a.R;
+    const int RB = VRB ? a.rb : 32;
+    const int QW = RB * 4;
+    const int iw = VRB ? (i < RB ? i : RB - 1) : i;
 #ifdef CVC_TS
     unsigned long long ts_[4] = {0, 0, 0, 0};
 #endif
@@ -132,10 +125,11 @@
     }
     const int wblk = NB == 1 ? 0 : wave / NWK, kw = NB == 1 ? wave : wave % NWK;
     const int n_my = nchunk > kw ? (nchunk - kw + NWK - 1) / NWK : 0;
-    const WT* wl = reinterpret_cast<const WT*>(a.wp) + (size_t)((int)blockIdx.x * NB + wblk) * a.wstride + (size_t)i * (WB16 ? 8 : 4) +
-                   (size_t)(c0 + kw) * 8 * 128 + kh * 4 * 128;
+    const WT* wl = reinterpret_cast<const WT*>(a.wp) + (size_t)((int)blockIdx.x * NB + wblk) * a.wstride + (size_t)iw * (WB16 ? 8 : 4) +
+                   (size_t)(c0 + kw) * 8 * QW + kh * 4 * QW;
     const float* xl = a.xq + (size_t)i * 4 + (size_t)(c0 + kw) * 8 * 256 + kh * 4 * 256;
-    constexpr size_t WSTEP = (size_t)NWK * 8 * 128, XSTEP = (size_t)NWK * 8 * 256;
+    const size_t WSTEP = (size_t)NWK * 8 * QW;
+    constexpr size_t XSTEP = (size_t)NWK * 8 * 256;
 #ifndef CVC_ROT_MUL
 #define CVC_ROT_MUL 5
 #endif
@@ -156,8 +150,8 @@
         if constexpr (WB16) {
 #pragma unroll
             for (int s2 = 0; s2 < 2; ++s2) {
-                if constexpr (LSTM && !WC) f.w[s2] = __builtin_nontemporal_load(reinterpret_cast<const u32x4*>(w + s2 * 256));
-                else f.w[s2] = *reinterpret_cast<const u32x4*>(w + s2 * 256);
+                if constexpr (LSTM && !WC) f.w[s2] = __builtin_nontemporal_load(reinterpret_cast<const u32x4*>(w + s2 * 2 * QW));
+                else f.w[s2] = *reinterpret_cast<const u32x4*>(w + s2 * 2 * QW);
 #pragma unroll
                 for (int q = 2 * s2; q < 2 * s2 + 2; ++q)
 #pragma unroll
@@ -166,8 +160,8 @@
         } else {
 #pragma unroll
             for (int q = 0; q < 4; ++q) {
-                if constexpr (((LSTM && !GRU) || CVC_LIN_W_NT) && !WC) f.w[q] = __builtin_nontemporal_load(reinterpret_cast<const f32x4*>(w + q * 128));
-                else f.w[q] = ld4(w + q * 128);
+                if constexpr (((LSTM && !GRU) || CVC_LIN_W_NT) && !WC) f.w[q] = __builtin_nontemporal_load(reinterpret_cast<const f32x4*>(w + q * QW));
+                else f.w[q] = ld4(w + q * QW);
 #if defined(CVC_PABL) && CVC_PABL == 3
                 if (j > 0) continue;
 #endif
@@ -373,7 +367,7 @@
     float ebias[ECPW];
 #pragma unroll
     for (int c = 0; c < ECPW; ++c) {
-        const int n = (int)blockIdx.x * 32 + wave * ECPW + c;
+        const int n = (int)blockIdx.x * RB + wave * ECPW + c;
         ebias[c] = (!LSTM && a.top2_part != nullptr && a.bias != nullptr) ? a.bias[n < a.Nout ? n : a.Nout - 1] : 0.f;
     }
 
@@ -471,14 +465,14 @@
         }
 #endif
     } else {
-        const int n0 = blockIdx.x * 32;
+        const int n0 = blockIdx.x * RB;
         const bool lead = blockIdx.y == 0;
         float* y = a.y != nullptr ? a.y + (long long)blockIdx.y * a.split_stride : nullptr;
         if (y != nullptr) {
             for (int u = tid; u < 32 * MT * 32; u += NW * 64) {
                 const int nl = u & 31, m = u >> 5;
                 const int n = n0 + nl;
-                if (m >= M || n >= a.Nout) continue;
+                if (m >= M || nl >= RB || n >= a.Nout) continue;
                 float v = sum_partials<NW>(red, nl, LDM, m);
                 if (lead && a.bias != nullptr) v += a.bias[n];
                 y[(size_t)m * a.ldy + n] = v;
@@ -493,7 +487,7 @@
 #pragma unroll
             for (int c = 0; c < CPW; ++c) {
                 const int nl = wave * CPW + c, n = n0 + nl;
-                if (n >= a.Nout) break;
+                if (nl >= RB || n >= a.Nout) break;
                 const float v = sum_partials<NW>(red, nl, LDM, m) + ebias[c];
                 if (v > v1) { v2 = v1; i2 = i1; v1 = v; i1 = n; }
                 else if (v > v2) { v2 = v; i2 = n; }
@@ -515,7 +509,7 @@
                     se = (nm == -__builtin_inff()) ? 0.f : se * __expf(mx - nm) + q4[5] * __expf(q4[4] - nm);
                     mx = nm;
                 }
-                float* rec = a.top2_part + ((size_t)blockIdx.x * 64 + lane) * 6;
+                float* rec = a.top2_part + (VRB ? (size_t)lane * gridDim.x + blockIdx.x : (size_t)blockIdx.x * 64 + lane) * 6;
                 if (a.sel_counter != nullptr) {
                     const float r6[6] = {v1, __int_as_float(i1), v2, __int_as_float(i2), mx, se};
 #pragma unroll
@@ -592,11 +586,12 @@
     return prev;
 }
 
-template <bool LSTM>
+template <bool LSTM, bool VRB = false>
 static int launch_packed(const PackedArgs& a_in, int blocks, hipStream_t st) {
+    static_assert(!VRB || !LSTM, "variable block rows: linear form only");
     PackedArgs a = a_in;
     if (a.M < 1 || a.M > 64 || (a.nquad & 7) || a.nquad < 8) return CVC_E_BADARG;
-    if (a.wstride == 0) a.wstride = (long long)a.nquad * 128;
+    if (a.wstride == 0) a.wstride = (long long)a.nquad * (VRB ? a.rb * 4 : 128);
     const dim3 grid(blocks, LSTM || a.ksplit < 1 ? 1 : a.ksplit);
     if constexpr (LSTM) {
         if (cvc_gemm_split_mode == 2 && cvc_packed_lstm_blocks == 2 && (blocks & 1) == 0 && a.M > 32 && a.h_rm == nullptr && a.c_prev_rm == nullptr) {
@@ -612,21 +607,22 @@
         }
     }
     if (cvc_gemm_split_mode == 2) {
-        if (a.M <= 32) hipLaunchKernelGGL((skinny_gemm_packed_kernel<1, LSTM, CVC_PACKED_DEPTH8, true, 8>), grid, dim3(512), 0, st, a);
-        else hipLaunchKernelGGL((skinny_gemm_packed_kernel<2, LSTM, CVC_PACKED_DEPTH8, true, 8>), grid, dim3(512), 0, st, a);
+        if (a.M <= 32) hipLaunchKernelGGL((skinny_gemm_packed_kernel<1, LSTM, CVC_PACKED_DEPTH8, true, 8, false, 1, false, false, false, VRB>), grid, dim3(512), 0, st, a);
+        else hipLaunchKernelGGL((skinny_gemm_packed_kernel<2, LSTM, CVC_PACKED_DEPTH8, true, 8, false, 1, false, false, false, VRB>), grid, dim3(512), 0, st, a);
     } else if (cvc_gemm_split_mode) {
-        if (a.M <= 32) hipLaunchKernelGGL((skinny_gemm_packed_kernel<1, LSTM, CVC_PACKED_DEPTH, true, 4>), grid, dim3(256), 0, st, a);
-        else hipLaunchKernelGGL((skinny_gemm_packed_kernel<2, LSTM, CVC_PACKED_DEPTH, true, 4>), grid, dim3(256), 0, st, a);
+        if (a.M <= 32) hipLaunchKernelGGL((skinny_gemm_packed_kernel<1, LSTM, CVC_PACKED_DEPTH, true, 4, false, 1, false, false, false, VRB>), grid, dim3(256), 0, st, a);
+        else hipLaunchKernelGGL((skinny_gemm_packed_kernel<2, LSTM, CVC_PACKED_DEPTH, true, 4, false, 1, false, false, false, VRB>), grid, dim3(256), 0, st, a);
     } else {
-        if (a.M <= 32) hipLaunchKernelGGL((skinny_gemm_packed_kernel<1, LSTM, CVC_PACKED_DEPTH, false, 4>), grid, dim3(256), 0, st, a);
-        else hipLaunchKernelGGL((skinny_gemm_packed_kernel<2, LSTM, CVC_PACKED_DEPTH, false, 4>), grid, dim3(256), 0, st, a);
+        if (a.M <= 32) hipLaunchKernelGGL((skinny_gemm_packed_kernel<1, LSTM, CVC_PACKED_DEPTH, false, 4, false, 1, false, false, false, VRB>), grid, dim3(256), 0, st, a);
+        else hipLaunchKernelGGL((skinny_gemm_packed_kernel<2, LSTM, CVC_PACKED_DEPTH, false, 4, false, 1, false, false, false, VRB>), grid, dim3(256), 0, st, a);
     }
     return cvc_launch_status();
 }
 
-template <bool LSTM>
+template <bool LSTM, bool VRB = false>
 static int launch_packed_bf16w(PackedArgs a, int blocks, hipStream_t st) {
-    if (a.wstride == 0) a.wstride = (long long)a.nquad * 128;
+    static_assert(!VRB || !LSTM, "variable block rows: linear form only");
+    if (a.wstride == 0) a.wstride = (long long)a.nquad * (VRB ? a.rb * 4 : 128);
     const dim3 grid(blocks, LSTM || a.ksplit < 1 ? 1 : a.ksplit);
     if constexpr (LSTM) {
         if (a.w_cached) {
@@ -635,8 +631,8 @@
             return cvc_launch_status();
         }
     }
-    if (a.M <= 32) hipLaunchKernelGGL((skinny_gemm_packed_kernel<1, LSTM, CVC_BF16W_DEPTH, true, 8, false, 1, false, false, true>), grid, dim3(512), 0, st, a);
-    else hipLaunchKernelGGL((skinny_gemm_packed_kernel<2, LSTM, CVC_BF16W_DEPTH, true, 8, false, 1, false, false, true>), grid, dim3(512), 0, st, a);
+    if (a.M <= 32) hipLaunchKernelGGL((skinny_gemm_packed_kernel<1, LSTM, CVC_BF16W_DEPTH, true, 8, false, 1, false, false, true, VRB>), grid, dim3(512), 0, st, a);
+    else hipLaunchKernelGGL((skinny_gemm_packed_kernel<2, LSTM, CVC_BF16W_DEPTH, true, 8, false, 1, false, false, true, VRB>), grid, dim3(512), 0, st, a);
     return cvc_launch_status();
 }
 
@@ -969,3 +965,43 @@
     a.bias = bias; a.y = y; a.ldy = ldy; a.ksplit = ksplit; a.split_stride = (long long)M * ldy; a.top2_part = top2_part;
     return launch_packed_bf16w<false>(a, (Nout + 31) / 32, (hipStream_t)stream);
 }
+
+extern "C" int cvc_packed_linear_block_rows(int V) {
+    if (V < 1) return CVC_E_BADARG;
+    static const int cus = [] {
+        int dev = 0, n = 0;
+        if (hipGetDevice(&dev) != hipSuccess || hipDeviceGetAttribute(&n, hipDeviceAttributeMultiprocessorCount, dev) != hipSuccess || n < 1) {
+            (void)hipGetLastError();
+            return 256;
+        }
+        return n;
+    }();
+    const long long rows = 4LL * ((V + 4LL * cus - 1) / (4LL * cus));
+    return rows < 32 ? (int)rows : 32;
+}
+
+static int packed_linear_rows_args(PackedArgs& a, const void* wp, const float* xq, int K, const float* bias, int M, int Nout, int block_rows,
+                                   float* y, int ldy, float* top2_rows) {
+    if (!wp || !xq || (K & 31) || K < 32 || Nout < 1 || M < 1 || M > 64 || block_rows < 1 || block_rows > 32 || (!y && !top2_rows)) return CVC_E_BADARG;
+    if (y != nullptr && ldy < Nout) return CVC_E_BADARG;
+    if (((uintptr_t)wp & 15) || ((uintptr_t)xq & 15)) return CVC_E_BADARG;
+    a.wp = reinterpret_cast<const float*>(wp); a.xq = xq; a.nquad = K / 4; a.M = M; a.Nout = Nout; a.R = 0; a.rb = block_rows;
+    a.bias = bias; a.y = y; a.ldy = ldy; a.ksplit = 1; a.split_stride = (long long)M * ldy; a.top2_part = top2_rows;
+    return 0;
+}
+
+extern "C" int cvc_packed_linear_rows_fwd(const float* wp, const float* xq, int K, const float* bias, int M, int Nout, int block_rows,
+                                          float* y, int ldy, float* top2_rows, cvc_stream_t stream) {
+    PackedArgs a{};
+    const int rc = packed_linear_rows_args(a, wp, xq, K, bias, M, Nout, block_rows, y, ldy, top2_rows);
+    if (rc != 0) return rc;
+    return launch_packed<false, true>(a, (Nout + block_rows - 1) / block_rows, (hipStream_t)stream);
+}
+
+extern "C" int cvc_packed_linear_rows_bf16w_fwd(const uint16_t* wp, const float* xq, int K, const float* bias, int M, int Nout,
+                                                int block_rows, float* y, int ldy, float* top2_rows, cvc_stream_t stream) {
+    PackedArgs a{};
+    const int rc = packed_linear_rows_args(a, wp, xq, K, bias, M, Nout, block_rows, y, ldy, top2_rows);
+    if (rc != 0) return rc;
+    return launch_packed_bf16w<false, true>(a, (Nout + block_rows - 1) / block_rows, (hipStream_t)stream);
+}
diff --git a/cyclical-visual-captioning_amd/csrc/vocab.hip b/cyclical-visual-captioning_amd/csrc/vocab.hip
--- a/cyclical-visual-captioning_amd/csrc/vocab.hip
+++ b/cyclical-visual-captioning_amd/csrc/vocab.hip
@@ -1,6 +1,7 @@
 #include "cvc_common.h"
 #include "gsk.h"
 #include "dropout_rng.h"
+#include "word_select.h"
 #include <math.h>
 
 namespace {
@@ -183,43 +184,39 @@
     }
 }
 
-__global__ __launch_bounds__(WG) void top2_final_kernel(const float* part, int nblocks, int unk, int64_t* word, int wstride,
-                                                        float* logprob, const float* table, int E, float* emb_out, int emb_ld) {
-    __shared__ float red[4];
-    __shared__ Top2 tred[4];
+__global__ __launch_bounds__(WG) void top2_final_kernel(const float* part, int nblocks, long long row_stride, long long blk_stride, int unk,
+                                                        int64_t* word, int wstride, float* logprob, const float* table, int E,
+                                                        float* emb_out, int emb_ld) {
+    using f32x2 = __attribute__((ext_vector_type(2))) float;
+    __shared__ SelState wred[4];
     __shared__ int chosen;
     const int row = blockIdx.x;
-    Top2 t{-INFINITY, 0x7fffffff, -INFINITY, 0x7fffffff};
-    float mx = -INFINITY;
+    const float* base = part + (size_t)row * row_stride;
+    SelState s = sel_init();
     for (int b = threadIdx.x; b < nblocks; b += WG) {
-        const float* rec = part + ((size_t)b * 64 + row) * 6;
-        Top2 u{rec[0], __float_as_int(rec[1]), rec[2], __float_as_int(rec[3])};
-        t = merge(t, u);
-        mx = fmaxf(mx, rec[4]);
+        const f32x2* q2 = reinterpret_cast<const f32x2*>(base + (size_t)b * blk_stride);
+        const f32x2 r0 = q2[0], r1 = q2[1], r2 = q2[2];
+        s = sel_merge(s, r0.x, __float_as_int(r0.y), r1.x, __float_as_int(r1.y), r2.x, r2.y);
     }
 #pragma unroll
     for (int o = 32; o > 0; o >>= 1) {
-        Top2 u;
-        u.v1 = __shfl_xor(t.v1, o, 64); u.i1 = __shfl_xor(t.i1, o, 64);
-        u.v2 = __shfl_xor(t.v2, o, 64); u.i2 = __shfl_xor(t.i2, o, 64);
-        t = merge(t, u);
+        SelState u;
+        u.t1 = __shfl_xor(s.t1, o, 64); u.j1 = __shfl_xor(s.j1, o, 64);
+        u.t2 = __shfl_xor(s.t2, o, 64); u.j2 = __shfl_xor(s.j2, o, 64);
+        u.gm = __shfl_xor(s.gm, o, 64); u.gs = __shfl_xor(s.gs, o, 64);
+        s = sel_merge(s, u);
     }
     const int lane = threadIdx.x & 63, wave = threadIdx.x >> 6;
-    if (lane == 0) tred[wave] = t;
-    mx = block_max(mx, red);
-    t = merge(merge(tred[0], tred[1]), merge(tred[2], tred[3]));
-    float se = 0.f;
-    for (int b = threadIdx.x; b < nblocks; b += WG) {
-        const float* rec = part + ((size_t)b * 64 + row) * 6;
-        se += rec[5] * expf(rec[4] - mx);
-    }
-    se = block_sum(se, red);
+    if (lane == 0) wred[wave] = s;
+    __syncthreads();
     if (threadIdx.x == 0) {
-        const bool use2 = (t.i1 == unk) && t.i2 != 0x7fffffff;
-        int w = use2 ? t.i2 : t.i1;
+#pragma unroll
+        for (int w = 1; w < 4; ++w) s = sel_merge(s, wred[w]);
+        const bool use2 = (s.j1 == unk) && s.j2 != 0x7fffffff;
+        int w = use2 ? s.j2 : s.j1;
         if (w == 0x7fffffff || w < 0) w = 0;
         word[(size_t)row * wstride] = w;
-        if (logprob != nullptr) logprob[row] = (use2 ? t.v2 : t.v1) - (mx + logf(se));
+        if (logprob != nullptr) logprob[row] = (use2 ? s.t2 : s.t1) - (s.gm + logf(s.gs));
         chosen = w;
     }
     if (emb_out != nullptr) {
@@ -887,14 +884,25 @@
     return cvc_launch_status();
 }
 
+static int top2_final_impl(const float* part, int nblocks, long long row_stride, long long blk_stride, int M, int unk_idx, int64_t* word,
+                           int word_stride, float* logprob, const float* table, int E, float* emb_out, int emb_ld, cvc_stream_t stream) {
+    if (!part || !word || nblocks < 1 || M < 1 || M > 64 || word_stride < 1 || ((uintptr_t)part & 7)) return CVC_E_BADARG;
+    if (emb_out != nullptr && (!table || E < 4 || (E & 3) || (emb_ld & 3) || (emb_ld != 0 && emb_ld < E))) return CVC_E_BADARG;
+    hipLaunchKernelGGL(top2_final_kernel, dim3(M), dim3(WG), 0, (hipStream_t)stream, part, nblocks, row_stride, blk_stride, unk_idx, word,
+                       word_stride, logprob, table, E, emb_out, emb_ld);
+    return cvc_launch_status();
+}
+
 extern "C" int cvc_top2_final(const float* part, int nblocks, int M, int unk_idx, int64_t* word, int word_stride,
                               float* logprob, const float* table, int E, float* emb_out, int emb_ld,
                               cvc_stream_t stream) {
-    if (!part || !word || nblocks < 1 || M < 1 || M > 64 || word_stride < 1) return CVC_E_BADARG;
-    if (emb_out != nullptr && (!table || E < 4 || (E & 3) || (emb_ld & 3) || (emb_ld != 0 && emb_ld < E))) return CVC_E_BADARG;
-    hipLaunchKernelGGL(top2_final_kernel, dim3(M), dim3(WG), 0, (hipStream_t)stream, part, nblocks, unk_idx, word, word_stride,
-                       logprob, table, E, emb_out, emb_ld);
-    return cvc_launch_status();
+    return top2_final_impl(part, nblocks, 6, 64 * 6, M, unk_idx, word, word_stride, logprob, table, E, emb_out, emb_ld, stream);
+}
+
+extern "C" int cvc_top2_final_rows(const float* part, int nblocks, int M, int unk_idx, int64_t* word, int word_stride,
+                                   float* logprob, const float* table, int E, float* emb_out, int emb_ld,
+                                   cvc_stream_t stream) {
+    return top2_final_impl(part, nblocks, (long long)nblocks * 6, 6, M, unk_idx, word, word_stride, logprob, table, E, emb_out, emb_ld, stream);
 }
 
 extern "C" int cvc_top2_slab(const cvc_gsk_segs* logits, const float* bias, int V, int M, int unk_idx, int64_t* word,
diff --git a/cyclical-visual-captioning_amd/csrc/word_select.h b/cyclical-visual-captioning_amd/csrc/word_select.h
--- /dev/null
+++ b/cyclical-visual-captioning_amd/csrc/word_select.h
@@ -0,0 +1,17 @@
+#pragma once
+#include "cvc_common.h"
+
+struct SelState { float t1, t2, gm, gs; int j1, j2; };
+__device__ __forceinline__ SelState sel_init() { return SelState{-__builtin_inff(), -__builtin_inff(), -__builtin_inff(), 0.f, 0x7fffffff, 0x7fffffff}; }
+__device__ __forceinline__ bool sel_better(float va, int ia, float vb, int ib) { return (va > vb) | ((va == vb) & (ia < ib)); }
+__device__ __forceinline__ SelState sel_merge(SelState s, float u1, int k1, float u2, int k2, float um, float us) {
+    if (sel_better(u1, k1, s.t1, s.j1)) {
+        if (sel_better(s.t1, s.j1, u2, k2)) { s.t2 = s.t1; s.j2 = s.j1; } else { s.t2 = u2; s.j2 = k2; }
+        s.t1 = u1; s.j1 = k1;
+    } else if (sel_better(u1, k1, s.t2, s.j2)) { s.t2 = u1; s.j2 = k1; }
+    const float nm = fmaxf(s.gm, um);
+    s.gs = (nm == -__builtin_inff()) ? 0.f : s.gs * __expf(s.gm - nm) + us * __expf(um - nm);
+    s.gm = nm;
+    return s;
+}
+__device__ __forceinline__ SelState sel_merge(SelState s, const SelState& u) { return sel_merge(s, u.t1, u.j1, u.t2, u.j2, u.gm, u.gs); }
diff --git a/cyclical-visual-captioning_amd/cvc/decode/engine.py b/cyclical-visual-captioning_amd/cvc/decode/engine.py
--- a/cyclical-visual-captioning_amd/cvc/decode/engine.py
+++ b/cyclical-visual-captioning_amd/cvc/decode/engine.py
@@ -103,7 +103,7 @@
         self.QSPLIT = 8
         self.q_parts = z(self.QSPLIT, rows, A)
         self.emb = z(rows, W.E)
-        self.top2_part = z((V + 31) // 32, 64, 6)
+        self.top2_part = z(max((V + 31) // 32, -(-V // linear_block_rows(V))), 64, 6)
         self.att_steps = z(self.T, rows, N)
         self.words = torch.zeros(self.T + 1, rows, dtype=torch.int64, device=dev)
         self.logprob = z(self.T, rows)
@@ -191,7 +191,7 @@
         if self.packed:
             R = W.R
             d.path, d.qsplit = 0, self.QSPLIT
-            d.w_att, d.w_lang, d.w_h, d.w_o = ptr(W.p_att2 if self.embgate else W.p_att), ptr(W.p_lang), ptr(W.p_h), ptr(W.p_o)
+            d.w_att, d.w_lang, d.w_h, d.w_o = ptr(W.p_att2 if self.embgate else W.p_att), ptr(W.p_lang), ptr(W.p_h), ptr(W.p_o if self.gsk else W.p_o_rows)
             w_fc = W.w_ih_att[:, R:2 * R]
             d.w_fc, d.ld_w_fc = w_fc.data_ptr(), w_fc.stride(0)
             d.gate_fc, d.q_parts, d.top2_part = ptr(self.gate_fc), ptr(self.q_parts), ptr(self.top2_part)
diff --git a/cyclical-visual-captioning_amd/cvc/decode/path_packed.py b/cyclical-visual-captioning_amd/cvc/decode/path_packed.py
--- a/cyclical-visual-captioning_amd/cvc/decode/path_packed.py
+++ b/cyclical-visual-captioning_amd/cvc/decode/path_packed.py
@@ -22,7 +22,11 @@
         if not self.bf16w and not hasattr(W, "p_lang"):
             W.p_lang = pack_weights(torch.cat([W.w_ih_lang, W.w_hh_lang], 1), R)
             W.p_h = pack_weights(W.w_h)
+        if not self.bf16w and self.gsk and not hasattr(W, "p_o"):
             W.p_o = pack_weights(W.w_o)
+        if not self.bf16w and not self.gsk and not hasattr(W, "p_o_rows"):
+            W.vocab_rb = linear_block_rows(W.V)
+            W.p_o_rows = pack_weights_rows(W.w_o, W.vocab_rb)
         if self.embgate and not self.bf16w and not hasattr(W, "p_att2"):
             W.p_att2 = pack_weights(torch.cat([W.w_ih_att[:, 0:R], W.w_hh_att], 1), R)
             W.t_embgate = embgate_table(W)
@@ -69,11 +73,12 @@
         out.append(("gate_fc", L.cvc_linear_fwd, (seg_fc, 1, ptr(W.b_ih_att), ptr(W.b_hh_att), rows, 4 * R, ptr(self.gate_fc),
                                                   4 * R)))
         self._keep.append(seg_fc)
-        nblk_v = (V + 31) // 32
         if self.gsk:
             return out + self._build_gsk_steps()
         if self.embgate:
             return out + self._build_embgate_steps()
+        rb_v = W.vocab_rb
+        nblk_v = (V + rb_v - 1) // rb_v
         for t in range(self.T):
             rd, wr = t & 1, (t + 1) & 1
             XA_r, XA_w, XL_r, XL_w = self.XA[rd], self.XA[wr], self.XL[rd], self.XL[wr]
@@ -117,10 +122,10 @@
                 out.append(("lang_lstm", L.cvc_packed_lstm_fwd, (ptr(W.p_lang), ptr(XL_r), 3 * R, ptr(W.b_ih_lang), ptr(W.b_hh_lang),
                                                                  None, ptr(self.cL[rd]), rows, R, ptr(XA_w), qoff(XL_w, 2 * R),
                                                                  ptr(self.cL[wr]))))
-            out.append(("logits", L.cvc_packed_linear_fwd, (ptr(W.p_o), ptr(XA_w), R, ptr(W.b_o), rows, V, 1, None, V,
-                                                            ptr(self.top2_part))))
-            out.append(("word_select", L.cvc_top2_final, (ptr(self.top2_part), nblk_v, rows, self.unk, ptr(self.words[t + 1]), 1,
-                                                          ptr(self.logprob[t]), ptr(W.embed), E, qoff(XA_w, R), 0)))
+            out.append(("logits", L.cvc_packed_linear_rows_fwd, (ptr(W.p_o_rows), ptr(XA_w), R, ptr(W.b_o), rows, V, rb_v, None, V,
+                                                                 ptr(self.top2_part))))
+            out.append(("word_select", L.cvc_top2_final_rows, (ptr(self.top2_part), nblk_v, rows, self.unk, ptr(self.words[t + 1]), 1,
+                                                               ptr(self.logprob[t]), ptr(W.embed), E, qoff(XA_w, R), 0)))
             self._keep.append(sets)
         return out
 
@@ -131,13 +136,14 @@
         ptr = lambda t: None if t is None else t.data_ptr()
         qoff = lambda buf, k0: buf.data_ptr() + (k0 // 4) * 64 * 4 * 4
         out = []
-        nblk_v = (V + 31) // 32
+        rb_v = W.vocab_rb
+        nblk_v = (V + rb_v - 1) // rb_v
         if self.bf16w:
-            att_fn, linear_fn = L.cvc_packed_lstm_bf16w_fwd, L.cvc_packed_linear_bf16w_fwd
+            att_fn, linear_fn, head_fn = L.cvc_packed_lstm_bf16w_fwd, L.cvc_packed_linear_bf16w_fwd, L.cvc_packed_linear_rows_bf16w_fwd
             w_att, att_stride, embgate, w_h, w_o = W.pb_att2, 2 * R * 32, W.r_embgate, W.pb_h, W.pb_o
         else:
-            att_fn, linear_fn = L.cvc_packed_lstm_embgate_ex_fwd, L.cvc_packed_linear_fwd
-            w_att, att_stride, embgate, w_h, w_o = W.p_att2, (2 * R // 4) * 128, W.t_embgate, W.p_h, W.p_o
+            att_fn, linear_fn, head_fn = L.cvc_packed_lstm_embgate_ex_fwd, L.cvc_packed_linear_fwd, L.cvc_packed_linear_rows_fwd
+            w_att, att_stride, embgate, w_h, w_o = W.p_att2, (2 * R // 4) * 128, W.t_embgate, W.p_h, W.p_o_rows
         for t in range(self.T):
             rd, wr = t & 1, (t + 1) & 1
             XA_r, XA_w, XL_r, XL_w = self.XA[rd], self.XA[wr], self.XL[rd], self.XL[wr]
@@ -171,13 +177,13 @@
                                                                  None, ptr(self.cL[rd]), rows, R, ptr(XA_w), qoff(XL_w, 2 * R),
                                                                  ptr(self.cL[wr]))))
             if self.sampling:
-                out.append(("logits", linear_fn, (ptr(w_o), ptr(XA_w), R, ptr(W.b_o), rows, V, 1, ptr(self.logits), V, None)))
+                out.append(("logits", head_fn, (ptr(w_o), ptr(XA_w), R, ptr(W.b_o), rows, V, rb_v, ptr(self.logits), V, None)))
                 out.append(("word_select", L.cvc_sample_select_parts, (ptr(self.logits), 1, 0, None, rows, V, self.unk, self.inv_tau,
                                                                        ptr(self.rng), t, ptr(self.words[t + 1]), 1,
                                                                        ptr(self.logprob[t]))))
             else:
-                out.append(("logits", linear_fn, (ptr(w_o), ptr(XA_w), R, ptr(W.b_o), rows, V, 1, None, V, ptr(self.top2_part))))
-                out.append(("word_select", L.cvc_top2_final, (ptr(self.top2_part), nblk_v, rows, self.unk, ptr(self.words[t + 1]), 1,
-                                                              ptr(self.logprob[t]), None, 0, None, 0)))
+                out.append(("logits", head_fn, (ptr(w_o), ptr(XA_w), R, ptr(W.b_o), rows, V, rb_v, None, V, ptr(self.top2_part))))
+                out.append(("word_select", L.cvc_top2_final_rows, (ptr(self.top2_part), nblk_v, rows, self.unk, ptr(self.words[t + 1]),
+                                                                   1, ptr(self.logprob[t]), None, 0, None, 0)))
             self._keep.append(sets)
         return out
diff --git a/cyclical-visual-captioning_amd/cvc/decode/weights.py b/cyclical-visual-captioning_amd/cvc/decode/weights.py
--- a/cyclical-visual-captioning_amd/cvc/decode/weights.py
+++ b/cyclical-visual-captioning_amd/cvc/decode/weights.py
@@ -65,6 +65,28 @@
     return out.contiguous()
 
 
+def linear_block_rows(V: int) -> int:
+    rb = int(hip.lib().cvc_packed_linear_block_rows(int(V)))
+    if not 1 <= rb <= 32:
+        raise RuntimeError(f"cvc_packed_linear_block_rows({V}) = {rb}")
+    return rb
+
+
+def pack_weights_rows(w: torch.Tensor, rb: int) -> torch.Tensor:
+    n, k = w.shape
+    assert k % 32 == 0 and 1 <= rb <= 32, (k, rb)
+    nb = (n + rb - 1) // rb
+    if nb * rb != n:
+        w = torch.cat([w, w.new_zeros(nb * rb - n, k)], 0)
+    return w.view(nb, rb, k // 4, 4).permute(0, 2, 1, 3).contiguous()
+
+
+def unpack_weights_rows(p: torch.Tensor, n: Optional[int] = None) -> torch.Tensor:
+    nb, nq, rb = p.shape[0], p.shape[1], p.shape[2]
+    w = p.permute(0, 2, 1, 3).reshape(nb * rb, nq * 4)
+    return w if n is None else w[:n]
+
+
 def lstm_packed_rows(R: int, device) -> torch.Tensor:
     i = torch.arange(32, device=device)
     return (((i >> 3) * R + (i & 7)).view(1, 32) + (torch.arange(R // 8, device=device) * 8).view(-1, 1)).reshape(-1)
@@ -107,13 +129,29 @@
     return w if n is None else w[:n]
 
 
+def pack_weights_rows_bf16(w: torch.Tensor, rb: int) -> torch.Tensor:
+    n, k = w.shape
+    assert k % 32 == 0 and 1 <= rb <= 32, (k, rb)
+    nb = (n + rb - 1) // rb
+    if nb * rb != n:
+        w = torch.cat([w, w.new_zeros(nb * rb - n, k)], 0)
+    return bf16_round(w).to(torch.bfloat16).view(nb, rb, k // 8, 8).permute(0, 2, 1, 3).contiguous()
+
+
+def unpack_weights_rows_bf16(p: torch.Tensor, n: Optional[int] = None) -> torch.Tensor:
+    nb, k8, rb = p.shape[0], p.shape[1], p.shape[2]
+    w = p.permute(0, 2, 1, 3).reshape(nb * rb, k8 * 8).float()
+    return w if n is None else w[:n]
+
+
 def bind_bf16(W: "DecodeWeights") -> "DecodeWeights":
     if hasattr(W, "pb_lang"):
         return W
     R, E = W.R, W.E
     W.pb_att2 = pack_weights_bf16(torch.cat([W.w_ih_att[:, 0:R], W.w_hh_att], 1), R)
     W.pb_h = pack_weights_bf16(W.w_h)
-    W.pb_o = pack_weights_bf16(W.w_o)
+    W.vocab_rb = linear_block_rows(W.V)
+    W.pb_o = pack_weights_rows_bf16(W.w_o, W.vocab_rb)
     W.r_w_fc = bf16_round(W.w_ih_att[:, R:2 * R])
     W.r_embgate = hip.tile_mm(torch.relu(W.embed), bf16_round(W.w_ih_att[:, 2 * R:2 * R + E]))
     W.pb_lang = pack_weights_bf16(torch.cat([W.w_ih_lang, W.w_hh_lang], 1), R)
diff --git a/cyclical-visual-captioning_amd/cvc/hip.py b/cyclical-visual-captioning_amd/cvc/hip.py
--- a/cyclical-visual-captioning_amd/cvc/hip.py
+++ b/cyclical-visual-captioning_amd/cvc/hip.py
@@ -218,6 +218,10 @@
     "cvc_sample_advance": [_P, _P],
     "cvc_packed_lstm_bf16w_fwd": [_P, _LL, _P, _I, _P, _P, _P, _P, _P, _P, _I, _I, _P, _P, _P, _I, _P],
     "cvc_packed_linear_bf16w_fwd": [_P, _P, _I, _P, _I, _I, _I, _P, _I, _P, _P],
+    "cvc_packed_linear_block_rows": [_I],
+    "cvc_packed_linear_rows_fwd": [_P, _P, _I, _P, _I, _I, _I, _P, _I, _P, _P],
+    "cvc_packed_linear_rows_bf16w_fwd": [_P, _P, _I, _P, _I, _I, _I, _P, _I, _P, _P],
+    "cvc_top2_final_rows": [_P, _I, _I, _I, _P, _I, _P, _P, _I, _P, _I, _P],
     "cvc_gather_rows": [_P, _P, _I, _I, _I, _P, _P],
     "cvc_tile_rows_alloc": [_I],
     "cvc_tile_gemm_loaders": [_I],
@@ -257,7 +261,8 @@
     "cvc_tile_gemm_loaders", "cvc_gru_persistent_waves8", "cvc_relu_dropout_fwd", "cvc_relu_dropout_bwd", "cvc_bn_workspace",
     "cvc_bn_relu_train_fwd", "cvc_bn_relu_train_bwd", "cvc_class_softmax_bwd", "cvc_layernorm_cat_bwd", "cvc_stable_order", "cvc_col_sum", "cvc_col_sum_ws", "cvc_attn_weighted_rows",
     "cvc_lstm_persistent_sync_words", "cvc_lstm_seq_persistent_fwd", "cvc_lstm_seq_persistent_train_fwd", "cvc_lstm_seq_fwd", "cvc_lstm_seq_train_fwd", "cvc_lstm_seq_bwd_work", "cvc_lstm_seq_bwd",
-    "cvc_packed_lstm_bf16w_fwd", "cvc_packed_linear_bf16w_fwd"}
+    "cvc_packed_lstm_bf16w_fwd", "cvc_packed_linear_bf16w_fwd",
+    "cvc_packed_linear_block_rows", "cvc_packed_linear_rows_fwd", "cvc_packed_linear_rows_bf16w_fwd", "cvc_top2_final_rows"}
 EXPERIMENTAL = {
     "cvc_gsk_plan", "cvc_gsk_gemm", "cvc_attn_scores_qslab", "cvc_top2_slab", "cvc_packed_lstm_ks_slices", "cvc_packed_lstm_ks_fwd",
     "cvc_packed_lstm_ksf_fwd", "cvc_packed_lstm_ksx_local", "cvc_packed_lstm_ksx_fwd", "cvc_packed_lstm_wg_blocks",
diff --git a/include/cvc_hip_blocks.h b/include/cvc_hip_blocks.h
--- a/include/cvc_hip_blocks.h
+++ b/include/cvc_hip_blocks.h
@@ -164,6 +164,14 @@
 int cvc_packed_linear_bf16w_fwd(const uint16_t* wp, const float* xq, int K, const float* bias, int M, int Nout, int ksplit,
                                 float* y, int ldy, float* top2_part, cvc_stream_t stream);
 
+int cvc_packed_linear_block_rows(int V);
+int cvc_packed_linear_rows_fwd(const float* wp, const float* xq, int K, const float* bias, int M, int Nout, int block_rows,
+                               float* y, int ldy, float* top2_rows, cvc_stream_t stream);
+int cvc_packed_linear_rows_bf16w_fwd(const uint16_t* wp, const float* xq, int K, const float* bias, int M, int Nout,
+                                     int block_rows, float* y, int ldy, float* top2_rows, cvc_stream_t stream);
+int cvc_top2_final_rows(const float* part, int nblocks, int M, int unk_idx, int64_t* word, int word_stride,
+                        float* logprob, const float* table, int E, float* emb_out, int emb_ld, cvc_stream_t stream);
+
 #ifdef __cplusplus
 }
 #endif
```

Result: no change. 331,100 decode-steps/s (-0.4%).
